# vandenheuvel/rust-lp

Measured on AMD Instinct MI355X. Metric: simplex iterations/sec, higher is better.
Workload: dtype f64; 1 GPU; dense10k: synthetic dense LP 10000x10000 f64 (+10000 slack columns), SteepestDescent, dense tableau with blocked f64-MFMA updates; m=10000, n=10000, seed=20250002, engine=tableau, update_block=64, parallelism=single GPU, solves=1

## Files before the change

include/relp_engine.h:

```cpp
#ifndef RELP_ENGINE_H
#define RELP_ENGINE_H

#include <stdint.h>

#ifdef __cplusplus
extern "C" {
#endif

typedef struct relp_engine relp_engine_t;

typedef enum {
    RELP_OK = 0,
    RELP_E_ARG = -1,
    RELP_E_HIP = -2,
    RELP_E_ZERO_PIVOT = -3,
    RELP_E_SINGULAR = -4,
    RELP_E_STATE = -5,
    RELP_E_UNSUPPORTED = -6,
    RELP_E_ALLOC = -7
} relp_status_t;

typedef enum {
    RELP_RUNNING = 0,
    RELP_OPTIMAL = 1,
    RELP_UNBOUNDED = 2,
    RELP_INFEASIBLE = 3,
    RELP_PHASE_ONE_DONE = 4,
    RELP_NO_ROW_PHASE_ONE = 5
} relp_outcome_t;

typedef enum {
    RELP_RULE_FIRST_PROFITABLE = 0,
    RELP_RULE_FIRST_PROFITABLE_WITH_MEMORY = 1,
    RELP_RULE_STEEPEST_DESCENT = 2
} relp_pivot_rule_t;

typedef enum { RELP_FORMAT_CSC = 0, RELP_FORMAT_DENSE = 1 } relp_format_t;
typedef enum { RELP_MEM_HOST = 0, RELP_MEM_DEVICE = 1 } relp_memory_t;

typedef struct {
    int32_t nr_normal;
    int32_t nr_eq, nr_range, nr_le, nr_ge;
    int32_t format;
    int32_t matrix_memory;
    const int64_t *col_ptr;
    const int32_t *row_idx;
    const double  *values;
    const double  *dense;
    int64_t        dense_ld;
    const double  *b;
    const double  *ranges;
    const double  *cost;
    const double  *upper_bound;
} relp_matrix_data_t;

typedef struct {
    int32_t device;
    int32_t phase_one_rule;
    int32_t phase_two_rule;
    double  tol_cost;
    double  tol_pivot;
    double  tol_zero;
    double  tol_tie;
    double  tol_feas;
    int32_t poll_interval;
    int32_t trace_capacity;
    int32_t shard_rank, shard_count;
    int32_t update_block;
    int32_t engine;
    int32_t ratio_rule;
    int32_t artificial_removal;
    int32_t pivot_rescue;
    int32_t auto_reinversion;
} relp_config_t;

typedef enum { RELP_RATIO_REFERENCE = 0, RELP_RATIO_LARGEST_PIVOT = 1 } relp_ratio_rule_t;
typedef enum { RELP_ARTIFICIAL_REFERENCE = 0, RELP_ARTIFICIAL_TEXTBOOK = 1 } relp_artificial_removal_t;

typedef enum {
    RELP_ENGINE_REVISED = 0,
    RELP_ENGINE_TABLEAU = 1,
    RELP_ENGINE_LU = 2,
    RELP_ENGINE_AUTO = 3
} relp_engine_kind_t;

void relp_default_config(relp_config_t *cfg);
void relp_robust_config(relp_config_t *cfg);
int32_t relp_engine_kind(const relp_engine_t *h);
relp_status_t relp_robust_stats(const relp_engine_t *h, int64_t *out4);
const char *relp_last_error(const relp_engine_t *h);
const char *relp_version(void);

relp_status_t relp_engine_create(const relp_matrix_data_t *md, const relp_config_t *cfg, relp_engine_t **out);
void          relp_engine_destroy(relp_engine_t *h);
relp_status_t relp_set_stream(relp_engine_t *h, void *hip_stream);

relp_status_t relp_select_primal_pivot_column(relp_engine_t *h, int32_t rule, int32_t *found,
                                              int32_t *column, double *relative_cost);
relp_status_t relp_relative_costs(relp_engine_t *h, double *out_n);
relp_status_t relp_generate_column(relp_engine_t *h, int32_t column, double *out_m);
relp_status_t relp_generate_element(relp_engine_t *h, int32_t row, int32_t column, double *out);
relp_status_t relp_select_primal_pivot_row(relp_engine_t *h, int32_t *found, int32_t *row);
relp_status_t relp_select_primal_pivot_row_of(relp_engine_t *h, const double *column_m, int32_t *found, int32_t *row);
relp_status_t relp_bring_into_basis(relp_engine_t *h, int32_t column, int32_t row, double relative_cost,
                                    int32_t *leaving_column);

relp_status_t relp_run(relp_engine_t *h, int64_t max_iters, int64_t *iterations_done, int32_t *outcome);
relp_status_t relp_solve_relaxation(relp_engine_t *h, int64_t max_iters, int32_t *outcome);
relp_status_t relp_from_basis(relp_engine_t *h, const int32_t *basis_columns_m);
relp_status_t relp_set_reinversion_interval(relp_engine_t *h, int64_t pivots);
int64_t       relp_reinversions(const relp_engine_t *h);
relp_status_t relp_flush(relp_engine_t *h);
relp_status_t relp_tab_flush_stats(relp_engine_t *h, int64_t *out2);
int32_t       relp_update_block(const relp_engine_t *h);
relp_status_t relp_lu_stats(const relp_engine_t *h, int64_t *out8);
relp_status_t relp_lu_lookahead_stats(const relp_engine_t *h, int64_t *out4);
relp_status_t relp_lu_kernel_layout(const relp_engine_t *h, int32_t *out4);
relp_status_t relp_lu_set_device_factorisation(relp_engine_t *h, int32_t on);
relp_status_t relp_lu_device_factorisation_stats(const relp_engine_t *h, int64_t *out6);
relp_status_t relp_lu_factor_residual(relp_engine_t *h, double *out);

relp_status_t relp_lu_phase_cycles(relp_engine_t *h, int64_t *out16);

relp_status_t relp_basis_inverse_row(relp_engine_t *h, int32_t row, double *out_m);
relp_status_t relp_should_refactor(relp_engine_t *h, int32_t *out);
relp_status_t relp_generate_column_of(relp_engine_t *h, const int32_t *row_idx, const double *values, int32_t nnz, double *out_m);
relp_status_t relp_cost_difference_of(relp_engine_t *h, const int32_t *row_idx, const double *values, int32_t nnz, double *out);
relp_status_t relp_lu_change_basis(relp_engine_t *h, int32_t pivot_row_index);
relp_status_t relp_lu_set_factors(relp_engine_t *h, const int64_t *l_col_ptr, const int32_t *l_row_idx, const double *l_values,
                                  const int64_t *u_col_ptr, const int32_t *u_row_idx, const double *u_values);
relp_status_t relp_lu_updates(relp_engine_t *h, int32_t *count);
relp_status_t relp_lu_get_update(relp_engine_t *h, int32_t k, int32_t *pivot, int32_t *idx, double *values, int32_t cap, int32_t *nnz);
relp_status_t relp_lu_get_upper(relp_engine_t *h, int64_t *col_ptr_m1, int32_t *row_idx, double *values, int64_t cap, int64_t *nnz);

int32_t relp_nr_rows(const relp_engine_t *h);
int32_t relp_nr_columns(const relp_engine_t *h);
int32_t relp_phase(const relp_engine_t *h);
int32_t relp_nr_artificial(const relp_engine_t *h);
relp_status_t relp_get_objective(relp_engine_t *h, double *out);
relp_status_t relp_get_b(relp_engine_t *h, double *out_m);
relp_status_t relp_get_minus_pi(relp_engine_t *h, double *out_m);
relp_status_t relp_get_basis_indices(relp_engine_t *h, int32_t *out_m);
relp_status_t relp_get_basis_inverse(relp_engine_t *h, double *out_mm);
relp_status_t relp_current_bfs(relp_engine_t *h, int32_t *cols, double *vals, int32_t cap, int32_t *count);
relp_status_t relp_get_iterations(relp_engine_t *h, int64_t *out);
relp_status_t relp_get_degenerate_pivots(relp_engine_t *h, int64_t *out);
relp_status_t relp_get_trace(relp_engine_t *h, int32_t *phase, int32_t *entering, int32_t *row,
                             int32_t *leaving, int64_t cap, int64_t *count);
relp_status_t relp_check_basis(relp_engine_t *h, double *max_identity_error, double *max_basic_cost,
                               double *min_b);

typedef enum {
    RELP_K_PRICE = 0, RELP_K_SELECT_COLUMN = 1, RELP_K_BUILD_COLUMN = 2, RELP_K_FTRAN = 3,
    RELP_K_RATIO = 4, RELP_K_UPDATE_VECTORS = 5, RELP_K_UPDATE_INVERSE = 6,
    RELP_K_APPLY_W = 7,
    RELP_K_UPDATE_W = 8,
    RELP_K_FLUSH = 9,
    RELP_K_FT_RUN = 10,
    RELP_K_COUNT = 11
} relp_kernel_id_t;
relp_status_t relp_profile_enable(relp_engine_t *h, int32_t enable, int64_t max_launches, int32_t sample_every);
relp_status_t relp_profile_read(relp_engine_t *h, int32_t kernel_id, int64_t *launches, double *total_ms);

relp_status_t relp_synth_fill_dense(double *device_a, int64_t ld, int32_t m, int32_t n, uint64_t seed,
                                    int64_t first_column, void *hip_stream);
relp_status_t relp_device_alloc(void **out, int64_t bytes);
relp_status_t relp_device_free(void *p);

relp_status_t relp_shard_ranges(const relp_engine_t *h, int32_t *col_lo, int32_t *col_hi,
                                int32_t *row_lo, int32_t *row_hi, int32_t *row_slice_stride);
void          relp_shard_column_range(int32_t nr_normal, int32_t rank, int32_t count, int32_t *lo, int32_t *hi);
int64_t       relp_shard_candidate_len(const relp_engine_t *h);
int64_t       relp_shard_rho_len(const relp_engine_t *h);
relp_status_t relp_shard_price(relp_engine_t *h, double *dev_candidate);
relp_status_t relp_shard_select_column(relp_engine_t *h, const double *dev_candidates, int32_t count);
relp_status_t relp_shard_ftran(relp_engine_t *h, double *dev_alpha_slice);
relp_status_t relp_shard_ratio(relp_engine_t *h, const double *dev_alpha_slices, int32_t count, double *dev_rho);
relp_status_t relp_shard_update(relp_engine_t *h, const double *dev_rho);
relp_status_t relp_shard_plan(const relp_matrix_data_t *md, const relp_config_t *cfg, int32_t *col_lo, int32_t *col_hi);
relp_status_t relp_shard_pivot(relp_engine_t *h);
relp_status_t relp_shard_flush_begin(relp_engine_t *h, double **dev_snapshot, int64_t *len_doubles);
relp_status_t relp_shard_flush_end(relp_engine_t *h);
relp_status_t relp_poll(relp_engine_t *h, int32_t *outcome, int64_t *iterations);

typedef int (*relp_allgather_fn)(void *ctx, const void *dev_send, void *dev_recv, int64_t bytes_per_rank, void *hip_stream);
typedef int (*relp_allreduce_sum_fn)(void *ctx, double *dev_buf, int64_t count, void *hip_stream);
relp_status_t relp_shard_set_collectives(relp_engine_t *h, relp_allgather_fn allgather, relp_allreduce_sum_fn allreduce_sum,
                                         void *ctx);
relp_status_t relp_shard_run(relp_engine_t *h, int64_t max_iters, int64_t *done, int32_t *outcome);
relp_status_t relp_shard_inject_failure(relp_engine_t *h, int64_t after_pivots);
#define RELP_RCCL_ID_BYTES 128
relp_status_t relp_rccl_unique_id(uint8_t id[RELP_RCCL_ID_BYTES]);
relp_status_t relp_rccl_attach(relp_engine_t *h, const uint8_t id[RELP_RCCL_ID_BYTES]);

#ifdef __cplusplus
}
#endif
#endif
```

rust-lp_amd/csrc/relp_abi.cpp:

```cpp
#include <cstring>
#include <new>

#include "relp_engine.hpp"

using relp::Engine;

struct relp_engine { Engine impl; };

#define H(h) ((h)->impl)

extern "C" {

void relp_default_config(relp_config_t* cfg) {
    std::memset(cfg, 0, sizeof(*cfg));
    cfg->device = -1;
    cfg->phase_one_rule = RELP_RULE_FIRST_PROFITABLE_WITH_MEMORY;
    cfg->phase_two_rule = RELP_RULE_STEEPEST_DESCENT;
    cfg->tol_cost = 1e-7; cfg->tol_pivot = 1e-5; cfg->tol_zero = 1e-11; cfg->tol_tie = 1e-9; cfg->tol_feas = 1e-7;
    cfg->poll_interval = 64;
    cfg->trace_capacity = 0;
    cfg->shard_rank = 0; cfg->shard_count = 1;
    cfg->update_block = -1;
    cfg->engine = RELP_ENGINE_REVISED;
}

void relp_robust_config(relp_config_t* cfg) {
    relp_default_config(cfg);
    cfg->ratio_rule = RELP_RATIO_LARGEST_PIVOT;
    cfg->artificial_removal = RELP_ARTIFICIAL_TEXTBOOK;
    cfg->pivot_rescue = 1;
    cfg->auto_reinversion = 1;
    cfg->engine = RELP_ENGINE_AUTO;
}
int32_t relp_engine_kind(const relp_engine_t* h) { return h ? H(h).engine_kind() : -1; }
relp_status_t relp_robust_stats(const relp_engine_t* h, int64_t* out4) { return (h && out4) ? H(h).robust_stats(out4) : RELP_E_ARG; }

const char* relp_last_error(const relp_engine_t* h) { return h ? H(h).last_error() : "null handle"; }
const char* relp_version(void) { return "relp-mi355x 0.2 (gfx950; engines: explicit inverse, dense tableau, sparse LU + Forrest-Tomlin)"; }

relp_status_t relp_engine_create(const relp_matrix_data_t* md, const relp_config_t* cfg, relp_engine_t** out) {
    if (!md || !cfg || !out) return RELP_E_ARG;
    relp_engine_t* h = new (std::nothrow) relp_engine_t();
    if (!h) return RELP_E_ALLOC;
    relp_status_t st = H(h).create(*md, *cfg);
    *out = h;
    return st;
}

void relp_engine_destroy(relp_engine_t* h) { delete h; }
relp_status_t relp_set_stream(relp_engine_t* h, void* s) { return h ? H(h).set_stream((hipStream_t)s) : RELP_E_ARG; }

relp_status_t relp_select_primal_pivot_column(relp_engine_t* h, int32_t rule, int32_t* found, int32_t* column, double* cost) {
    return h ? H(h).select_primal_pivot_column(rule, found, column, cost) : RELP_E_ARG;
}
relp_status_t relp_relative_costs(relp_engine_t* h, double* out) { return (h && out) ? H(h).relative_costs(out) : RELP_E_ARG; }
relp_status_t relp_generate_column(relp_engine_t* h, int32_t column, double* out) { return h ? H(h).generate_column(column, out) : RELP_E_ARG; }
relp_status_t relp_generate_element(relp_engine_t* h, int32_t row, int32_t column, double* out) {
    return h ? H(h).generate_element(row, column, out) : RELP_E_ARG;
}
relp_status_t relp_select_primal_pivot_row(relp_engine_t* h, int32_t* found, int32_t* row) {
    return h ? H(h).select_primal_pivot_row(found, row) : RELP_E_ARG;
}
relp_status_t relp_select_primal_pivot_row_of(relp_engine_t* h, const double* column, int32_t* found, int32_t* row) {
    return (h && column) ? H(h).select_primal_pivot_row_of(column, found, row) : RELP_E_ARG;
}
relp_status_t relp_bring_into_basis(relp_engine_t* h, int32_t column, int32_t row, double cost, int32_t* leaving) {
    return h ? H(h).bring_into_basis(column, row, cost, leaving) : RELP_E_ARG;
}

relp_status_t relp_run(relp_engine_t* h, int64_t max_iters, int64_t* done, int32_t* outcome) {
    return h ? H(h).run(max_iters, done, outcome) : RELP_E_ARG;
}
relp_status_t relp_solve_relaxation(relp_engine_t* h, int64_t max_iters, int32_t* outcome) {
    return h ? H(h).solve_relaxation(max_iters, outcome) : RELP_E_ARG;
}
relp_status_t relp_from_basis(relp_engine_t* h, const int32_t* basis) { return (h && basis) ? H(h).from_basis(basis) : RELP_E_ARG; }

relp_status_t relp_flush(relp_engine_t* h) { return h ? H(h).flush() : RELP_E_ARG; }
relp_status_t relp_set_reinversion_interval(relp_engine_t* h, int64_t pivots) { return h ? H(h).set_reinversion_interval(pivots) : RELP_E_ARG; }
int64_t relp_reinversions(const relp_engine_t* h) { return h ? H(h).reinversions() : -1; }
int32_t relp_update_block(const relp_engine_t* h) { return h ? H(h).update_block() : -1; }
relp_status_t relp_lu_stats(const relp_engine_t* h, int64_t* out8) { return (h && out8) ? H(h).lu_stats(out8) : RELP_E_ARG; }
relp_status_t relp_lu_lookahead_stats(const relp_engine_t* h, int64_t* out4) { return (h && out4) ? H(h).lu_lookahead_stats(out4) : RELP_E_ARG; }
relp_status_t relp_lu_kernel_layout(const relp_engine_t* h, int32_t* out4) { return (h && out4) ? H(h).lu_kernel_layout(out4) : RELP_E_ARG; }
relp_status_t relp_lu_set_device_factorisation(relp_engine_t* h, int32_t on) { return h ? H(h).lu_set_device_factorisation(on != 0) : RELP_E_ARG; }
relp_status_t relp_lu_factor_residual(relp_engine_t* h, double* out) { return (h && out) ? H(h).lu_factor_residual(out) : RELP_E_ARG; }
relp_status_t relp_lu_device_factorisation_stats(const relp_engine_t* h, int64_t* out6) { return (h && out6) ? H(h).luf_stats(out6) : RELP_E_ARG; }
relp_status_t relp_shard_inject_failure(relp_engine_t* h, int64_t after_pivots) { if (!h) return RELP_E_ARG; H(h).shard_inject_failure(after_pivots); return RELP_OK; }
relp_status_t relp_lu_phase_cycles(relp_engine_t* h, int64_t* out16) { return (h && out16) ? H(h).lu_phase_cycles(out16) : RELP_E_ARG; }
relp_status_t relp_basis_inverse_row(relp_engine_t* h, int32_t row, double* out_m) { return (h && out_m) ? H(h).basis_inverse_row(row, out_m) : RELP_E_ARG; }
relp_status_t relp_should_refactor(relp_engine_t* h, int32_t* out) { return (h && out) ? H(h).should_refactor(out) : RELP_E_ARG; }
relp_status_t relp_generate_column_of(relp_engine_t* h, const int32_t* idx, const double* val, int32_t nnz, double* out_m) {
    return h ? H(h).generate_column_of(idx, val, nnz, out_m) : RELP_E_ARG;
}
relp_status_t relp_cost_difference_of(relp_engine_t* h, const int32_t* idx, const double* val, int32_t nnz, double* out) {
    return h ? H(h).cost_difference_of(idx, val, nnz, out) : RELP_E_ARG;
}
relp_status_t relp_lu_change_basis(relp_engine_t* h, int32_t row) { return h ? H(h).lu_change_basis(row) : RELP_E_ARG; }
relp_status_t relp_lu_set_factors(relp_engine_t* h, const int64_t* l_ptr, const int32_t* l_idx, const double* l_val,
                                  const int64_t* u_ptr, const int32_t* u_idx, const double* u_val) {
    return h ? H(h).lu_set_factors(l_ptr, l_idx, l_val, u_ptr, u_idx, u_val) : RELP_E_ARG;
}
relp_status_t relp_lu_updates(relp_engine_t* h, int32_t* count) { return (h && count) ? H(h).lu_updates(count) : RELP_E_ARG; }
relp_status_t relp_lu_get_update(relp_engine_t* h, int32_t k, int32_t* pivot, int32_t* idx, double* val, int32_t cap, int32_t* nnz) {
    return h ? H(h).lu_get_update(k, pivot, idx, val, cap, nnz) : RELP_E_ARG;
}
relp_status_t relp_lu_get_upper(relp_engine_t* h, int64_t* col_ptr, int32_t* row_idx, double* values, int64_t cap, int64_t* nnz) {
    return h ? H(h).lu_get_upper(col_ptr, row_idx, values, cap, nnz) : RELP_E_ARG;
}
relp_status_t relp_shard_flush_begin(relp_engine_t* h, double** snap, int64_t* len) {
    return h ? H(h).shard_flush_begin(snap, len) : RELP_E_ARG;
}
relp_status_t relp_shard_flush_end(relp_engine_t* h) { return h ? H(h).shard_flush_end() : RELP_E_ARG; }
relp_status_t relp_shard_set_collectives(relp_engine_t* h, relp_allgather_fn ag, relp_allreduce_sum_fn ar, void* ctx) {
    return h ? H(h).shard_set_collectives(ag, ar, ctx) : RELP_E_ARG;
}
relp_status_t relp_shard_run(relp_engine_t* h, int64_t max_iters, int64_t* done, int32_t* outcome) {
    return h ? H(h).shard_run(max_iters, done, outcome) : RELP_E_ARG;
}
relp_status_t relp_rccl_attach(relp_engine_t* h, const uint8_t* id) { return (h && id) ? H(h).rccl_attach(id) : RELP_E_ARG; }

int32_t relp_nr_rows(const relp_engine_t* h) { return h ? H(h).nr_rows() : -1; }
int32_t relp_nr_columns(const relp_engine_t* h) { return h ? H(h).nr_columns() : -1; }
int32_t relp_phase(const relp_engine_t* h) { return h ? H(h).phase() : -1; }
int32_t relp_nr_artificial(const relp_engine_t* h) { return h ? H(h).nr_artificial() : -1; }
relp_status_t relp_get_objective(relp_engine_t* h, double* out) { return (h && out) ? H(h).get_objective(out) : RELP_E_ARG; }
relp_status_t relp_get_b(relp_engine_t* h, double* out) { return (h && out) ? H(h).get_vector(0, out) : RELP_E_ARG; }
relp_status_t relp_get_minus_pi(relp_engine_t* h, double* out) { return (h && out) ? H(h).get_vector(1, out) : RELP_E_ARG; }
relp_status_t relp_get_basis_indices(relp_engine_t* h, int32_t* out) { return (h && out) ? H(h).get_basis_indices(out) : RELP_E_ARG; }
relp_status_t relp_get_basis_inverse(relp_engine_t* h, double* out) { return (h && out) ? H(h).get_basis_inverse(out) : RELP_E_ARG; }
relp_status_t relp_current_bfs(relp_engine_t* h, int32_t* cols, double* vals, int32_t cap, int32_t* count) {
    return h ? H(h).current_bfs(cols, vals, cap, count) : RELP_E_ARG;
}
relp_status_t relp_get_iterations(relp_engine_t* h, int64_t* out) { return (h && out) ? H(h).get_iterations(out) : RELP_E_ARG; }
relp_status_t relp_get_degenerate_pivots(relp_engine_t* h, int64_t* out) { return (h && out) ? H(h).get_degenerate_pivots(out) : RELP_E_ARG; }
relp_status_t relp_tab_flush_stats(relp_engine_t* h, int64_t* out2) { return (h && out2) ? H(h).tab_flush_stats(out2) : RELP_E_ARG; }
relp_status_t relp_get_trace(relp_engine_t* h, int32_t* phase, int32_t* entering, int32_t* row, int32_t* leaving,
                             int64_t cap, int64_t* count) {
    return h ? H(h).get_trace(phase, entering, row, leaving, cap, count) : RELP_E_ARG;
}
relp_status_t relp_check_basis(relp_engine_t* h, double* e1, double* e2, double* mb) { return h ? H(h).check_basis(e1, e2, mb) : RELP_E_ARG; }

relp_status_t relp_profile_enable(relp_engine_t* h, int32_t enable, int64_t max_launches, int32_t sample_every) {
    return h ? H(h).profile_enable(enable != 0, max_launches, sample_every) : RELP_E_ARG;
}
relp_status_t relp_profile_read(relp_engine_t* h, int32_t kid, int64_t* launches, double* total_ms) {
    return h ? H(h).profile_read(kid, launches, total_ms) : RELP_E_ARG;
}

relp_status_t relp_synth_fill_dense(double* device_a, int64_t ld, int32_t m, int32_t n, uint64_t seed,
                                    int64_t first_column, void* hip_stream) {
    if (!device_a || ld < m || m < 0 || n < 0) return RELP_E_ARG;
    relp::launch_fill_dense(device_a, ld, m, n, seed, first_column, (hipStream_t)hip_stream);
    if (hipStreamSynchronize((hipStream_t)hip_stream) != hipSuccess) return RELP_E_HIP;
    return hipGetLastError() == hipSuccess ? RELP_OK : RELP_E_HIP;
}
relp_status_t relp_device_alloc(void** out, int64_t bytes) {
    if (!out || bytes < 0) return RELP_E_ARG;
    return hipMalloc(out, (size_t)(bytes ? bytes : 1)) == hipSuccess ? RELP_OK : RELP_E_ALLOC;
}
relp_status_t relp_device_free(void* p) { return hipFree(p) == hipSuccess ? RELP_OK : RELP_E_HIP; }

relp_status_t relp_shard_ranges(const relp_engine_t* h, int32_t* col_lo, int32_t* col_hi, int32_t* row_lo,
                                int32_t* row_hi, int32_t* stride) {
    if (!h) return RELP_E_ARG;
    H(h).shard_ranges(col_lo, col_hi, row_lo, row_hi, stride);
    return RELP_OK;
}
void relp_shard_column_range(int32_t nr_normal, int32_t rank, int32_t count, int32_t* lo, int32_t* hi) {
    relp::shard_column_range(nr_normal, rank, count, lo, hi);
}
int64_t relp_shard_candidate_len(const relp_engine_t* h) { return h ? H(h).candidate_len() : -1; }
int64_t relp_shard_rho_len(const relp_engine_t* h) { return h ? H(h).rho_len() : -1; }
relp_status_t relp_shard_price(relp_engine_t* h, double* c) { return (h && c) ? H(h).shard_price(c) : RELP_E_ARG; }
relp_status_t relp_shard_select_column(relp_engine_t* h, const double* c, int32_t count) {
    return (h && c) ? H(h).shard_select_column(c, count) : RELP_E_ARG;
}
relp_status_t relp_shard_ftran(relp_engine_t* h, double* a) { return (h && a) ? H(h).shard_ftran(a) : RELP_E_ARG; }
relp_status_t relp_shard_ratio(relp_engine_t* h, const double* a, int32_t count, double* rho) {
    return (h && a && rho) ? H(h).shard_ratio(a, count, rho) : RELP_E_ARG;
}
relp_status_t relp_shard_update(relp_engine_t* h, const double* rho) { return (h && rho) ? H(h).shard_update(rho) : RELP_E_ARG; }
relp_status_t relp_shard_pivot(relp_engine_t* h) { return h ? H(h).shard_pivot() : RELP_E_ARG; }
relp_status_t relp_shard_plan(const relp_matrix_data_t* md, const relp_config_t* cfg, int32_t* col_lo, int32_t* col_hi) {
    if (!md || !cfg) return RELP_E_ARG;
    relp::Layout layout;
    const relp_status_t st = layout.plan(*md, *cfg, nullptr);
    if (st) return st;
    if (col_lo) *col_lo = layout.col_lo;
    if (col_hi) *col_hi = layout.col_hi;
    return RELP_OK;
}
relp_status_t relp_poll(relp_engine_t* h, int32_t* outcome, int64_t* iterations) { return h ? H(h).poll(outcome, iterations) : RELP_E_ARG; }

}
```

rust-lp_amd/csrc/relp_engine.cpp:

```cpp
#include "relp_engine_internal.hpp"

#include <algorithm>
#include <chrono>
#include <cmath>
#include <cstdio>
#include <cstdlib>
#include <cstring>
#include <limits>

namespace relp {

bool Engine::hip_ok(hipError_t e, const char* what) {
    if (e == hipSuccess) return true;
    err_ = std::string(what) + ": " + hipGetErrorString(e);
    return false;
}

void Engine::free_all() {
    luf_release();
    auto fr = [](auto*& p) { if (p) { (void)hipFree(p); p = nullptr; } };
    if (owns_A_) fr(dA_);
    dA_ = nullptr;
    fr(dBinv_); fr(d_minus_pi_); fr(d_b_); fr(d_alpha_); fr(d_aq_); fr(d_rho_); fr(d_d_); fr(d_w_); fr(d_cost_);
    fr(d_basis_); fr(d_column_to_row_); fr(d_bound_row_); fr(d_vrow0_); fr(d_vrow1_); fr(d_vsign_); fr(d_trace_);
    fr(d_in_basis_); fr(d_rec_);
    fr(d_part_k1_); fr(d_part_j_);
    fr(d_fcols_); fr(d_fcount_); fr(d_fmask_); fr(d_fstats_); fr(d_R0c_);
    fr(dT0_); fr(dR0_); fr(d_b_alt_); fr(d_basis_alt_); fr(d_shadow_); fr(d_shadow_meta_);
    if (h_lu_buf_) { (void)hipHostFree(h_lu_buf_); h_lu_buf_ = nullptr; h_lu_cap_ = 0; }
    if (h_basis_) { (void)hipHostFree(h_basis_); h_basis_ = nullptr; }
    if (h_mirror_) { (void)hipHostFree(h_mirror_); h_mirror_ = nullptr; d_mirror_ = nullptr; }
    fr(d_cost_store_); fr(d_idcol_); fr(d_rmin_);
    fr(d_msg_cand_); fr(d_msg_cands_); fr(d_msg_slice_); fr(d_msg_slices_); fr(d_msg_rho_); fr(d_msg_status_); fr(d_msg_statuses_);
    fr(d_v_); fr(d_W_); fr(d_wr_); fr(d_R_); fr(d_S_); fr(d_pos_of_row_);
    fr(d_cptr_); fr(d_cidx_); fr(d_cval_); fr(d_lu_buf_); fr(d_lu_buf_alt_); fr(d_lu_scratch_); fr(d_ft_buf_); fr(d_pe_buf_);
    if (h_ft_hdr_) { (void)hipHostFree(h_ft_hdr_); h_ft_hdr_ = nullptr; }
    if (h_rec_) { (void)hipHostFree(h_rec_); h_rec_ = nullptr; }
    for (auto e : prof_ev_) (void)hipEventDestroy(e);
    prof_ev_.clear();
    if (owns_stream_ && stream_) { (void)hipStreamDestroy(stream_); }
    stream_ = nullptr;
}

Engine::~Engine() { rccl_release(); free_all(); }

ColumnTable Engine::table() const {
    ColumnTable ct;
    ct.nr_artificial = lay_.nr_artificial;
    ct.nr_normal = lay_.nr_normal;
    ct.nr_virtual = lay_.nr_virtual;
    ct.nr_constraints = lay_.mc;
    ct.column_to_row = d_column_to_row_;
    ct.bound_row = d_bound_row_;
    ct.vrow0 = d_vrow0_;
    ct.vrow1 = d_vrow1_;
    ct.vsign = d_vsign_;
    ct.cost = d_cost_;
    return ct;
}

Tolerances Engine::tolerances() const { return Tolerances{cfg_.tol_cost, cfg_.tol_pivot, cfg_.tol_zero, cfg_.tol_tie, cfg_.ratio_rule, (pivot_guard_on_ && guard_rel_ > 0.0) ? 1 : 0, guard_rel_}; }

TableauView Engine::tview() const {
    TableauView tv;
    tv.T0 = dT0_ - (int64_t)lay_.sc_lo * ld_t_; tv.ld_t = ld_t_;
    tv.R0 = dR0_ - (int64_t)lay_.sc_lo; tv.ld_r = ld_r_;
    tv.d = d_d_; tv.m = lay_.m; tv.n_store = n_store_;
    tv.col_off = phase_ == 1 ? 0 : tab_na_;
    tv.n = nr_columns();
    tv.c_lo = lay_.sc_lo; tv.c_hi = lay_.sc_hi;
    return tv;
}

FlushList Engine::flush_list() const {
    FlushList fl;
    fl.cols = d_fcols_; fl.count = d_fcount_; fl.mask = d_fmask_; fl.R0c = d_R0c_; fl.ld = ld_r_; fl.stats = d_fstats_;
    return fl;
}

SelectPartials Engine::tab_partials(int rule) const {
    SelectPartials sp;
    sp.k1 = d_part_k1_; sp.j = d_part_j_; sp.in_basis = d_in_basis_; sp.tol_cost = cfg_.tol_cost; sp.rule = rule;
    sp.n = nr_columns(); sp.offset = 0; sp.nb_struct = 0; sp.tol_tie = cfg_.tol_tie; sp.p_lo = 0; sp.cols_per_slot = 8;
    return sp;
}

DeferredUpdate Engine::deferred() const {
    DeferredUpdate du;
    du.W = d_W_; du.ld = ld_b_; du.kmax = block_; du.S = d_S_; du.pos_of_row = d_pos_of_row_; du.wr = d_wr_; du.R = d_R_;
    return du;
}

relp_status_t Engine::download_rec() {
    HIP_TRY(hipMemcpyAsync(h_rec_, d_rec_, sizeof(PivotRecord), hipMemcpyDeviceToHost, stream_));
    HIP_TRY(hipStreamSynchronize(stream_));
    return RELP_OK;
}

relp_status_t Engine::upload_rec() {
    HIP_TRY(hipMemcpyAsync(d_rec_, h_rec_, sizeof(PivotRecord), hipMemcpyHostToDevice, stream_));
    HIP_TRY(hipStreamSynchronize(stream_));
    return RELP_OK;
}

relp_status_t Engine::set_stream(hipStream_t s) {
    if (stream_) HIP_TRY(hipStreamSynchronize(stream_));
    if (owns_stream_ && stream_) HIP_TRY(hipStreamDestroy(stream_));
    stream_ = s;
    owns_stream_ = false;
    return RELP_OK;
}

relp_status_t Engine::create(const relp_matrix_data_t& md, const relp_config_t& cfg) {
    (void)hipGetLastError();
    cfg_ = cfg;
    if (cfg_.shard_count < 1) cfg_.shard_count = 1;
    if (cfg_.poll_interval < 1) cfg_.poll_interval = 64;
    if (const relp_status_t lst = lay_.build(md, cfg_, &err_)) return lst;
    if (cfg_.device >= 0) HIP_TRY(hipSetDevice(cfg_.device));
    phase_ = 1;
    n_alloc_ = lay_.nr_columns();

    HIP_TRY(hipStreamCreateWithFlags(&stream_, hipStreamNonBlocking));
    owns_stream_ = true;
    const int32_t n_local = lay_.col_hi - lay_.col_lo;
    lu_ = lay_.engine == RELP_ENGINE_LU;
    tableau_ = lay_.engine == RELP_ENGINE_TABLEAU;
    if (lu_) {
        if (cfg_.shard_count > 1) return fail(RELP_E_UNSUPPORTED, "the LU engine is not sharded");
        relp_status_t lst = lu_load_matrix(md);
        if (lst) return lst;
    } else if (md.format == RELP_FORMAT_DENSE) {
        if (lay_.nr_normal > 0 && lay_.mc > 0 && !md.dense) return fail(RELP_E_ARG, "dense matrix missing");
        const int64_t src_ld = md.dense_ld > 0 ? md.dense_ld : lay_.mc;
        if (src_ld < lay_.mc) return fail(RELP_E_ARG, "dense_ld < nr_constraints");
        if (md.matrix_memory == RELP_MEM_DEVICE && (src_ld % 2) == 0) {
            dA_ = const_cast<double*>(md.dense); ld_a_ = src_ld; owns_A_ = false;
        } else {
            ld_a_ = round_up(std::max<int64_t>(lay_.mc, 1), 2);
            HIP_TRY(dev_alloc(&dA_, ld_a_ * std::max(n_local, 1)));
            owns_A_ = true;
            if (n_local > 0 && lay_.mc > 0)
                HIP_TRY(hipMemcpy2D(dA_, ld_a_ * sizeof(double), md.dense, src_ld * sizeof(double), lay_.mc * sizeof(double),
                                    n_local, md.matrix_memory == RELP_MEM_DEVICE ? hipMemcpyDeviceToDevice : hipMemcpyHostToDevice));
        }
    } else if (md.format == RELP_FORMAT_CSC) {
        if (md.matrix_memory != RELP_MEM_HOST) return fail(RELP_E_UNSUPPORTED, "CSC input must be in host memory");
        if (!md.col_ptr) return fail(RELP_E_ARG, "col_ptr missing");
        ld_a_ = round_up(std::max<int64_t>(lay_.mc, 1), 2);
        const int64_t e0 = n_local > 0 ? md.col_ptr[lay_.col_lo] : 0, e1 = n_local > 0 ? md.col_ptr[lay_.col_hi] : 0;
        for (int64_t p = e0; p < e1; ++p)
            if (md.row_idx[p] < 0 || md.row_idx[p] >= lay_.mc) return fail(RELP_E_ARG, "row index out of range");
        const int64_t cells = ld_a_ * std::max(n_local, 1);
        HIP_TRY(dev_alloc(&dA_, cells));
        owns_A_ = true;
        HIP_TRY(hipMemset(dA_, 0, (size_t)cells * sizeof(double)));
        if (e1 > e0) {
            int64_t* t_ptr = nullptr; int32_t* t_idx = nullptr; double* t_val = nullptr;
            auto drop = [&]() { if (t_ptr) (void)hipFree(t_ptr); if (t_idx) (void)hipFree(t_idx); if (t_val) (void)hipFree(t_val); };
            if (hipMalloc(reinterpret_cast<void**>(&t_ptr), sizeof(int64_t) * (size_t)(n_local + 1)) != hipSuccess ||
                hipMalloc(reinterpret_cast<void**>(&t_idx), sizeof(int32_t) * (size_t)(e1 - e0)) != hipSuccess ||
                hipMalloc(reinterpret_cast<void**>(&t_val), sizeof(double) * (size_t)(e1 - e0)) != hipSuccess) {
                drop();
                return fail(RELP_E_ALLOC, "staging the CSC arrays");
            }
            hipError_t err = hipMemcpy(t_ptr, md.col_ptr + lay_.col_lo, sizeof(int64_t) * (size_t)(n_local + 1), hipMemcpyHostToDevice);
            if (err == hipSuccess) err = hipMemcpy(t_idx, md.row_idx + e0, sizeof(int32_t) * (size_t)(e1 - e0), hipMemcpyHostToDevice);
            if (err == hipSuccess) err = hipMemcpy(t_val, md.values + e0, sizeof(double) * (size_t)(e1 - e0), hipMemcpyHostToDevice);
            if (err == hipSuccess) {
                launch_csc_to_dense(t_ptr, t_idx, t_val, n_local, dA_, ld_a_, nullptr);
                err = hipDeviceSynchronize();
            }
            drop();
            if (err != hipSuccess) return fail(RELP_E_HIP, "dense copy of the CSC input");
        }
    } else {
        return fail(RELP_E_ARG, "unknown matrix format");
    }

    ld_b_ = round_up(lay_.m, 16);
    const int64_t rows_local = std::max(lay_.row_hi - lay_.row_lo, 1);
    HIP_TRY(dev_alloc(&dBinv_, (tableau_ || lu_) ? 16 : rows_local * ld_b_));
    HIP_TRY(dev_alloc(&d_minus_pi_, ld_b_));
    HIP_TRY(dev_alloc(&d_b_, ld_b_));
    HIP_TRY(dev_alloc(&d_alpha_, ld_b_));
    HIP_TRY(dev_alloc(&d_aq_, ld_b_));
    HIP_TRY(dev_alloc(&d_rho_, ld_b_));
    HIP_TRY(dev_alloc(&d_w_, ld_b_));
    HIP_TRY(dev_alloc(&d_d_, n_alloc_));
    HIP_TRY(dev_alloc(&d_cost_, lay_.nr_normal));
    HIP_TRY(dev_alloc(&d_basis_, lay_.m));
    HIP_TRY(dev_alloc(&d_column_to_row_, lay_.nr_artificial));
    HIP_TRY(dev_alloc(&d_bound_row_, lay_.nr_normal));
    HIP_TRY(dev_alloc(&d_vrow0_, lay_.nr_virtual));
    HIP_TRY(dev_alloc(&d_vrow1_, lay_.nr_virtual));
    HIP_TRY(dev_alloc(&d_vsign_, lay_.nr_virtual));
    HIP_TRY(dev_alloc(&d_in_basis_, n_alloc_));
    HIP_TRY(dev_alloc(&d_rec_, 1));
    {
        const int64_t slots = price_structural_blocks(lay_.col_lo, lay_.col_hi) + (lay_.nr_artificial + lay_.nr_virtual + 255) / 256 + 8 +
                              tab_scan_blocks(n_alloc_) + price_csc_blocks(0, lay_.nr_normal);
        HIP_TRY(dev_alloc(&d_part_k1_, slots));
        HIP_TRY(dev_alloc(&d_part_j_, slots));
    }
    block_ = cfg_.update_block < 0 ? (lay_.m >= 4096 ? 64 : 0) : std::min(cfg_.update_block, 128);
    if (lu_) {
        block_ = cfg_.update_block < 0 ? 128 : std::max(1, std::min(cfg_.update_block, 128));
        HIP_TRY(dev_alloc(&d_lu_scratch_, ld_b_));
        {
            const char* la = std::getenv("RELP_LU_LOOKAHEAD");
            const char* fl = std::getenv("RELP_FUSE_LANES");
            const char* df = std::getenv("RELP_LU_DEVICE_FACTOR");
            luf_enabled_ = df && std::atoi(df) != 0;
            luf_download_ = df && std::atoi(df) == 2;
            lu_lookahead_env_ = la ? std::atoi(la) : 8;
            lu_lookahead_set_ = la != nullptr;
            lu_fuse_lanes_env_ = fl ? std::atoi(fl) : 256;
        }
        relp_status_t fst = ft_plan_and_alloc();
        if (fst) return fst;
    }
    if (tableau_) {
        if (block_ == 0) block_ = 64;
        if (cfg_.update_block < 0 && lay_.m >= 4096 && n_alloc_ >= 40000) block_ = 96;
        n_store_ = n_alloc_;
        tab_na_ = lay_.nr_artificial;
        const int64_t n_owned = std::max(lay_.sc_hi - lay_.sc_lo, 1);
        ld_t_ = round_up(lay_.m, 2);
        ld_r_ = round_up(n_owned, 2);
        HIP_TRY(dev_alloc(&dT0_, ld_t_ * n_owned));
        HIP_TRY(dev_alloc(&dR0_, ld_r_ * (block_ + 1)));
        {
            const char* e = std::getenv("RELP_TAB_FLUSH_ALL");
            flush_all_ = e && std::atoi(e) != 0;
            HIP_TRY(dev_alloc(&d_fstats_, 2));
            if (!flush_all_) {
                HIP_TRY(dev_alloc(&d_fcols_, n_owned));
                HIP_TRY(dev_alloc(&d_fcount_, 1));
                HIP_TRY(dev_alloc(&d_fmask_, (n_owned + 63) / 64));
                HIP_TRY(dev_alloc(&d_R0c_, ld_r_ * block_));
            }
        }
        {
            const char* e = std::getenv("RELP_FUSED_UPDATE");
            fused_update_ = !(e && std::atoi(e) == 0);
            if (cfg_.pivot_rescue && cfg_.shard_count == 1) fused_update_ = false;
            if (fused_update_) {
                HIP_TRY(dev_alloc(&d_b_alt_, ld_b_));
                HIP_TRY(dev_alloc(&d_basis_alt_, lay_.m));
                HIP_TRY(dev_alloc(&d_shadow_, std::max(block_, 1) + 1));
                HIP_TRY(hipMalloc(reinterpret_cast<void**>(&d_shadow_meta_), 2 * sizeof(int32_t)));
                const int32_t none[2] = {-1, 0};
                HIP_TRY(hipMemcpy(d_shadow_meta_, none, sizeof none, hipMemcpyHostToDevice));
            }
        }
        HIP_TRY(dev_alloc(&d_cost_store_, n_store_));
        HIP_TRY(dev_alloc(&d_idcol_, lay_.m));
    }
    if (block_ > 0 && ft_) {
        HIP_TRY(dev_alloc(&d_v_, ld_b_));
    } else if (block_ > 0) {
        HIP_TRY(dev_alloc(&d_v_, ld_b_));
        HIP_TRY(dev_alloc(&d_W_, ld_b_ * block_));
        if (!tableau_) HIP_TRY(dev_alloc(&d_R_, ld_b_ * block_));
        HIP_TRY(dev_alloc(&d_wr_, block_));
        HIP_TRY(dev_alloc(&d_S_, block_));
        HIP_TRY(dev_alloc(&d_pos_of_row_, lay_.m));
        HIP_TRY(hipMemset(d_pos_of_row_, 0xFF, sizeof(int32_t) * lay_.m));
    }
    HIP_TRY(dev_alloc(&d_rmin_, lay_.m / 8 + 2));
    HIP_TRY(hipHostMalloc(reinterpret_cast<void**>(&h_rec_), sizeof(PivotRecord), hipHostMallocDefault));
    trace_cap_ = std::max(cfg_.trace_capacity, 0);
    if (trace_cap_ > 0) HIP_TRY(dev_alloc(&d_trace_, 4 * trace_cap_));

    auto up = [&](void* dst, const void* src, size_t bytes) -> hipError_t {
        return bytes ? hipMemcpy(dst, src, bytes, hipMemcpyHostToDevice) : hipSuccess;
    };
    HIP_TRY(up(d_cost_, lay_.cost.data(), sizeof(double) * lay_.nr_normal));
    HIP_TRY(up(d_bound_row_, lay_.bound_row.data(), sizeof(int32_t) * lay_.nr_normal));
    HIP_TRY(up(d_vrow0_, lay_.vrow0.data(), sizeof(int32_t) * lay_.nr_virtual));
    HIP_TRY(up(d_vrow1_, lay_.vrow1.data(), sizeof(int32_t) * lay_.nr_virtual));
    HIP_TRY(up(d_vsign_, lay_.vsign.data(), sizeof(int32_t) * lay_.nr_virtual));
    HIP_TRY(up(d_column_to_row_, lay_.column_to_row.data(), sizeof(int32_t) * lay_.nr_artificial));
    HIP_TRY(up(d_basis_, lay_.basis.data(), sizeof(int32_t) * lay_.m));
    HIP_TRY(up(d_b_, lay_.rhs.data(), sizeof(double) * lay_.m));
    HIP_TRY(up(d_minus_pi_, lay_.minus_pi.data(), sizeof(double) * lay_.m));
    std::vector<uint8_t> flags(n_alloc_, 0);
    for (int32_t r = 0; r < lay_.m; ++r) flags[lay_.basis[r]] = 1;
    HIP_TRY(up(d_in_basis_, flags.data(), flags.size()));
    if (lay_.row_hi > lay_.row_lo && !tableau_ && !lu_) launch_set_identity(dBinv_, ld_b_, lay_.row_lo, lay_.row_hi, stream_);
    if (tableau_) {
        idcol_h_ = lay_.basis;
        HIP_TRY(up(d_idcol_, idcol_h_.data(), sizeof(int32_t) * lay_.m));
        const double* A = dA_ - (int64_t)lay_.col_lo * ld_a_;
        launch_tab_build(tview(), A, ld_a_, table(), stream_);
        cost_store_h_.assign(n_store_, 0.0);
        for (int32_t k = 0; k < lay_.nr_artificial; ++k) cost_store_h_[k] = 1.0;
        std::vector<double> w(ld_b_, 0.0);
        for (int32_t k = 0; k < lay_.nr_artificial; ++k) w[lay_.column_to_row[k]] = 1.0;
        HIP_TRY(up(d_cost_store_, cost_store_h_.data(), sizeof(double) * n_store_));
        HIP_TRY(up(d_w_, w.data(), sizeof(double) * ld_b_));
        launch_tab_price_init(tview(), d_w_, d_cost_store_, stream_);
    }
    {
        bool sparse_input = false;
        if (md.format == RELP_FORMAT_CSC && md.col_ptr && lay_.nr_normal > 0 && lay_.mc > 0)
            sparse_input = (double)md.col_ptr[lay_.nr_normal] <= 0.10 * (double)lay_.nr_normal * (double)lay_.mc;
        reinvert_interval_ = (!lu_ && cfg_.shard_count == 1 && lay_.m <= 4096 && sparse_input) ? 1000 : 0;
        if (cfg_.auto_reinversion && !lu_ && cfg_.shard_count == 1) reinvert_interval_ = 256;
    }
    std::memset(h_rec_, 0, sizeof(PivotRecord));
    h_rec_->outcome = DEV_RUNNING;
    h_rec_->minus_objective = -lay_.phase1_objective;
    h_rec_->last_selected = -1;
    h_rec_->phase = 1;
    relp_status_t st = upload_rec();
    if (st) return st;
    HIP_TRY(hipDeviceSynchronize());
    if (hipGetLastError() != hipSuccess) return fail(RELP_E_HIP, "a kernel launch of the set-up failed");
    if (lu_ && (st = lu_refactor())) return st;
    return RELP_OK;
}

relp_status_t Engine::profile_enable(bool enable, int64_t max_launches, int32_t sample_every) {
    prof_stride_ = sample_every > 0 ? sample_every : 1;
    prof_tick_ = 0;
    HIP_TRY(hipStreamSynchronize(stream_));
    for (auto e : prof_ev_) (void)hipEventDestroy(e);
    prof_ev_.clear(); prof_kid_.clear(); prof_open_ = false;
    prof_on_ = enable;
    if (enable) {
        prof_ev_.resize((size_t)max_launches * 2);
        for (auto& e : prof_ev_) HIP_TRY(hipEventCreate(&e));
        prof_kid_.reserve((size_t)max_launches);
    }
    return RELP_OK;
}

void Engine::prof_begin(int kid, hipStream_t on) {
    prof_open_ = false;
    if (!prof_on_ || (prof_kid_.size() + 1) * 2 > prof_ev_.size()) return;
    if (kid != RELP_K_FLUSH && (prof_tick_ % prof_stride_) != 0) return;
    (void)hipEventRecord(prof_ev_[2 * prof_kid_.size()], on ? on : stream_);
    prof_kid_.push_back(kid);
    prof_open_ = true;
}

void Engine::prof_end(hipStream_t on) {
    if (!prof_open_) return;
    (void)hipEventRecord(prof_ev_[2 * (prof_kid_.size() - 1) + 1], on ? on : stream_);
    prof_open_ = false;
}

relp_status_t Engine::profile_read(int kernel_id, int64_t* launches, double* total_ms) {
    HIP_TRY(hipStreamSynchronize(stream_));
    int64_t n = 0; double ms = 0.0;
    for (size_t k = 0; k < prof_kid_.size(); ++k) {
        if (prof_kid_[k] != kernel_id) continue;
        float t = 0.f;
        if (hipEventElapsedTime(&t, prof_ev_[2 * k], prof_ev_[2 * k + 1]) == hipSuccess) { ms += t; ++n; }
    }
    if (launches) *launches = n;
    if (total_ms) *total_ms = ms;
    return RELP_OK;
}

void Engine::enqueue_price(int cost_mode, const double* vec, const PivotRecord* rec, int32_t p_lo, int32_t p_hi) {
    const ColumnTable ct = table();
    if (lu_) {
        launch_price_csc(csc(), ct, vec, d_d_, 0, lay_.nr_normal, cost_mode, SelectPartials{}, rec, stream_);
        launch_price_virtual(ct, vec, d_d_, cost_mode, rec, stream_);
        return;
    }
    const double* A = dA_ - (int64_t)lay_.col_lo * ld_a_;
    launch_price_structural(A, ld_a_, ct, vec, d_d_, p_lo, p_hi, cost_mode, rec, stream_);
    if (p_lo > 0 || p_hi < lay_.nr_normal) launch_price_mask_unowned(ct, d_d_, p_lo, p_hi, rec, stream_);
    launch_price_virtual(ct, vec, d_d_, cost_mode, rec, stream_);
}

void Engine::enqueue_iteration_tableau(int rule) {
    const TableauView tv = tview();
    const DeferredUpdate du = deferred();
    const SelectPartials sp = tab_partials(rule);
    if (fused_update_ && in_loop_) {
        prof_begin(RELP_K_FTRAN);
        launch_tab_select_column_rmin(tv, du, sp, tab_scan_blocks(lay_.sc_hi - lay_.sc_lo), d_alpha_, d_b_, tolerances(), d_rmin_,
                                      d_rec_, stream_, d_shadow_, d_shadow_meta_);
        prof_end();
        prof_begin(RELP_K_PRICE);
        launch_tab_ratio_update_all(tv, du, sp, lay_.m, d_alpha_, d_b_, d_b_alt_, d_basis_, d_basis_alt_, d_in_basis_, d_trace_,
                                    trace_cap_, tolerances(), d_rmin_, d_shadow_, d_shadow_meta_, d_rec_, stream_);
        prof_end();
        std::swap(d_b_, d_b_alt_);
        std::swap(d_basis_, d_basis_alt_);
        shadow_pending_ = true;
        if (++since_flush_ >= block_) enqueue_flush();
        return;
    }
    tab_settle();
    prof_begin(RELP_K_FTRAN);
    launch_tab_select_column_rmin(tv, du, sp, tab_scan_blocks(lay_.sc_hi - lay_.sc_lo), d_alpha_, d_b_, tolerances(), d_rmin_,
                                  d_rec_, stream_);
    prof_end();
    prof_begin(RELP_K_RATIO);
    launch_ratio_blocks(d_alpha_, d_b_, d_basis_, lay_.m, tolerances(), du, d_rmin_, d_rec_, stream_);
    prof_end();
    prof_begin(RELP_K_PRICE);
    launch_tab_update_all(tv, du, sp, lay_.m, d_alpha_, d_b_, d_basis_, d_in_basis_, d_trace_, trace_cap_, d_rec_, stream_);
    prof_end();
    if (++since_flush_ >= block_) enqueue_flush();
}

void Engine::enqueue_iteration(int rule) {
    struct Tick { int64_t& t; ~Tick() { ++t; } } tick{prof_tick_};
    if (tableau_) { enqueue_iteration_tableau(rule); return; }
    if (lu_) { enqueue_iteration_lu(rule); return; }
    const ColumnTable ct = table();
    const double* A = dA_ - (int64_t)lay_.col_lo * ld_a_;
    double* Binv = dBinv_ - (int64_t)lay_.row_lo * ld_b_;
    const int n = nr_columns();
    SelectPartials sp;
    sp.k1 = d_part_k1_; sp.j = d_part_j_; sp.in_basis = d_in_basis_; sp.tol_cost = cfg_.tol_cost; sp.rule = rule;
    const int nb_struct = price_structural_blocks(lay_.col_lo, lay_.col_hi);
    sp.n = n; sp.offset = 0; sp.nb_struct = nb_struct; sp.tol_tie = cfg_.tol_tie; sp.p_lo = lay_.col_lo; sp.cols_per_slot = 8;
    const int nb_virt = price_virtual_blocks(ct);
    prof_begin(RELP_K_PRICE);
    if (lay_.col_lo > 0 || lay_.col_hi < lay_.nr_normal) {
        launch_price_structural_sel(A, ld_a_, ct, d_minus_pi_, d_d_, lay_.col_lo, lay_.col_hi, phase_, sp, d_rec_, stream_);
        launch_price_mask_unowned(ct, d_d_, lay_.col_lo, lay_.col_hi, d_rec_, stream_);
        SelectPartials spv = sp;
        spv.offset = nb_struct;
        launch_price_virtual_sel(ct, d_minus_pi_, d_d_, phase_, spv, d_rec_, stream_);
    } else {
        launch_price_all_sel(A, ld_a_, ct, d_minus_pi_, d_d_, lay_.col_lo, lay_.col_hi, phase_, sp, d_rec_, stream_);
    }
    prof_end();
    prof_begin(RELP_K_SELECT_COLUMN);
    launch_select_partials(sp, nb_struct + nb_virt, d_d_, A, ld_a_, ct, lay_.m, d_aq_, d_rec_, stream_);
    prof_end();
    if (block_ == 0) {
        prof_begin(RELP_K_FTRAN);
        launch_ftran_rmin(Binv, ld_b_, lay_.m, d_aq_, d_alpha_, d_b_, tolerances(), d_rmin_, d_rec_, stream_);
        prof_end();
        prof_begin(RELP_K_RATIO);
        launch_ratio_rows(d_alpha_, d_b_, d_basis_, lay_.m, tolerances(), DeferredUpdate{}, d_rmin_, ftran_rows_per_block(), d_rec_,
                          stream_);
        prof_end();
        prof_begin(RELP_K_UPDATE_VECTORS);
        launch_compute_rho(Binv, ld_b_, lay_.m, lay_.row_lo, lay_.row_hi, d_rho_, d_rec_, stream_);
        prof_end();
        prof_begin(RELP_K_UPDATE_INVERSE);
        launch_update_inverse_vectors(Binv, ld_b_, lay_.m, d_alpha_, d_rho_, d_b_, d_minus_pi_, d_basis_, d_in_basis_, d_trace_,
                                      trace_cap_, d_rec_, stream_);
        prof_end();
        return;
    }
    const DeferredUpdate du = deferred();
    prof_begin(RELP_K_FTRAN);
    launch_ftran(Binv, ld_b_, lay_.m, lay_.row_lo, lay_.row_hi, d_aq_, d_v_, 0, d_rec_, stream_);
    prof_end();
    prof_begin(RELP_K_APPLY_W);
    launch_apply_w_rmin(du, lay_.m, d_v_, d_alpha_, d_b_, tolerances(), d_rmin_, d_rec_, stream_);
    prof_end();
    prof_begin(RELP_K_RATIO);
    launch_ratio_rows(d_alpha_, d_b_, d_basis_, lay_.m, tolerances(), du, d_rmin_, 256, d_rec_, stream_);
    prof_end();
    prof_begin(RELP_K_UPDATE_W);
    launch_update_w(du, lay_.m, d_alpha_, d_rec_, stream_);
    launch_rho_deferred(du, Binv, ld_b_, lay_.m, lay_.row_lo, lay_.row_hi, d_rho_, d_rec_, stream_);
    prof_end();
    prof_begin(RELP_K_UPDATE_VECTORS);
    launch_update_vectors(lay_.m, d_alpha_, d_rho_, d_b_, d_minus_pi_, d_basis_, d_in_basis_, d_trace_, trace_cap_, d_rec_,
                          stream_);
    prof_end();
    if (++since_flush_ >= block_) enqueue_flush();
}

void Engine::tab_settle() {
    if (shadow_pending_) {
        launch_tab_apply_shadow(deferred(), d_shadow_, d_shadow_meta_, stream_);
        shadow_pending_ = false;
    }
}

void Engine::enqueue_flush() {
    if (block_ == 0) return;
    if (lu_) {
        if (since_flush_ == 0 && !ft_need_refactor_) return;
        prof_begin(RELP_K_FLUSH);
        const relp_status_t st = lu_refactor();
        prof_end();
        if (st && !lu_status_) lu_status_ = st;
        return;
    }
    if (tableau_) {
        tab_settle();
        const DeferredUpdate dut = deferred();
        prof_begin(RELP_K_FLUSH);
        launch_tab_flush(tview(), dut, d_rec_, flush_list(), stream_);
        launch_flush_reset(dut, d_rec_, stream_);
        prof_end();
        since_flush_ = 0;
        if (++flushes_since_reprice_ >= kRepriceEveryFlushes) {
            flushes_since_reprice_ = 0;
            const TableauView tv = tview();
            const int rule = phase_ == 1 ? cfg_.phase_one_rule : cfg_.phase_two_rule;
            launch_tab_basis_costs(tv, d_basis_, d_cost_store_, d_w_, stream_);
            launch_tab_price_init(tv, d_w_, d_cost_store_, stream_);
            launch_tab_scan(tv, tab_partials(rule), d_rec_, stream_);
        }
        return;
    }
    const DeferredUpdate du = deferred();
    double* Binv = dBinv_ - (int64_t)lay_.row_lo * ld_b_;
    prof_begin(RELP_K_FLUSH);
    launch_flush_snapshot(du, Binv, ld_b_, lay_.row_lo, lay_.row_hi, d_rec_, stream_);
    launch_flush_apply(du, Binv, ld_b_, lay_.m, lay_.row_lo, lay_.row_hi, d_rec_, stream_);
    launch_flush_reset(du, d_rec_, stream_);
    prof_end();
    since_flush_ = 0;
}

relp_status_t Engine::flush() {
    tab_settle();
    if (cfg_.shard_count > 1 && block_ > 0 && !tableau_) {
        if (!coll_allreduce_) return fail(RELP_E_STATE, "sharded flush needs relp_shard_flush_begin/end (or the collective hooks)");
        if (since_flush_ == 0) return RELP_OK;
        double* snap = nullptr; int64_t len = 0;
        relp_status_t st = shard_flush_begin(&snap, &len);
        if (st) return st;
        if (len > 0) {
            if (coll_allreduce_(coll_ctx_, snap, len, stream_)) return fail(RELP_E_HIP, "all-reduce of the flush snapshot failed");
            if ((st = shard_flush_end())) return st;
        }
        since_flush_ = 0;
        return RELP_OK;
    }
    enqueue_flush();
    return RELP_OK;
}

relp_status_t Engine::select_primal_pivot_column(int rule, int32_t* found, int32_t* column, double* cost) {
    relp_status_t st = download_rec();
    if (st) return st;
// ... 954 lines not shown
```

rust-lp_amd/csrc/relp_engine.hpp:

```cpp
#pragma once
#include <hip/hip_runtime.h>

#include <cstdint>
#include <chrono>
#include <condition_variable>
#include <functional>
#include <mutex>
#include <string>
#include <thread>
#include <vector>

#include "../../include/relp_engine.h"
#include "relp_kernels.h"
#include "relp_layout.hpp"
#include "relp_lu.hpp"

namespace relp {

class Engine {
  public:
    Engine() = default;
    ~Engine();

    relp_status_t create(const relp_matrix_data_t& md, const relp_config_t& cfg);
    relp_status_t set_stream(hipStream_t s);

    relp_status_t select_primal_pivot_column(int rule, int32_t* found, int32_t* column, double* cost);
    relp_status_t relative_costs(double* out_n);
    relp_status_t generate_column(int32_t column, double* out_m);
    relp_status_t generate_element(int32_t row, int32_t column, double* out);
    relp_status_t select_primal_pivot_row(int32_t* found, int32_t* row);
    relp_status_t select_primal_pivot_row_of(const double* column, int32_t* found, int32_t* row);
    relp_status_t bring_into_basis(int32_t column, int32_t row, double cost, int32_t* leaving);

    relp_status_t run(int64_t max_iters, int64_t* done, int32_t* outcome);
    int32_t engine_kind() const { return lay_.engine; }
    relp_status_t robust_stats(int64_t* out4) const;
    relp_status_t solve_relaxation(int64_t max_iters, int32_t* outcome);
    relp_status_t from_basis(const int32_t* basis_columns);
    relp_status_t set_reinversion_interval(int64_t pivots);
    int64_t reinversions() const { return reinversions_; }
    relp_status_t flush();
    int32_t update_block() const { return block_; }
    relp_status_t lu_stats(int64_t* out8) const;
    relp_status_t lu_lookahead_stats(int64_t* out4) const;
    relp_status_t lu_kernel_layout(int32_t* out4) const;
    relp_status_t luf_stats(int64_t* out6) const;
    relp_status_t lu_set_device_factorisation(bool on);
    relp_status_t lu_factor_residual(double* out);
    relp_status_t lu_basis_columns(std::vector<std::vector<std::pair<int32_t, double>>>& cols);
    relp_status_t lu_basis_flat(std::vector<int64_t>& ptr, std::vector<int32_t>& idx, std::vector<double>& val);
    relp_status_t lu_phase_cycles(int64_t* out16);
    relp_status_t lu_download_basis();
    relp_status_t lu_factor_downloaded_basis();
    relp_status_t lu_refactor_lookahead(int rule, int64_t budget, bool have_basis);
    relp_status_t ft_read_report(bool* have_basis);
    void lu_refactor_clock(std::chrono::steady_clock::time_point tb, std::chrono::steady_clock::time_point t0,
                           std::chrono::steady_clock::time_point t1, std::chrono::steady_clock::time_point t2);
    relp_status_t basis_inverse_row(int32_t row, double* out_m);
    relp_status_t should_refactor(int32_t* out);
    relp_status_t generate_column_of(const int32_t* idx, const double* val, int32_t nnz, double* out_m);
    relp_status_t cost_difference_of(const int32_t* idx, const double* val, int32_t nnz, double* out);
    relp_status_t lu_change_basis(int32_t row);
    relp_status_t lu_updates(int32_t* count);
    relp_status_t lu_get_update(int32_t k, int32_t* pivot, int32_t* idx, double* val, int32_t cap, int32_t* nnz);
    relp_status_t lu_get_upper(int64_t* col_ptr, int32_t* row_idx, double* values, int64_t cap, int64_t* nnz);
    relp_status_t lu_set_factors(const int64_t* l_ptr, const int32_t* l_idx, const double* l_val, const int64_t* u_ptr,
                                 const int32_t* u_idx, const double* u_val);
    relp_status_t shard_flush_begin(double** dev_snapshot, int64_t* len);
    relp_status_t shard_flush_end();

    int32_t nr_rows() const { return lay_.m; }
    int32_t nr_columns() const { return lay_.nr_columns(); }
    int32_t phase() const { return phase_; }
    int32_t nr_artificial() const { return lay_.nr_artificial; }
    relp_status_t get_objective(double* out);
    relp_status_t get_vector(int which, double* out);
    relp_status_t get_basis_indices(int32_t* out);
    relp_status_t get_basis_inverse(double* out);
    relp_status_t current_bfs(int32_t* cols, double* vals, int32_t cap, int32_t* count);
    relp_status_t get_iterations(int64_t* out);
    relp_status_t get_degenerate_pivots(int64_t* out);
    relp_status_t tab_flush_stats(int64_t* out2);
    relp_status_t get_trace(int32_t* phase, int32_t* entering, int32_t* row, int32_t* leaving, int64_t cap,
                            int64_t* count);
    relp_status_t check_basis(double* max_identity_error, double* max_basic_cost, double* min_b);

    relp_status_t profile_enable(bool enable, int64_t max_launches, int32_t sample_every);
    relp_status_t profile_read(int kernel_id, int64_t* launches, double* total_ms);

    void shard_ranges(int32_t* col_lo, int32_t* col_hi, int32_t* row_lo, int32_t* row_hi, int32_t* stride) const;
    int64_t candidate_len() const { return lay_.candidate_len; }
    int64_t rho_len() const { return ld_b_; }
    relp_status_t shard_price(double* dev_candidate);
    relp_status_t shard_select_column(const double* dev_candidates, int32_t count);
    relp_status_t shard_ftran(double* dev_alpha_slice);
    relp_status_t shard_ratio(const double* dev_alpha_slices, int32_t count, double* dev_rho);
    relp_status_t shard_update(const double* dev_rho);
    relp_status_t shard_pivot();
    relp_status_t shard_set_collectives(relp_allgather_fn ag, relp_allreduce_sum_fn ar, void* ctx);
    relp_status_t shard_run(int64_t max_iters, int64_t* done, int32_t* outcome);
    void shard_inject_failure(int64_t after_pivots) { inject_failure_after_ = after_pivots; }
    relp_status_t rccl_attach(const uint8_t* id);
    relp_status_t poll(int32_t* outcome, int64_t* iterations);

    const char* last_error() const { return err_.c_str(); }

  private:
    Layout lay_;
    relp_config_t cfg_{};
    int32_t phase_ = 1;

    double* dA_ = nullptr; int64_t ld_a_ = 0; bool owns_A_ = false;
    double* dBinv_ = nullptr; int64_t ld_b_ = 0;
    double *d_minus_pi_ = nullptr, *d_b_ = nullptr, *d_alpha_ = nullptr, *d_aq_ = nullptr, *d_rho_ = nullptr,
           *d_d_ = nullptr, *d_w_ = nullptr, *d_cost_ = nullptr;
    int32_t *d_basis_ = nullptr, *d_column_to_row_ = nullptr, *d_bound_row_ = nullptr, *d_vrow0_ = nullptr,
            *d_vrow1_ = nullptr, *d_vsign_ = nullptr, *d_trace_ = nullptr;
    uint8_t* d_in_basis_ = nullptr;
    PivotRecord* d_rec_ = nullptr;
    PivotRecord* h_rec_ = nullptr;
    hipStream_t stream_ = nullptr; bool owns_stream_ = false;
    int64_t trace_cap_ = 0;
    int32_t block_ = 0;
    int64_t since_flush_ = 0;
    double* d_v_ = nullptr;
    double *d_W_ = nullptr, *d_wr_ = nullptr, *d_R_ = nullptr;
    int32_t *d_S_ = nullptr, *d_pos_of_row_ = nullptr;
    double* d_part_k1_ = nullptr;
    int32_t* d_part_j_ = nullptr;
    bool tableau_ = false;
    double* dT0_ = nullptr; int64_t ld_t_ = 0;
    double* dR0_ = nullptr; int64_t ld_r_ = 0;
    bool flush_all_ = false;
    int32_t *d_fcols_ = nullptr, *d_fcount_ = nullptr;
    unsigned long long *d_fmask_ = nullptr, *d_fstats_ = nullptr;
    double* d_R0c_ = nullptr;
    FlushList flush_list() const;
    double* d_cost_store_ = nullptr;
    int32_t* d_idcol_ = nullptr;
    bool fused_update_ = false, shadow_pending_ = false;
    double *d_b_alt_ = nullptr, *d_shadow_ = nullptr;
    int32_t *d_basis_alt_ = nullptr, *d_shadow_meta_ = nullptr;
    double* d_rmin_ = nullptr;
    int32_t n_store_ = 0;
    int32_t tab_na_ = 0;
    bool tab_partials_valid_ = false;
    static constexpr int kRepriceEveryFlushes = 8;
    int32_t flushes_since_reprice_ = 0;
    std::vector<int32_t> idcol_h_;
    std::vector<double> cost_store_h_;
    bool in_loop_ = false;
    void tab_settle();
    struct LoopScope {
        Engine& e;
        explicit LoopScope(Engine& en) : e(en) { e.in_loop_ = true; }
        ~LoopScope() { e.in_loop_ = false; e.tab_settle(); }
    };
    struct SettledScope {
        Engine& e; bool was;
        explicit SettledScope(Engine& en) : e(en), was(en.in_loop_) { e.in_loop_ = false; e.tab_settle(); }
        ~SettledScope() { e.in_loop_ = was; }
    };
    TableauView tview() const;
    double* d_aq_big() { return dR0_ + (int64_t)block_ * ld_r_; }
    SelectPartials tab_partials(int rule) const;
    void enqueue_iteration_tableau(int rule);
    relp_status_t tableau_reprice();
    bool lu_ = false;
    std::vector<int64_t> hc_ptr_; std::vector<int32_t> hc_idx_; std::vector<double> hc_val_;
    int64_t* d_cptr_ = nullptr; int32_t* d_cidx_ = nullptr; double* d_cval_ = nullptr;
    LUFactors hlu_;
    char* d_lu_buf_ = nullptr; int64_t lu_cap_ = 0;
    std::vector<std::vector<std::pair<int32_t, double>>> basis_cols_;
    std::vector<int64_t> basis_ptr_; std::vector<int32_t> basis_idx_; std::vector<double> basis_val_;
    struct HostPool {
        struct Slot { std::thread th; std::mutex mu; std::condition_variable cv; std::function<void()> job; bool busy = false, stop = false; };
        Slot slot[2];
        void run(int i, std::function<void()> f) {
            Slot& s = slot[i];
            if (!s.th.joinable())
                s.th = std::thread([&s] {
                    std::unique_lock<std::mutex> lk(s.mu);
                    for (;;) {
                        s.cv.wait(lk, [&s] { return s.busy || s.stop; });
                        if (s.stop) return;
                        lk.unlock(); s.job(); lk.lock();
                        s.busy = false;
                        s.cv.notify_all();
                    }
                });
            { std::lock_guard<std::mutex> lk(s.mu); s.job = std::move(f); s.busy = true; }
            s.cv.notify_all();
        }
        void wait() {
            for (Slot& s : slot) { std::unique_lock<std::mutex> lk(s.mu); s.cv.wait(lk, [&s] { return !s.busy; }); }
        }
        ~HostPool() {
            for (Slot& s : slot) {
                if (!s.th.joinable()) continue;
                { std::lock_guard<std::mutex> lk(s.mu); s.stop = true; }
                s.cv.notify_all();
                s.th.join();
            }
        }
    } host_pool_;
    char* h_lu_buf_ = nullptr; size_t h_lu_cap_ = 0;
    char* d_lu_buf_alt_ = nullptr; int64_t lu_cap_alt_ = 0;
    int32_t* h_basis_ = nullptr; int32_t m_alloc_rows_ = 0;
    FtMirror* h_mirror_ = nullptr; FtMirror* d_mirror_ = nullptr;
    double* d_lu_scratch_ = nullptr;
    DeviceLU dlu_{};
    relp_status_t lu_status_ = RELP_OK;
    int64_t lu_refactors_ = 0;
    int64_t lu_lookahead_installs_ = 0, lu_replayed_changes_ = 0;
    int32_t lu_lookahead_env_ = 8, lu_fuse_lanes_env_ = 256;
    bool lu_lookahead_set_ = false;
    int32_t lu_pipeline_cap_ = 0;
    double refactor_us_[3] = {0.0, 0.0, 0.0};
    int64_t reinvert_interval_ = 0, since_reinvert_ = 0, reinversions_ = 0;
    DeviceCSC csc() const { return DeviceCSC{d_cptr_, d_cidx_, d_cval_}; }
    auto csc_column() const {
        return [this](int32_t p, auto&& put) { for (int64_t e = hc_ptr_[p]; e < hc_ptr_[p + 1]; ++e) put(hc_idx_[e], hc_val_[e]); };
    }
    relp_status_t lu_load_matrix(const relp_matrix_data_t& md);
    relp_status_t lu_refactor();
    relp_status_t lu_upload_factors();
    relp_status_t reinvert();
    relp_status_t retabulate();
    bool retab_done_ = false;
    relp_status_t build_basis_columns(const std::vector<int32_t>& basis, std::vector<std::vector<std::pair<int32_t, double>>>* cols);
    void enqueue_iteration_lu(int rule);
    bool ft_ = false;
    FtState fts_{};
    char* d_ft_buf_ = nullptr;
    int32_t* h_ft_hdr_ = nullptr;
    int32_t ft_tcap_ = 0, ft_eta_cap_ = 0;
    struct LufState;
    LufState* luf_ = nullptr;
    bool luf_enabled_ = false;
    int64_t luf_runs_ = 0, luf_fallbacks_ = 0, luf_lds_retries_ = 0; double luf_kernel_us_ = 0.0; int32_t luf_last_bump_ = 0, luf_last_peeled_ = 0;
    relp_status_t luf_prepare();
    relp_status_t lu_factor_on_device(int32_t* device_status);
    relp_status_t luf_download_factors();
    relp_status_t lu_host_factors();
    bool luf_is_resident() const;
    bool luf_download_ = false;
    void luf_release();
    void luf_mark_dirty();
    bool hyper_forced_ = false; int32_t hyper_probe_in_[4] = {0, 0, 0, 0};
    bool ft_big_ = false; int32_t ft_rhs_cap_ = 0;
    bool ft_grid_price_ = false;
    int32_t ft_tier_ = 0;
    int64_t ft_zero_bytes_ = 0, ft_ones_bytes_ = 0;
    bool ft_need_refactor_ = false;
    relp_status_t ft_plan_and_alloc();
    relp_status_t ft_reset();
    relp_status_t ft_read_hdr();
    FtProblem ft_problem(int rule) const;
    void ft_enqueue_pivots(const FtState& go, int rule, int64_t left);
    char* d_pe_buf_ = nullptr; PriceEll pe_{};
    relp_status_t ft_build_price_ell();
    relp_status_t run_ft(int64_t max_iters, int64_t* done, int32_t* outcome);
    DeferredUpdate deferred() const;
    void enqueue_flush();
    int32_t n_alloc_ = 0;

    relp_allgather_fn coll_allgather_ = nullptr;
    relp_allreduce_sum_fn coll_allreduce_ = nullptr;
    void* coll_ctx_ = nullptr;
    void* rccl_comm_ = nullptr;
    double* d_msg_cand_ = nullptr;
    double* d_msg_cands_ = nullptr;
    double* d_msg_slice_ = nullptr;
    double* d_msg_slices_ = nullptr;
    double* d_msg_rho_ = nullptr;
    relp_status_t shard_iteration();
    relp_status_t shard_iteration_comm_only(int from_step);
    int coll_step_ = 0;
    int64_t shadow_flush_ = 0;
    relp_status_t shard_agree_on_status(relp_status_t local);
    double* d_msg_status_ = nullptr;
    double* d_msg_statuses_ = nullptr;
    int64_t inject_failure_after_ = -1;
    bool coll_broken_ = false;
    relp_status_t remove_artificial_basis_variables_sharded(std::vector<int32_t>& rows_to_remove);
    void rccl_release();

    bool prof_on_ = false;
    std::vector<hipEvent_t> prof_ev_;
    std::vector<int> prof_kid_;
    bool prof_open_ = false;
    int32_t prof_stride_ = 1;
    int64_t prof_tick_ = 0;

    std::string err_;

    ColumnTable table() const;
    Tolerances tolerances() const;
    bool hip_ok(hipError_t e, const char* what);
    relp_status_t fail(relp_status_t code, const std::string& msg) { err_ = msg; return code; }
    relp_status_t download_rec();
    relp_status_t upload_rec();
    void prof_begin(int kid, hipStream_t on = nullptr);
    void prof_end(hipStream_t on = nullptr);
    void enqueue_price(int cost_mode, const double* vec, const PivotRecord* rec, int32_t p_lo, int32_t p_hi);
    void enqueue_iteration(int rule);
    relp_status_t finish_phase_one(int32_t* outcome);
    relp_status_t remove_artificial_basis_variables(std::vector<int32_t>& rows_to_remove);
    relp_status_t switch_to_phase_two(const std::vector<int32_t>& rows_to_remove);
    std::vector<int32_t> stuck_artificials_;
    relp_status_t run_loop(int64_t max_iters, int64_t* done, int32_t* outcome);
    relp_status_t rescue_unbar_all();
    void auto_reinversion_adapt(const std::vector<double>& before, const std::vector<double>& after);
    std::vector<int32_t> barred_;
    double guard_rel_ = 0.0;
    bool pivot_guard_on_ = false;
    bool hold_phase_end_ = false;
    int64_t rescue_small_pivots_ = 0, rescue_barred_ = 0, rescue_confirmations_ = 0;
    double last_reinvert_drift_ = -1.0;
    relp_status_t remove_rows(const std::vector<int32_t>& rows);
    void free_all();
};

}
```

rust-lp_amd/csrc/relp_kernels.h:

```cpp
#pragma once
#include <hip/hip_runtime.h>
#include <stdint.h>

#include "relp_layout.hpp"

namespace relp {

enum DeviceOutcome : int32_t { DEV_RUNNING = 0, DEV_NO_CANDIDATE = 1, DEV_NO_ROW = 2 };

struct PivotRecord {
    int32_t outcome;
    int32_t q;
    double  d_q;
    int32_t r;
    int32_t leaving;
    double  alpha_r;
    double  b_r;
    double  minus_objective;
    long long iterations;
    int32_t last_selected;
    int32_t phase;
    int32_t owner_has_row;
    int32_t pad_;
    double  key1;
    int32_t n_eta;
    int32_t eta_target;
    int32_t n_eta_old;
    int32_t degenerate;
    int32_t p_now;
    int32_t pad2_;
};

struct DeferredUpdate {
    double*  W;
    int64_t  ld;
    int32_t  kmax;
    int32_t* S;
    int32_t* pos_of_row;
    double*  wr;
    double*  R;
};

struct ColumnTable {
    int32_t nr_artificial;
    int32_t nr_normal;
    int32_t nr_virtual;
    int32_t nr_constraints;
    const int32_t* column_to_row;
    const int32_t* bound_row;
    const int32_t* vrow0;
    const int32_t* vrow1;
    const int32_t* vsign;
    const double*  cost;
};

struct Tolerances { double cost, pivot, zero, tie; int32_t ratio_rule, pivot_guard; double guard_rel; };

struct SelectPartials {
    double*        k1;
    int32_t*       j;
    const uint8_t* in_basis;
    double         tol_cost;
    int32_t        rule;
    int32_t        n;
    int32_t        offset;
    int32_t        nb_struct;
    double         tol_tie;
    int32_t        p_lo;
    int32_t        cols_per_slot;
};

struct LuRow { int32_t k, e0, e1, pad_; double diag; };
struct DeviceSchedule {
    const LuRow* rows;
    const int32_t* idx; const double* val;
    const int32_t* level_ptr;
    int32_t n_levels; int32_t nnz;
    const int32_t* seg; int32_t n_seg; int32_t pad_;
};
struct DeviceLU {
    int32_t m; int32_t pad_;
    const int32_t* rowperm;
    const int32_t* colperm;
    DeviceSchedule Lf, Uf, Ub, Lb;
};
static constexpr int kEllLg = 13;
static constexpr int kEllLgWide = 24;
static constexpr int kEllPadHeaders = 4;
struct EllPass { int32_t lane0, lanes, info, level; };
struct EllSchedule {
    const EllPass*  passes;
    const int32_t*  lvl_pass;
    double*         rdiag;
    double*         sval;
    const double*   oval;
    const int32_t*  rovf;
    const uint16_t* sidx;
    const uint16_t* oidx;
    const int32_t*  via_ptr;
    const int32_t*  via_pos;
    int32_t n_passes, n_levels, m, n_lanes, n_ovf;
    int32_t bytes;
    int32_t rhs_base;
    int32_t n_triv;
    const int32_t* triv;
    const int32_t* reach;
    const int32_t* rhs_src;
    int32_t n_rhs, pad_;
    const int32_t* rhs_pos;
    const uint32_t* triv_bits;
};

struct DeviceCSC { const int64_t* col_ptr; const int32_t* row_idx; const double* values; };

static constexpr int kFtThreads = 512;
static constexpr int kFtWaves = kFtThreads / 64;
static constexpr int kFtMaxSlots = 64;
static constexpr int kFtMaxRows = 1 << 20;
static constexpr int kFtLdsBudget = 156 * 1024;
static constexpr int kFtBitmapBytes = 40 * 1024;
static inline __host__ __device__ int ft_bitmap_shift(int m, int rhs_cap) {
    int s = 0;
    while (((((long long)m + 1 + rhs_cap) >> s) + 64 + (((long long)m) >> s) + 64) / 8 > kFtBitmapBytes) ++s;
    return s;
}
struct FtPivotInfo {
    int32_t u_e0, u_e1;
    int32_t via_u0, via_u1;
    int32_t via_t0, via_t1;
    int32_t lev_ub, pad_;
};
struct FtState {
    int32_t  m, tcap, ldt, eta_cap;
    int32_t* hdr;
    int32_t* slot_pivot;
    int32_t* slot_prev;
    int32_t* slot_live;
    int32_t* tslot;
    double*  TC;
    int32_t* eta_off;
    int32_t* eta_idx; double* eta_val;
    int32_t* spk_off;
    int32_t* spk_idx; double* spk_val;
    const int32_t* inv_rowperm;
    const int32_t* inv_colperm;
    const int32_t* task_uf;
    const int32_t* task_ub;
    EllSchedule ell[4];
    const int32_t* lev_ub;
    const struct FtPivotInfo* pinfo;
    int32_t* journal;
    double*  spike;
    double*  sp_work;
    int32_t  hyper;
    int32_t  pad2_;
    double*  x_work;
    unsigned long long* chunk_mask;
    int32_t* nz_idx; double* nz_val;
    int32_t* rho_idx;
    int32_t* nzc;
    uint32_t* bits_save;
    int32_t  big;
    int32_t  rhs_cap;
    int32_t  stage[4];
    int32_t  stage_bytes;
    int32_t  lds_bytes;
    int32_t  max_updates;
    int32_t  pad_;
    long long* prof;
};
static constexpr int kPriceSlots = 8;
static constexpr int kPriceLongSlots = 24;
static constexpr int kPriceLongFlag = 0x8000;
static constexpr uint32_t kPriceLongFlag32 = 0x80000000u;
struct PriceEll {
    const uint16_t* idx; const double* val;
    const uint16_t* lidx; const double* lval;
    const uint32_t* idx32; const uint32_t* lidx32;
    const int32_t* long_cols;
    const int32_t* very_long;
    const uint16_t* long_of;
    int32_t n_long, n_very_long;
};
struct FtMirror {
    PivotRecord rec;
    int32_t hdr[4];
    int32_t walked[4], whole[4];
    int32_t sweeps[4];
    int32_t basis[1];
};
struct FtProblem {
    DeviceCSC csc; ColumnTable ct; PriceEll pe;
    double *minus_pi, *b, *alpha, *rho, *d;
    int32_t* basis; uint8_t* in_basis; int32_t* trace; int64_t trace_cap;
    PivotRecord* rec;
    FtMirror* mirror;
    Tolerances tol;
    int32_t rule, n, phase;
    int32_t external_price;
};

void launch_price_structural(const double* A, int64_t ld_a, const ColumnTable& ct, const double* minus_pi,
                             double* d, int32_t p_lo, int32_t p_hi, int32_t cost_mode, const PivotRecord* rec,
                             hipStream_t s);
void launch_price_mask_unowned(const ColumnTable& ct, double* d, int32_t p_lo, int32_t p_hi,
                               const PivotRecord* rec, hipStream_t s);
void launch_price_structural_sel(const double* A, int64_t ld_a, const ColumnTable& ct, const double* minus_pi,
                                 double* d, int32_t p_lo, int32_t p_hi, int32_t cost_mode, SelectPartials sp,
                                 const PivotRecord* rec, hipStream_t s);
void launch_price_virtual_sel(const ColumnTable& ct, const double* minus_pi, double* d, int32_t cost_mode,
                              SelectPartials sp, const PivotRecord* rec, hipStream_t s);
void launch_price_all_sel(const double* A, int64_t ld_a, const ColumnTable& ct, const double* minus_pi, double* d,
                          int32_t p_lo, int32_t p_hi, int32_t cost_mode, SelectPartials sp, const PivotRecord* rec,
                          hipStream_t s);
int32_t price_structural_blocks(int32_t p_lo, int32_t p_hi);
int32_t price_virtual_blocks(const ColumnTable& ct);
void launch_select_partials(SelectPartials sp, int32_t count, const double* d, const double* A, int64_t ld_a,
                            const ColumnTable& ct, int32_t m, double* aq, PivotRecord* rec, hipStream_t s);
void launch_ratio_eta(const double* alpha, const double* b, const int32_t* basis_indices, int32_t m, Tolerances tol,
                      const DeferredUpdate& du, PivotRecord* rec, hipStream_t s);
void launch_price_virtual(const ColumnTable& ct, const double* minus_pi, double* d, int32_t cost_mode,
                          const PivotRecord* rec, hipStream_t s);
void launch_select_column(const double* d, const uint8_t* in_basis, int32_t n, int32_t rule, double tol_cost,
                          double tol_tie, PivotRecord* rec, hipStream_t s);
void launch_build_column(const double* A, int64_t ld_a, const ColumnTable& ct, int32_t m, double* aq,
                         const PivotRecord* rec, hipStream_t s);
void launch_ftran(const double* Binv, int64_t ld_b, int32_t m, int32_t row_lo, int32_t row_hi,
                  const double* aq, double* out, int32_t out_offset, const PivotRecord* rec, hipStream_t s);
void launch_ratio(const double* alpha, const double* b, const int32_t* basis_indices, int32_t m,
                  Tolerances tol, PivotRecord* rec, hipStream_t s);
void launch_compute_rho(const double* Binv, int64_t ld_b, int32_t m, int32_t row_lo, int32_t row_hi,
                        double* rho, PivotRecord* rec, hipStream_t s);
void launch_update_vectors(int32_t m, const double* alpha, const double* rho, double* b, double* minus_pi,
                           int32_t* basis_indices, uint8_t* in_basis, int32_t* trace, int64_t trace_cap,
                           PivotRecord* rec, hipStream_t s);
void launch_update_inverse(double* Binv, int64_t ld_b, int32_t m, int32_t row_lo, int32_t row_hi,
                           const double* alpha, const double* rho, const PivotRecord* rec, hipStream_t s);
void launch_update_inverse_vectors(double* Binv, int64_t ld_b, int32_t m, const double* alpha, const double* rho, double* b,
                                   double* minus_pi, int32_t* basis_indices, uint8_t* in_basis, int32_t* trace,
                                   int64_t trace_cap, PivotRecord* rec, hipStream_t s);

void launch_weighted_column_sums(const double* Binv, int64_t ld_b, int32_t m, const double* w,
                                 double* minus_pi, hipStream_t s);
void launch_set_identity(double* Binv_local, int64_t ld_b, int32_t row_lo, int32_t row_hi, hipStream_t s);
void launch_fill_dense(double* A, int64_t ld, int32_t m, int32_t n, uint64_t seed, int64_t first_column,
                       hipStream_t s);
void launch_csc_to_dense(const int64_t* col_ptr, const int32_t* row_idx, const double* values, int32_t n_cols, double* A,
                         int64_t ld, hipStream_t s);

void launch_apply_w(const DeferredUpdate& du, int32_t m, const double* v, double* alpha, const PivotRecord* rec,
                    hipStream_t s);
int32_t ftran_rows_per_block();
void launch_ftran_rmin(const double* Binv, int64_t ld_b, int32_t m, const double* aq, double* out, const double* b,
                       Tolerances tol, double* rmin, const PivotRecord* rec, hipStream_t s);
void launch_apply_w_rmin(const DeferredUpdate& du, int32_t m, const double* v, double* alpha, const double* b, Tolerances tol,
                         double* rmin, const PivotRecord* rec, hipStream_t s);
void launch_ratio_rows(const double* alpha, const double* b, const int32_t* basis_indices, int32_t m, Tolerances tol,
                       const DeferredUpdate& du, const double* rmin, int32_t rows_per_block, PivotRecord* rec, hipStream_t s);
void launch_eta_prepare(const DeferredUpdate& du, PivotRecord* rec, hipStream_t s);
void launch_update_w(const DeferredUpdate& du, int32_t m, const double* alpha, const PivotRecord* rec, hipStream_t s);
void launch_rho_deferred(const DeferredUpdate& du, const double* Binv, int64_t ld_b, int32_t m, int32_t row_lo,
                         int32_t row_hi, double* rho, PivotRecord* rec, hipStream_t s);
void launch_flush_snapshot(const DeferredUpdate& du, const double* Binv, int64_t ld_b, int32_t row_lo, int32_t row_hi,
                           const PivotRecord* rec, hipStream_t s);
void launch_flush_apply(const DeferredUpdate& du, double* Binv, int64_t ld_b, int32_t m, int32_t row_lo,
                        int32_t row_hi, const PivotRecord* rec, hipStream_t s);
void launch_flush_reset(const DeferredUpdate& du, PivotRecord* rec, hipStream_t s);

struct TableauView {
    double*  T0;      int64_t ld_t;
    double*  R0;      int64_t ld_r;
    double*  d;
    int32_t  m;
    int32_t  n_store;
    int32_t  col_off;
    int32_t  n;
    int32_t  c_lo, c_hi;
};
void launch_tab_build(const TableauView& tv, const double* A, int64_t ld_a, const ColumnTable& ct, hipStream_t s);
void launch_tab_price_init(const TableauView& tv, const double* w, const double* cost_store, hipStream_t s);
void launch_tab_basis_costs(const TableauView& tv, const int32_t* basis_indices, const double* cost_store, double* w,
                            hipStream_t s);
void launch_tab_scan(const TableauView& tv, SelectPartials sp, const PivotRecord* rec, hipStream_t s);
int32_t tab_scan_blocks(int32_t n_owned_columns);
bool launch_lu_ftran_cols(const DeviceLU& lu, const TableauView& tv, const double* A, int64_t ld_a, const ColumnTable& ct,
                          int32_t c_first, int32_t c_count, hipStream_t s);
void launch_tab_select(const TableauView& tv, SelectPartials sp, int32_t count, PivotRecord* rec, hipStream_t s);
void launch_tab_column(const TableauView& tv, const DeferredUpdate& du, double* alpha, const PivotRecord* rec,
                       hipStream_t s);
void launch_tab_row_update(const TableauView& tv, const DeferredUpdate& du, SelectPartials sp, PivotRecord* rec,
                           hipStream_t s);
void launch_tab_update_vectors(int32_t m, const double* alpha, double* b, int32_t* basis_indices, uint8_t* in_basis,
                               int32_t* trace, int64_t trace_cap, PivotRecord* rec, hipStream_t s);
void launch_tab_update_w_vectors(const DeferredUpdate& du, int32_t m, const double* alpha, double* b,
                                 int32_t* basis_indices, uint8_t* in_basis, int32_t* trace, int64_t trace_cap,
                                 PivotRecord* rec, hipStream_t s);
void launch_tab_select_column(const TableauView& tv, const DeferredUpdate& du, SelectPartials sp, int32_t count,
                              double* alpha, PivotRecord* rec, hipStream_t s);
void launch_tab_select_column_rmin(const TableauView& tv, const DeferredUpdate& du, SelectPartials sp, int32_t count,
                                   double* alpha, const double* b, Tolerances tol, double* rmin, PivotRecord* rec,
                                   hipStream_t s, const double* shadow = nullptr, int32_t* shadow_meta = nullptr);
void launch_ratio_blocks(const double* alpha, const double* b, const int32_t* basis_indices, int32_t m, Tolerances tol,
                         const DeferredUpdate& du, const double* rmin, PivotRecord* rec, hipStream_t s);
void launch_tab_select_column_msg(const TableauView& tv, const DeferredUpdate& du, SelectPartials sp, int32_t count,
                                  double* msg, const double* b, Tolerances tol, PivotRecord* rec, hipStream_t s,
                                  const double* shadow = nullptr, int32_t* shadow_meta = nullptr);
void launch_tab_select_candidate_ratio(const double* msgs, int32_t count, int64_t msg_len, int32_t m, double* alpha,
                                       const double* b, const int32_t* basis_indices, int32_t rule, Tolerances tol,
                                       const DeferredUpdate& du, int32_t forced_row, PivotRecord* rec, hipStream_t s);
void launch_tab_zero_level_scan(const TableauView& tv, const DeferredUpdate& du, SelectPartials sp, int32_t row,
                                int32_t nr_artificial, Tolerances tol, const PivotRecord* rec, hipStream_t s);
void launch_select_candidate_ratio(const double* msgs, int32_t count, int64_t msg_len, int32_t m, double* alpha,
                                   const double* b, const int32_t* basis_indices, int32_t rule, Tolerances tol,
                                   const DeferredUpdate& du, PivotRecord* rec, hipStream_t s);
void launch_tab_update_all(const TableauView& tv, const DeferredUpdate& du, SelectPartials sp, int32_t m,
                           const double* alpha, double* b, int32_t* basis_indices, uint8_t* in_basis, int32_t* trace,
                           int64_t trace_cap, PivotRecord* rec, hipStream_t s);
struct FlushList {
    int32_t*            cols;
    int32_t*            count;
    unsigned long long* mask;
    double*             R0c;
    int64_t             ld;
    unsigned long long* stats;
};
void launch_tab_flush(const TableauView& tv, const DeferredUpdate& du, const PivotRecord* rec, const FlushList& fl,
                      hipStream_t s);
void launch_tab_ratio_update_all(const TableauView& tv, const DeferredUpdate& du, SelectPartials sp, int32_t m,
                                 const double* alpha, const double* b_in, double* b_out, const int32_t* basis_in,
                                 int32_t* basis_out, uint8_t* in_basis, int32_t* trace, int64_t trace_cap, Tolerances tol,
                                 const double* rmin, double* shadow, int32_t* shadow_meta, PivotRecord* rec, hipStream_t s,
                                 const double* msgs = nullptr, int32_t count = 0, int64_t msg_len = 0, int32_t rule = 0);
void launch_tab_apply_shadow(const DeferredUpdate& du, double* shadow, int32_t* shadow_meta, hipStream_t s);
void launch_tab_gather_columns(const TableauView& tv, const int32_t* cols, double* out, hipStream_t s);
void launch_tab_row(const TableauView& tv, const DeferredUpdate& du, int32_t row, double* out, const PivotRecord* rec,
                    hipStream_t s);

void launch_price_csc(const DeviceCSC& csc, const ColumnTable& ct, const double* vec, double* d, int32_t p_lo,
                      int32_t p_hi, int32_t cost_mode, SelectPartials sp, const PivotRecord* rec, hipStream_t s);
void launch_price_csc_all(const DeviceCSC& csc, const ColumnTable& ct, const double* vec, double* d, int32_t nr_normal,
                          int32_t cost_mode, SelectPartials sp, int32_t nb_virtual, const PivotRecord* rec, hipStream_t s);
int32_t price_csc_blocks(int32_t p_lo, int32_t p_hi);
void launch_select_partials_csc(SelectPartials sp, int32_t count, const double* d, const DeviceCSC& csc,
                                const ColumnTable& ct, int32_t m, double* aq, PivotRecord* rec, hipStream_t s);
void launch_build_column_csc(const DeviceCSC& csc, const ColumnTable& ct, int32_t m, double* aq, const PivotRecord* rec,
                             hipStream_t s);
void launch_lu_ftran(const DeviceLU& lu, const double* aq, double* v, double* scratch, const PivotRecord* rec,
                     hipStream_t s);
void launch_lu_btran(const DeviceLU& lu, const DeferredUpdate& du, const double* rhs, int32_t row, double* rho,
                     double* scratch, const PivotRecord* rec, hipStream_t s);
void launch_lu_btran_rows(const DeviceLU& lu, const DeferredUpdate& none, double* out, int64_t ld, double* scratch,
                          hipStream_t s);

size_t ft_lds_base_bytes(int32_t m, int32_t tcap, int32_t eta_cap, int32_t tier, int32_t rhs_cap);
int64_t ft_schedule_stage_bytes(int32_t m, int64_t nnz, int32_t n_levels, int32_t n_seg);
void launch_ft_run(const DeviceLU& lu, const FtState& st, const FtProblem& pb, int64_t max_pivots, hipStream_t s);
void launch_ft_ftran(const DeviceLU& lu, const FtState& st, const FtProblem& pb, int32_t column, const double* rhs, double* alpha,
                     hipStream_t s);
void launch_ft_btran(const DeviceLU& lu, const FtState& st, const FtProblem& pb, int32_t row, const double* rhs, double* rho,
                     hipStream_t s);
void launch_ft_update(const DeviceLU& lu, const FtState& st, const FtProblem& pb, hipStream_t s);
void launch_ft_replay(const DeviceLU& lu, const FtState& st, const FtProblem& pb, int32_t count, hipStream_t s);

void launch_pack_candidate(const double* aq, int32_t m, double* msg, PivotRecord* rec, hipStream_t s);
void launch_select_candidate(const double* msgs, int32_t count, int64_t msg_len, int32_t m, double* aq,
                             int32_t rule, double tol_tie, PivotRecord* rec, hipStream_t s);
void launch_gather_alpha(const double* slices, int32_t count, int32_t stride, int32_t m, double* alpha,
                         const PivotRecord* rec, hipStream_t s);
void launch_pad_slice(double* slice, int32_t valid, int32_t stride, hipStream_t s);

}
```

rust-lp_amd/csrc/relp_kernels_tableau.hip:

```cpp
#include "relp_device_common.h"

namespace relp {

typedef double double4_t __attribute__((ext_vector_type(4)));

__global__ void k_tab_build(TableauView tv, const double* __restrict__ A, int64_t ld_a, ColumnTable ct) {
    const int64_t total = (int64_t)tv.m * (tv.c_hi - tv.c_lo);
    for (int64_t idx = (int64_t)blockIdx.x * blockDim.x + threadIdx.x; idx < total; idx += (int64_t)gridDim.x * blockDim.x) {
        const int c = tv.c_lo + (int)(idx / tv.m), i = (int)(idx % tv.m);
        double v = 0.0;
        if (c < ct.nr_artificial) {
            v = (i == ct.column_to_row[c]) ? 1.0 : 0.0;
        } else {
            const int p = c - ct.nr_artificial;
            if (p < ct.nr_normal) {
                if (i < ct.nr_constraints) v = A[(int64_t)p * ld_a + i];
                else v = (i == ct.bound_row[p]) ? 1.0 : 0.0;
            } else {
                const int vv = p - ct.nr_normal;
                if (i == ct.vrow0[vv]) v = (double)ct.vsign[vv];
                else if (i == ct.vrow1[vv]) v = 1.0;
            }
        }
        tv.T0[(int64_t)c * tv.ld_t + i] = v;
    }
}

__global__ __launch_bounds__(kThreads) void k_tab_price_init(TableauView tv, const double* __restrict__ w,
                                                             const double* __restrict__ cost_store) {
    __shared__ double s_partial[4 * kVecPerBlock];
    const int v0 = tv.c_lo + blockIdx.x * kVecPerBlock;
    double dot = 0.0;
    block_multi_dot(tv.T0, tv.ld_t, tv.m, v0, tv.c_hi, w, s_partial, dot);
    const int c = v0 + threadIdx.x;
    if (threadIdx.x < kVecPerBlock && c < tv.c_hi) tv.d[c] = cost_store[c] - dot;
}

__global__ void k_tab_basis_costs(const int32_t* __restrict__ basis_indices, const double* __restrict__ cost_store,
                                  int col_off, int n_store, int m, double* __restrict__ w) {
    const int i = blockIdx.x * blockDim.x + threadIdx.x;
    if (i >= m) return;
    const int j = basis_indices[i];
    const int c = j + col_off;
    w[i] = (j < kWrappedArtificialBase && c >= 0 && c < n_store) ? cost_store[c] : 0.0;
}

__global__ __launch_bounds__(kThreads) void k_tab_scan(TableauView tv, SelectPartials sp, const PivotRecord* rec) {
    if (rec->outcome != DEV_RUNNING) return;
    const int c = tv.c_lo + blockIdx.x * kThreads + threadIdx.x;
    const int j = c - tv.col_off;
    double key = INFINITY;
    int kj = 0x7fffffff;
    if (c < tv.c_hi && j >= 0 && j < tv.n) {
        const double v = tv.d[c];
        if (!sp.in_basis[j] && v < -sp.tol_cost) { key = select_key(sp.rule, sp.n, rec, j, v); kj = j; }
    }
    block_partial_min(key, kj, sp, blockIdx.x);
}

__global__ __launch_bounds__(kSingleBlock) void k_tab_select(TableauView tv, SelectPartials sp, int count,
                                                             PivotRecord* rec) {
    if (rec->outcome != DEV_RUNNING) return;
    __shared__ double s_k1[kSingleBlock / 64];
    __shared__ int s_j[kSingleBlock / 64];
    double k1 = INFINITY;
    int bj = 0x7fffffff;
    for (int t = threadIdx.x; t < count; t += kSingleBlock) {
        const double key = sp.k1[t];
        const int j = sp.j[t];
        if (key < k1 || (key == k1 && j < bj)) { k1 = key; bj = j; }
    }
#pragma unroll
    for (int off = 32; off > 0; off >>= 1) {
        const double ok = __shfl_down(k1, off, 64);
        const int oj = __shfl_down(bj, off, 64);
        if (ok < k1 || (ok == k1 && oj < bj)) { k1 = ok; bj = oj; }
    }
    const int lane = threadIdx.x & 63, wave = threadIdx.x >> 6;
    if (lane == 0) { s_k1[wave] = k1; s_j[wave] = bj; }
    __syncthreads();
    if (threadIdx.x == 0) {
        for (int w = 1; w < kSingleBlock / 64; ++w)
            if (s_k1[w] < k1 || (s_k1[w] == k1 && s_j[w] < bj)) { k1 = s_k1[w]; bj = s_j[w]; }
        s_k1[0] = k1;
        s_j[0] = bj;
    }
    __syncthreads();
    k1 = s_k1[0];
    bj = s_j[0];
    __syncthreads();
    if (bj != 0x7fffffff && sp.rule == 2 && sp.tol_tie > 0.0) {
        const double bound = k1 + sp.tol_tie * fmax(1.0, fabs(k1));
        int lowest = 0x7fffffff;
        const int grp = threadIdx.x >> 8, u = threadIdx.x & 255;
        for (int t = grp; t < count; t += kSingleBlock / kThreads) {
            if (!(sp.k1[t] <= bound)) continue;
            const int c = tv.c_lo + t * kThreads + u;
            const int j = c - tv.col_off;
            if (c < tv.c_hi && j >= 0 && j < tv.n) {
                const double v = tv.d[c];
                if (!sp.in_basis[j] && v < -sp.tol_cost && v <= bound && j < lowest) lowest = j;
            }
        }
#pragma unroll
        for (int off = 32; off > 0; off >>= 1) lowest = min(lowest, __shfl_down(lowest, off, 64));
        if (lane == 0) s_j[wave] = lowest;
        __syncthreads();
        if (threadIdx.x == 0) {
            int low = 0x7fffffff;
            for (int w = 0; w < kSingleBlock / 64; ++w) low = min(low, s_j[w]);
            bj = low;
        }
    }
    if (threadIdx.x == 0) {
        if (bj == 0x7fffffff) {
            rec->outcome = DEV_NO_CANDIDATE;
            if (sp.rule == 1) rec->last_selected = -1;
        } else {
            rec->q = bj;
            rec->d_q = tv.d[bj + tv.col_off];
            rec->key1 = k1;
            if (sp.rule == 1) rec->last_selected = bj;
        }
    }
}

__global__ __launch_bounds__(kThreads) void k_tab_column(TableauView tv, DeferredUpdate du, double* __restrict__ alpha,
                                                         const PivotRecord* rec) {
    if (rec->outcome != DEV_RUNNING) return;
    __shared__ double s_vs[kMaxEta];
    const int p = rec->n_eta;
    const int cq = rec->q + tv.col_off;
    if ((int)threadIdx.x < p) s_vs[threadIdx.x] = tv.R0[(int64_t)threadIdx.x * tv.ld_r + cq];
    __syncthreads();
    const int i = blockIdx.x * kThreads + threadIdx.x;
    if (i >= tv.m) return;
    double a = tv.T0[(int64_t)cq * tv.ld_t + i];
    for (int j = 0; j < p; ++j) a = fma(du.W[(int64_t)j * du.ld + i], s_vs[j], a);
    alpha[i] = a;
}

__device__ __forceinline__ void tab_row_update_core(const TableauView& tv, const DeferredUpdate& du, const SelectPartials& sp,
                                                    const PivotRecord& R, int block, const double* s_wr, int p_old, int jt, int r,
                                                    int q, int leaving, double d_q, double alpha_r) {
    const PivotRecord* rec = &R;
    const int c = tv.c_lo + block * kThreads + threadIdx.x;
    const double d_old = c < tv.c_hi ? tv.d[c] : 0.0;
    __syncthreads();
    double key = INFINITY;
    int kj = 0x7fffffff;
    if (c < tv.c_hi) {
        double base;
        if (jt < p_old) base = tv.R0[(int64_t)jt * tv.ld_r + c];
        else {
            base = tv.T0[(int64_t)c * tv.ld_t + r];
            tv.R0[(int64_t)jt * tv.ld_r + c] = base;
        }
        double row = base;
        for (int j = 0; j < p_old; ++j) row = fma(s_wr[j], tv.R0[(int64_t)j * tv.ld_r + c], row);
        const double theta = d_q / alpha_r;
        const int j = c - tv.col_off;
        double dn = fma(-theta, row, d_old);
        if (j == q) dn = 0.0;
        tv.d[c] = dn;
        if (j >= 0 && j < tv.n) {
            const bool basic = (j == q) || (sp.in_basis[j] && j != leaving);
            if (!basic && dn < -sp.tol_cost) { key = select_key(sp.rule, sp.n, rec, j, dn); kj = j; }
        }
    }
    block_partial_min(key, kj, sp, block);
}

__device__ __forceinline__ void tab_row_update_body(const TableauView& tv, const DeferredUpdate& du,
                                                    const SelectPartials& sp, const PivotRecord& R, int block) {
    __shared__ double s_wr[kMaxEta];
    if ((int)threadIdx.x < du.kmax) s_wr[threadIdx.x] = du.wr[threadIdx.x];
    tab_row_update_core(tv, du, sp, R, block, s_wr, R.n_eta_old, R.eta_target, R.r, R.q, R.leaving, R.d_q, R.alpha_r);
}

__global__ __launch_bounds__(kThreads) void k_tab_row_update(TableauView tv, DeferredUpdate du, SelectPartials sp,
                                                             PivotRecord* rec) {
    const PivotRecord R = *rec;
    if (R.outcome != DEV_RUNNING) return;
    tab_row_update_body(tv, du, sp, R, blockIdx.x);
}

__device__ __forceinline__ void tab_update_w_vectors_body(const DeferredUpdate& du, int m, const double* __restrict__ alpha,
                                                          double* __restrict__ b, int32_t* __restrict__ basis_indices,
                                                          uint8_t* __restrict__ in_basis, int32_t* __restrict__ trace,
                                                          int64_t trace_cap, const PivotRecord& R, PivotRecord* rec,
                                                          int block) {
    __shared__ double s_wr2[kMaxEta];
    const int p_old = R.n_eta_old, jt = R.eta_target, r = R.r;
    if ((int)threadIdx.x < du.kmax) s_wr2[threadIdx.x] = du.wr[threadIdx.x];
    const int i = block * kThreads + threadIdx.x;
    const double a_i = i < m ? alpha[i] : 0.0;
    const double b_i = i < m ? b[i] : 0.0;
    __syncthreads();
    const double ar = R.alpha_r;
    const double br = R.b_r / ar;
    if (i < m) {
        const double a = a_i;
        const double u = (i == r) ? (1.0 / ar - 1.0) : (-a / ar);
        if (u != 0.0) {
            for (int j = 0; j < p_old; ++j) {
                const double w = s_wr2[j];
                if (w != 0.0) du.W[(int64_t)j * du.ld + i] = fma(u, w, du.W[(int64_t)j * du.ld + i]);
            }
        }
        double* tgt = du.W + (int64_t)jt * du.ld + i;
        if (jt < p_old) *tgt += u; else *tgt = u;
        if (i == r) b[i] = br;
        else if (a != 0.0) b[i] = fma(-a, br, b_i);
    }
    if (i == 0) {
        const int q = R.q, leaving = R.leaving;
        rec->minus_objective = fma(-R.d_q, br, R.minus_objective);
        basis_indices[r] = q;
        if (leaving < kWrappedArtificialBase) in_basis[leaving] = 0;
        in_basis[q] = 1;
        const long long it = R.iterations;
        if (trace && it < trace_cap) {
            trace[0 * trace_cap + it] = R.phase;
            trace[1 * trace_cap + it] = q;
            trace[2 * trace_cap + it] = r;
            trace[3 * trace_cap + it] = leaving;
        }
        if (br == 0.0) rec->degenerate += 1;
        rec->iterations = it + 1;
    }
}

__global__ __launch_bounds__(kThreads) void k_tab_update_w_vectors(DeferredUpdate du, int m,
                                                                   const double* __restrict__ alpha,
                                                                   double* __restrict__ b,
                                                                   int32_t* __restrict__ basis_indices,
                                                                   uint8_t* __restrict__ in_basis,
                                                                   int32_t* __restrict__ trace, int64_t trace_cap,
                                                                   PivotRecord* rec) {
    const PivotRecord R = *rec;
    if (R.outcome != DEV_RUNNING) return;
    tab_update_w_vectors_body(du, m, alpha, b, basis_indices, in_basis, trace, trace_cap, R, rec, blockIdx.x);
}

__global__ __launch_bounds__(kThreads) void k_tab_update_all(TableauView tv, DeferredUpdate du, SelectPartials sp,
                                                             int nb_row, int m, const double* __restrict__ alpha,
                                                             double* __restrict__ b, int32_t* __restrict__ basis_indices,
                                                             uint8_t* __restrict__ in_basis, int32_t* __restrict__ trace,
                                                             int64_t trace_cap, PivotRecord* rec) {
    const PivotRecord R = *rec;
    if (R.outcome != DEV_RUNNING) return;
    if ((int)blockIdx.x < nb_row) tab_row_update_body(tv, du, sp, R, blockIdx.x);
    else tab_update_w_vectors_body(du, m, alpha, b, basis_indices, in_basis, trace, trace_cap, R, rec, blockIdx.x - nb_row);
}

__global__ __launch_bounds__(kThreads) void k_tab_ratio_update_all(TableauView tv, DeferredUpdate du, SelectPartials sp, int nb_row,
                                                                   int m, const double* alpha,
                                                                   const double* __restrict__ b_in, double* __restrict__ b_out,
                                                                   const int32_t* __restrict__ basis_in,
                                                                   int32_t* __restrict__ basis_out, uint8_t* in_basis,
                                                                   int32_t* __restrict__ trace, int64_t trace_cap, Tolerances tol,
                                                                   const double* rmin, int nblk,
                                                                   double* __restrict__ shadow, int32_t* __restrict__ shadow_meta,
                                                                   PivotRecord* rec, const double* __restrict__ msgs, int count,
                                                                   int64_t msg_len, int rule) {
    const double first = (!msgs && (int)threadIdx.x < nblk) ? rmin[threadIdx.x] : INFINITY;
    PivotRecord R = *rec;
    const bool w_half = (int)blockIdx.x >= nb_row;
    const int wblock = (int)blockIdx.x - nb_row;
    const int i = wblock * kThreads + threadIdx.x;
    const bool mine = w_half && i < m;
    if (R.outcome != DEV_RUNNING) {
        if (mine) { b_out[i] = b_in[i]; basis_out[i] = basis_in[i]; }
        return;
    }
    if (msgs) {
        constexpr int kMaxRanks = 64;
        __shared__ double s_key[kMaxRanks], s_idx[kMaxRanks], s_dq[kMaxRanks];
        __shared__ int s_win;
        for (int g = threadIdx.x; g < count && g < kMaxRanks; g += kThreads) {
            s_key[g] = msgs[g * msg_len + 0]; s_idx[g] = msgs[g * msg_len + 1]; s_dq[g] = msgs[g * msg_len + 2];
        }
        __syncthreads();
        if (threadIdx.x == 0) {
            int win = -1; double k1 = INFINITY; double kj = 0.0;
            for (int g = 0; g < count; ++g) {
                const double a = s_key[g], j = s_idx[g];
                if (a < k1 || (a == k1 && win >= 0 && j < kj)) { k1 = a; kj = j; win = g; }
            }
            if (win >= 0 && rule == 2 && tol.tie > 0.0) {
                const double bound = k1 + tol.tie * fmax(1.0, fabs(k1));
                for (int g = 0; g < count; ++g)
                    if (s_key[g] <= bound && s_idx[g] < kj) { kj = s_idx[g]; win = g; }
            }
            s_win = win;
        }
        __syncthreads();
        const int win = s_win;
        if (win < 0) {
            if (mine) { b_out[i] = b_in[i]; basis_out[i] = basis_in[i]; }
            if (wblock == 0 && threadIdx.x == 0) {
                rec->outcome = DEV_NO_CANDIDATE;
                if (rule == 1) rec->last_selected = -1;
            }
            return;
        }
        R.q = (int)s_idx[win];
        R.d_q = s_dq[win];
        if (rule == 1) R.last_selected = R.q;
        alpha = msgs + win * msg_len + 3;
        rmin = alpha + m;
    }
    int r, leaving;
    ratio_blocks_pick<kThreads>(alpha, b_in, basis_in, m, tol, rmin, nblk, &r, &leaving, first, !msgs);
    if (r < 0) {
        if (mine) { b_out[i] = b_in[i]; basis_out[i] = basis_in[i]; }
        if (wblock == 0 && threadIdx.x == 0) rec->outcome = DEV_NO_ROW;
        return;
    }
    __shared__ double s_wr[kMaxEta];
    __shared__ double s_ab[2];
    __shared__ int s_jt;
    const int p_old = R.p_now;
    if ((int)threadIdx.x < p_old) s_wr[threadIdx.x] = du.W[(int64_t)threadIdx.x * du.ld + r];
    if (threadIdx.x == 0) {
        s_ab[0] = alpha[r]; s_ab[1] = b_in[r];
        const int slot = du.pos_of_row[r];
        s_jt = slot < 0 ? p_old : slot;
    }
    __syncthreads();
    const double alpha_r = s_ab[0], b_r = s_ab[1];
    const int jt = s_jt, q = R.q;
    if (!w_half) {
        tab_row_update_core(tv, du, sp, R, blockIdx.x, s_wr, p_old, jt, r, q, leaving, R.d_q, alpha_r);
        return;
    }
    const double br = b_r / alpha_r;
    if (i < m) {
        const double a = alpha[i], b_i = b_in[i];
        const double u = (i == r) ? (1.0 / alpha_r - 1.0) : (-a / alpha_r);
        if (i != r) {
            if (u != 0.0) {
                for (int j = 0; j < p_old; ++j) {
                    const double w = s_wr[j];
                    if (w != 0.0) du.W[(int64_t)j * du.ld + i] = fma(u, w, du.W[(int64_t)j * du.ld + i]);
                }
            }
            double* tgt = du.W + (int64_t)jt * du.ld + i;
            if (jt < p_old) *tgt += u; else *tgt = u;
        } else {
            for (int j = 0; j < p_old; ++j) {
                const double w = s_wr[j];
                shadow[j] = (u != 0.0 && w != 0.0) ? fma(u, w, w) : w;
            }
            if (jt < p_old) shadow[jt] += u; else shadow[jt] = u;
            shadow_meta[0] = r;
            shadow_meta[1] = jt < p_old ? p_old : p_old + 1;
        }
        b_out[i] = (i == r) ? br : (a != 0.0 ? fma(-a, br, b_i) : b_i);
        basis_out[i] = (i == r) ? q : basis_in[i];
    }
    if (i == 0) {
        if (msgs) { rec->q = q; rec->d_q = R.d_q; if (rule == 1) rec->last_selected = q; }
        rec->r = r; rec->leaving = leaving; rec->alpha_r = alpha_r; rec->b_r = b_r;
        rec->n_eta_old = p_old; rec->eta_target = jt;
        if (jt >= p_old) { du.S[p_old] = r; du.pos_of_row[r] = p_old; rec->n_eta = p_old + 1; }
        rec->minus_objective = fma(-R.d_q, br, R.minus_objective);
        if (leaving < kWrappedArtificialBase) in_basis[leaving] = 0;
        in_basis[q] = 1;
        const long long it = R.iterations;
        if (trace && it < trace_cap) {
            trace[0 * trace_cap + it] = R.phase;
            trace[1 * trace_cap + it] = q;
            trace[2 * trace_cap + it] = r;
            trace[3 * trace_cap + it] = leaving;
        }
        if (br == 0.0) rec->degenerate += 1;
        rec->iterations = it + 1;
    }
}

__global__ void k_tab_apply_shadow(DeferredUpdate du, double* __restrict__ shadow, int32_t* __restrict__ shadow_meta) {
    const int row = shadow_meta[0], len = shadow_meta[1];
    if (row < 0) return;
    for (int j = threadIdx.x; j < len; j += blockDim.x) du.W[(int64_t)j * du.ld + row] = shadow[j];
    __syncthreads();
    if (threadIdx.x == 0) shadow_meta[0] = -1;
}

__global__ __launch_bounds__(kThreads) void k_tab_select_column(TableauView tv, DeferredUpdate du, SelectPartials sp,
                                                                int count, double* alpha, double* msg,
                                                                const double* b, Tolerances tol,
                                                                double* rmin, PivotRecord* rec,
                                                                const double* shadow = nullptr, int32_t* shadow_meta = nullptr) {
    const int outcome = rec->outcome, p = rec->n_eta;
    if (shadow_meta) {
        const int srow = shadow_meta[0], slen = shadow_meta[1];
        if (srow >= 0 && srow / kThreads == (int)blockIdx.x) {
            if ((int)threadIdx.x < slen) du.W[(int64_t)threadIdx.x * du.ld + srow] = shadow[threadIdx.x];
            __syncthreads();
            if (threadIdx.x == 0) shadow_meta[0] = -1;
        }
        if (blockIdx.x == 0 && threadIdx.x == 0) rec->p_now = p;
    }
    double k1 = INFINITY;
    int bj = 0x7fffffff;
    if ((int)threadIdx.x < count) { k1 = sp.k1[threadIdx.x]; bj = sp.j[threadIdx.x]; }
    const int i = blockIdx.x * kThreads + threadIdx.x;
    const double b_i = (rmin && i < tv.m) ? b[i] : 0.0;
    if (outcome != DEV_RUNNING) return;
    __shared__ double s_k1[kThreads / 64];
    __shared__ int s_j[kThreads / 64];
    __shared__ double s_vs[kMaxEta];
    const int lane = threadIdx.x & 63, wave = threadIdx.x >> 6;
    for (int t = threadIdx.x + kThreads; t < count; t += kThreads) {
        const double key = sp.k1[t];
        const int j = sp.j[t];
        if (key < k1 || (key == k1 && j < bj)) { k1 = key; bj = j; }
    }
#pragma unroll
    for (int off = 32; off > 0; off >>= 1) {
        const double ok = __shfl_down(k1, off, 64);
        const int oj = __shfl_down(bj, off, 64);
        if (ok < k1 || (ok == k1 && oj < bj)) { k1 = ok; bj = oj; }
    }
    if (lane == 0) { s_k1[wave] = k1; s_j[wave] = bj; }
    __syncthreads();
    k1 = s_k1[0]; bj = s_j[0];
    for (int w = 1; w < kThreads / 64; ++w)
        if (s_k1[w] < k1 || (s_k1[w] == k1 && s_j[w] < bj)) { k1 = s_k1[w]; bj = s_j[w]; }
    __syncthreads();
    if (bj != 0x7fffffff && sp.rule == 2 && sp.tol_tie > 0.0) {
        const double bound = k1 + sp.tol_tie * fmax(1.0, fabs(k1));
        int lowest = 0x7fffffff;
        constexpr int kListMax = 32;
        __shared__ int s_list[kListMax];
        __shared__ int s_cnt;
        if (threadIdx.x == 0) s_cnt = 0;
        __syncthreads();
        for (int t = threadIdx.x; t < count; t += kThreads) {
            if (!(sp.k1[t] <= bound)) continue;
            const int pos = atomicAdd(&s_cnt, 1);
            if (pos < kListMax) s_list[pos] = t;
        }
        __syncthreads();
        const int listed = s_cnt;
        auto scan_slot = [&](int t) {
            const int c = tv.c_lo + t * kThreads + threadIdx.x;
            const int j = c - tv.col_off;
            if (c < tv.c_hi && j >= 0 && j < tv.n) {
                const double v = tv.d[c];
                if (!sp.in_basis[j] && v < -sp.tol_cost && v <= bound && j < lowest) lowest = j;
            }
        };
        if (listed <= kListMax) {
            for (int i = 0; i < listed; ++i) scan_slot(s_list[i]);
        } else {
            for (int t = 0; t < count; ++t)
                if (sp.k1[t] <= bound) scan_slot(t);
        }
#pragma unroll
        for (int off = 32; off > 0; off >>= 1) lowest = min(lowest, __shfl_down(lowest, off, 64));
        if (lane == 0) s_j[wave] = lowest;
        __syncthreads();
        bj = s_j[0];
        for (int w = 1; w < kThreads / 64; ++w) bj = min(bj, s_j[w]);
    }
    if (bj == 0x7fffffff) {
        if (msg) {
            if (i < tv.m) alpha[i] = 0.0;
            if (i == 0) { msg[0] = INFINITY; msg[1] = 0.0; msg[2] = 0.0; }
        } else if (blockIdx.x == 0 && threadIdx.x == 0) {
            rec->outcome = DEV_NO_CANDIDATE;
            if (sp.rule == 1) rec->last_selected = -1;
        }
        return;
    }
    const int cq = bj + tv.col_off;
    if (blockIdx.x == 0 && threadIdx.x == 0) {
        if (msg) { msg[0] = k1; msg[1] = (double)bj; msg[2] = tv.d[cq]; }
        else {
            rec->q = bj;
            rec->d_q = tv.d[cq];
            rec->key1 = k1;
            if (sp.rule == 1) rec->last_selected = bj;
        }
    }
    if ((int)threadIdx.x < p) s_vs[threadIdx.x] = tv.R0[(int64_t)threadIdx.x * tv.ld_r + cq];
    const double t0 = i < tv.m ? tv.T0[(int64_t)cq * tv.ld_t + i] : 0.0;
    __syncthreads();
    double ratio = INFINITY;
    if (i < tv.m) {
        double a = t0;
        for (int j = 0; j < p; ++j) a = fma(du.W[(int64_t)j * du.ld + i], s_vs[j], a);
        alpha[i] = a;
        const double bz = b_i <= tol.zero ? 0.0 : b_i;
        if (a > tol.pivot) ratio = bz / a;
    }
    if (!rmin) return;
#pragma unroll
    for (int off = 32; off > 0; off >>= 1) ratio = fmin(ratio, __shfl_down(ratio, off, 64));
    if (lane == 0) s_k1[wave] = ratio;
    __syncthreads();
    if (threadIdx.x == 0) rmin[blockIdx.x] = fmin(fmin(s_k1[0], s_k1[1]), fmin(s_k1[2], s_k1[3]));
}

__global__ __launch_bounds__(kSingleBlock) void k_ratio_blocks(const double* __restrict__ alpha, const double* __restrict__ b,
                                                               const int32_t* __restrict__ basis_indices, int m,
                                                               Tolerances tol, DeferredUpdate du,
                                                               const double* __restrict__ rmin, int nblk, PivotRecord* rec) {
    const int outcome = rec->outcome, p = rec->n_eta;
    const double first = (int)threadIdx.x < nblk ? rmin[threadIdx.x] : INFINITY;
    if (outcome != DEV_RUNNING) return;
    ratio_blocks_body<kSingleBlock>(alpha, b, basis_indices, m, tol, du, rmin, nblk, p, rec, first, true);
}

__global__ __launch_bounds__(kSingleBlock) void k_tab_select_candidate_ratio(const double* __restrict__ msgs, int count,
                                                                             int64_t msg_len, int m, double* __restrict__ alpha,
                                                                             const double* __restrict__ b,
                                                                             const int32_t* __restrict__ basis_indices,
                                                                             int rule, Tolerances tol, DeferredUpdate du,
                                                                             int forced_row, PivotRecord* rec) {
    const int outcome = rec->outcome, p = rec->n_eta;
    if (outcome != DEV_RUNNING) return;
    constexpr int kMaxRanks = 64;
    __shared__ double s_key[kMaxRanks], s_idx[kMaxRanks], s_dq[kMaxRanks];
    __shared__ int s_win;
    for (int g = threadIdx.x; g < count && g < kMaxRanks; g += kSingleBlock) {
        s_key[g] = msgs[g * msg_len + 0];
        s_idx[g] = msgs[g * msg_len + 1];
        s_dq[g] = msgs[g * msg_len + 2];
    }
    __syncthreads();
    if (threadIdx.x == 0) {
        int win = -1; double k1 = INFINITY; double kj = 0.0;
        for (int g = 0; g < count; ++g) {
            const double a = s_key[g], j = s_idx[g];
            if (a < k1 || (a == k1 && win >= 0 && j < kj)) { k1 = a; kj = j; win = g; }
        }
        if (win >= 0 && rule == 2 && tol.tie > 0.0) {
            const double bound = k1 + tol.tie * fmax(1.0, fabs(k1));
            for (int g = 0; g < count; ++g)
                if (s_key[g] <= bound && s_idx[g] < kj) { kj = s_idx[g]; win = g; }
        }
        s_win = win;
        if (win < 0) {
            rec->outcome = DEV_NO_CANDIDATE;
            if (rule == 1) rec->last_selected = -1;
        } else {
            rec->q = (int)s_idx[win];
            rec->d_q = s_dq[win];
            if (rule == 1) rec->last_selected = (int)s_idx[win];
        }
    }
    __syncthreads();
    const int win = s_win;
    if (win < 0) return;
    const double* __restrict__ col = msgs + win * msg_len + 3;
    const int nblk = (m + kThreads - 1) / kThreads;
    if (forced_row >= 0) {
        for (int i = threadIdx.x; i < m; i += kSingleBlock) alpha[i] = col[i];
        ratio_commit<kSingleBlock>(basis_indices[forced_row], forced_row, col, b, du, p, rec);
        return;
    }
    const double first = (int)threadIdx.x < nblk ? col[m + threadIdx.x] : INFINITY;
    constexpr int kCopy = 16;
    double cp[kCopy];
#pragma unroll
    for (int u = 0; u < kCopy; ++u) {
        const int i = threadIdx.x + u * kSingleBlock;
        cp[u] = i < m ? col[i] : 0.0;
    }
    ratio_blocks_body<kSingleBlock>(col, b, basis_indices, m, tol, du, col + m, nblk, p, rec, first, true);
#pragma unroll
    for (int u = 0; u < kCopy; ++u) {
        const int i = threadIdx.x + u * kSingleBlock;
        if (i < m) alpha[i] = cp[u];
    }
    for (int i = threadIdx.x + kCopy * kSingleBlock; i < m; i += kSingleBlock) alpha[i] = col[i];
}

__global__ void k_tab_update_vectors(int m, const double* __restrict__ alpha, double* __restrict__ b,
                                     int32_t* __restrict__ basis_indices, uint8_t* __restrict__ in_basis,
                                     int32_t* __restrict__ trace, int64_t trace_cap, PivotRecord* rec) {
    if (rec->outcome != DEV_RUNNING) return;
    const int i = blockIdx.x * blockDim.x + threadIdx.x;
    const int r = rec->r;
    const double br = rec->b_r / rec->alpha_r;
    if (i < m) {
        if (i == r) b[i] = br;
        else {
            const double a = alpha[i];
            if (a != 0.0) b[i] = fma(-a, br, b[i]);
        }
    }
    if (i == 0) {
        const int q = rec->q, leaving = rec->leaving;
        rec->minus_objective = fma(-rec->d_q, br, rec->minus_objective);
        basis_indices[r] = q;
        if (leaving < kWrappedArtificialBase) in_basis[leaving] = 0;
        in_basis[q] = 1;
        const long long it = rec->iterations;
        if (trace && it < trace_cap) {
            trace[0 * trace_cap + it] = rec->phase;
            trace[1 * trace_cap + it] = q;
            trace[2 * trace_cap + it] = r;
            trace[3 * trace_cap + it] = leaving;
        }
        if (br == 0.0) rec->degenerate += 1;
        rec->iterations = it + 1;
    }
}

template <int MT, int NT>
__global__ __launch_bounds__(kThreads) void k_tab_flush(TableauView tv, DeferredUpdate du, const int32_t* p_dev,
                                                        unsigned long long* stats) {
    constexpr int kFlushMT = MT, kFlushNT = NT;
    const int p = *p_dev;
    if (p == 0) return;
    if (stats && blockIdx.x == 0 && blockIdx.y == 0 && threadIdx.x == 0) { stats[0] += 1; stats[1] += tv.c_hi - tv.c_lo; }
    const int lane = threadIdx.x & 63, wave = threadIdx.x >> 6;
    const int c_wave = tv.c_lo + blockIdx.x * (2 * 16 * MT) + (wave & 1) * (16 * MT);
    const int i_wave = blockIdx.y * (2 * 16 * NT) + (wave >> 1) * (16 * NT);
    if (c_wave >= tv.c_hi || i_wave >= tv.m) return;
    const int lm = lane & 15, lk = lane >> 4;
    double4_t acc[kFlushMT][kFlushNT];
#pragma unroll
    for (int a = 0; a < kFlushMT; ++a)
#pragma unroll
        for (int b = 0; b < kFlushNT; ++b)
#pragma unroll
            for (int g = 0; g < 4; ++g) {
                const int c = c_wave + a * 16 + lk + 4 * g;
                const int i = i_wave + b * 16 + lm;
                acc[a][b][g] = (c < tv.c_hi && i < tv.m) ? tv.T0[(int64_t)c * tv.ld_t + i] : 0.0;
            }
    double af[kFlushMT], bf[kFlushNT], afn[kFlushMT], bfn[kFlushNT];
    auto load_frags = [&](int k0, double* fa, double* fb) {
        const int k = k0 + lk;
        const bool kv = k < p;
#pragma unroll
        for (int a = 0; a < kFlushMT; ++a) {
            const int c = c_wave + a * 16 + lm;
            fa[a] = (kv && c < tv.c_hi) ? tv.R0[(int64_t)k * tv.ld_r + c] : 0.0;
        }
#pragma unroll
        for (int b = 0; b < kFlushNT; ++b) {
            const int i = i_wave + b * 16 + lm;
            fb[b] = (kv && i < tv.m) ? du.W[(int64_t)k * du.ld + i] : 0.0;
        }
    };
    load_frags(0, af, bf);
    for (int k0 = 0; k0 < p; k0 += 4) {
        load_frags(k0 + 4, afn, bfn);
#pragma unroll
        for (int a = 0; a < kFlushMT; ++a)
#pragma unroll
            for (int b = 0; b < kFlushNT; ++b)
                acc[a][b] = __builtin_amdgcn_mfma_f64_16x16x4f64(af[a], bf[b], acc[a][b], 0, 0, 0);
#pragma unroll
        for (int a = 0; a < kFlushMT; ++a) af[a] = afn[a];
#pragma unroll
        for (int b = 0; b < kFlushNT; ++b) bf[b] = bfn[b];
    }
#pragma unroll
    for (int a = 0; a < kFlushMT; ++a)
#pragma unroll
        for (int b = 0; b < kFlushNT; ++b)
#pragma unroll
            for (int g = 0; g < 4; ++g) {
                const int c = c_wave + a * 16 + lk + 4 * g;
                const int i = i_wave + b * 16 + lm;
                if (c < tv.c_hi && i < tv.m) tv.T0[(int64_t)c * tv.ld_t + i] = acc[a][b][g];
            }
}

template <int WC, int WR, int KC, bool kList>
__global__ __launch_bounds__(WC * WR * 64) void k_tab_flush_lds(TableauView tv, DeferredUpdate du, const int32_t* p_dev,
                                                                FlushList fl) {
    constexpr int MT = 4, NT = 2;
    constexpr int TC = WC * 16 * MT, TR = WR * 16 * NT, NTHR = WC * WR * 64;
    constexpr int RA = KC * TC / 2 / NTHR, RB = KC * TR / 2 / NTHR;
    static_assert(RA * NTHR * 2 == KC * TC && RB * NTHR * 2 == KC * TR, "staging must divide evenly");
    const int p = *p_dev;
    const int n_cols = kList ? *fl.count : tv.c_hi - tv.c_lo;
    if (p == 0) return;
    if (kList && (int)blockIdx.y * TC >= n_cols) return;
    if (!kList && fl.stats && blockIdx.x == 0 && blockIdx.y == 0 && threadIdx.x == 0) { fl.stats[0] += 1; fl.stats[1] += n_cols; }
    __shared__ __align__(16) double As[2][KC][TC];
    __shared__ __align__(16) double Bs[2][KC][TR];
    const int tid = threadIdx.x, lane = tid & 63, wave = tid >> 6;
    const int wc = wave % WC, wr = wave / WC;
    const int x_blk = blockIdx.y * TC, i_blk = blockIdx.x * TR;
    const int x_wave = x_blk + wc * 16 * MT, i_wave = i_blk + wr * 16 * NT;
    const bool active = x_wave < n_cols && i_wave < tv.m;
    const int lm = lane & 15, lk = lane >> 4;
    const double* a_src = kList ? fl.R0c : tv.R0 + tv.c_lo;
    const int64_t a_ld = kList ? fl.ld : tv.ld_r;
    const int col_lane = kList && active && x_wave + lane < n_cols ? fl.cols[x_wave + lane] : -1;
    auto column = [&](int a, int g) -> int {
        const int x = a * 16 + lk + 4 * g;
        if (kList) return __shfl(col_lane, x, 64);
        return x_wave + x < n_cols ? tv.c_lo + x_wave + x : -1;
    };
    double2 ra[RA], rb[RB];
    auto gload = [&](int kc) {
#pragma unroll
        for (int u = 0; u < RA; ++u) {
            const int idx = tid + NTHR * u, k = idx / (TC / 2), x = x_blk + 2 * (idx % (TC / 2));
            ra[u] = (kc + k < p && x < a_ld) ? *reinterpret_cast<const double2*>(a_src + (int64_t)(kc + k) * a_ld + x)
                                             : make_double2(0.0, 0.0);
        }
#pragma unroll
        for (int u = 0; u < RB; ++u) {
            const int idx = tid + NTHR * u, k = idx / (TR / 2), i = i_blk + 2 * (idx % (TR / 2));
            rb[u] = (kc + k < p && i < (int)du.ld) ? *reinterpret_cast<const double2*>(du.W + (int64_t)(kc + k) * du.ld + i)
                                                   : make_double2(0.0, 0.0);
        }
    };
    auto lstore = [&](int buf) {
#pragma unroll
        for (int u = 0; u < RA; ++u) {
            const int idx = tid + NTHR * u;
            *reinterpret_cast<double2*>(&As[buf][idx / (TC / 2)][2 * (idx % (TC / 2))]) = ra[u];
        }
#pragma unroll
        for (int u = 0; u < RB; ++u) {
            const int idx = tid + NTHR * u;
            *reinterpret_cast<double2*>(&Bs[buf][idx / (TR / 2)][2 * (idx % (TR / 2))]) = rb[u];
        }
    };
    gload(0);
    double4_t acc[MT][NT];
#pragma unroll
    for (int a = 0; a < MT; ++a)
#pragma unroll
        for (int b = 0; b < NT; ++b)
#pragma unroll
            for (int g = 0; g < 4; ++g) {
                const int c = column(a, g);
                const int i = i_wave + b * 16 + lm;
                acc[a][b][g] = (active && c >= 0 && i < tv.m) ? tv.T0[(int64_t)c * tv.ld_t + i] : 0.0;
            }
    lstore(0);
    __syncthreads();
    const int nchunks = (p + KC - 1) / KC;
    for (int ch = 0; ch < nchunks; ++ch) {
        const int buf = ch & 1;
        if (ch + 1 < nchunks) gload((ch + 1) * KC);
        if (active) {
            const int kmax = min(KC, p - ch * KC);
            for (int k0 = 0; k0 < kmax; k0 += 4) {
                double af[MT], bf[NT];
#pragma unroll
                for (int a = 0; a < MT; ++a) af[a] = As[buf][k0 + lk][wc * 16 * MT + a * 16 + lm];
#pragma unroll
                for (int b = 0; b < NT; ++b) bf[b] = Bs[buf][k0 + lk][wr * 16 * NT + b * 16 + lm];
#pragma unroll
                for (int a = 0; a < MT; ++a)
#pragma unroll
                    for (int b = 0; b < NT; ++b)
                        acc[a][b] = __builtin_amdgcn_mfma_f64_16x16x4f64(af[a], bf[b], acc[a][b], 0, 0, 0);
            }
        }
        if (ch + 1 < nchunks) lstore(buf ^ 1);
        __syncthreads();
    }
    if (!active) return;
#pragma unroll
    for (int a = 0; a < MT; ++a)
#pragma unroll
        for (int b = 0; b < NT; ++b)
#pragma unroll
            for (int g = 0; g < 4; ++g) {
                const int c = column(a, g);
                const int i = i_wave + b * 16 + lm;
                if (c >= 0 && i < tv.m) tv.T0[(int64_t)c * tv.ld_t + i] = acc[a][b][g];
            }
}

__global__ __launch_bounds__(kThreads) void k_tab_flush_mark(TableauView tv, FlushList fl, const int32_t* p_dev) {
    const int p = *p_dev;
    if (p == 0) return;
    __shared__ unsigned long long s_mask[kThreads / 64];
    const int lane = threadIdx.x & 63, wave = threadIdx.x >> 6;
    const int c = tv.c_lo + blockIdx.x * 64 + lane;
    bool nz = false;
    if (c < tv.c_hi) {
        for (int j0 = wave; j0 < p; j0 += 4 * 8) {
            double v[8];
#pragma unroll
            for (int u = 0; u < 8; ++u) v[u] = j0 + 4 * u < p ? tv.R0[(int64_t)(j0 + 4 * u) * tv.ld_r + c] : 0.0;
#pragma unroll
            for (int u = 0; u < 8; ++u) nz |= !(v[u] == 0.0);
        }
    }
    const unsigned long long m = __ballot(nz);
    if (lane == 0) s_mask[wave] = m;
    __syncthreads();
    if (threadIdx.x == 0) fl.mask[blockIdx.x] = s_mask[0] | s_mask[1] | s_mask[2] | s_mask[3];
}

__global__ __launch_bounds__(kThreads) void k_tab_flush_compact(TableauView tv, FlushList fl, const int32_t* p_dev, int nb) {
    const int p = *p_dev;
    if (p == 0) return;
    __shared__ int s_before[kThreads / 64];
    const int lane = threadIdx.x & 63, wave = threadIdx.x >> 6;
    int before = 0;
    for (int b = threadIdx.x; b < (int)blockIdx.x; b += kThreads) before += __popcll(fl.mask[b]);
#pragma unroll
    for (int off = 32; off > 0; off >>= 1) before += __shfl_down(before, off, 64);
    if (lane == 0) s_before[wave] = before;
    __syncthreads();
    before = s_before[0] + s_before[1] + s_before[2] + s_before[3];
    const unsigned long long mask = fl.mask[blockIdx.x];
    if ((mask >> lane) & 1ull) {
        const int c = tv.c_lo + blockIdx.x * 64 + lane;
        const int x = before + __popcll(mask & ((1ull << lane) - 1ull));
        if (wave == 0) fl.cols[x] = c;
        for (int j0 = wave; j0 < p; j0 += 4 * 8) {
            double v[8];
#pragma unroll
            for (int u = 0; u < 8; ++u) v[u] = j0 + 4 * u < p ? tv.R0[(int64_t)(j0 + 4 * u) * tv.ld_r + c] : 0.0;
#pragma unroll
            for (int u = 0; u < 8; ++u)
                if (j0 + 4 * u < p) fl.R0c[(int64_t)(j0 + 4 * u) * fl.ld + x] = v[u];
        }
    }
    if ((int)blockIdx.x == nb - 1 && threadIdx.x == 0) {
        const int count = before + __popcll(mask);
        *fl.count = count;
        fl.stats[0] += 1;
        fl.stats[1] += count;
    }
}

__global__ void k_tab_gather_columns(TableauView tv, const int32_t* __restrict__ cols, double* __restrict__ out) {
    const int64_t total = (int64_t)tv.m * tv.m;
    for (int64_t idx = (int64_t)blockIdx.x * blockDim.x + threadIdx.x; idx < total; idx += (int64_t)gridDim.x * blockDim.x) {
        const int k = (int)(idx / tv.m), i = (int)(idx % tv.m);
        out[(int64_t)i * tv.m + k] = tv.T0[(int64_t)cols[k] * tv.ld_t + i];
    }
}

__global__ __launch_bounds__(kThreads) void k_tab_row(TableauView tv, DeferredUpdate du, int row, double* __restrict__ out,
                                                      const PivotRecord* rec) {
    __shared__ double s_w[kMaxEta];
    const int p = rec->n_eta;
    if ((int)threadIdx.x < p) s_w[threadIdx.x] = du.W[(int64_t)threadIdx.x * du.ld + row];
    __syncthreads();
    const int c = tv.c_lo + blockIdx.x * kThreads + threadIdx.x;
    if (c >= tv.c_hi) return;
    double v = tv.T0[(int64_t)c * tv.ld_t + row];
    for (int j = 0; j < p; ++j) v = fma(s_w[j], tv.R0[(int64_t)j * tv.ld_r + c], v);
    out[c - tv.c_lo] = v;
}

__global__ __launch_bounds__(kThreads) void k_tab_zero_level_scan(TableauView tv, DeferredUpdate du, SelectPartials sp, int row,
                                                                  int nr_artificial, Tolerances tol, const PivotRecord* rec) {
    const int outcome = rec->outcome, p = rec->n_eta;
    if (outcome != DEV_RUNNING) return;
    __shared__ double s_w[kMaxEta];
    if ((int)threadIdx.x < p) s_w[threadIdx.x] = du.W[(int64_t)threadIdx.x * du.ld + row];
    __syncthreads();
    const int c = tv.c_lo + blockIdx.x * kThreads + threadIdx.x;
    const int j = c - tv.col_off;
    double key = INFINITY;
    int kj = 0x7fffffff;
    if (c < tv.c_hi && j >= nr_artificial && j < tv.n && !sp.in_basis[j] && fabs(tv.d[c]) <= tol.cost) {
        double v = tv.T0[(int64_t)c * tv.ld_t + row];
        for (int k = 0; k < p; ++k) v = fma(s_w[k], tv.R0[(int64_t)k * tv.ld_r + c], v);
        if (fabs(v) > tol.pivot) { key = (double)j; kj = j; }
    }
    block_partial_min(key, kj, sp, blockIdx.x);
}

int32_t tab_scan_blocks(int32_t n_owned_columns) { return cdiv(n_owned_columns, kThreads); }

void launch_tab_build(const TableauView& tv, const double* A, int64_t ld_a, const ColumnTable& ct, hipStream_t s) {
    const int64_t total = (int64_t)tv.m * (tv.c_hi - tv.c_lo);
    if (total <= 0) return;
    hipLaunchKernelGGL(k_tab_build, dim3(element_blocks(total)), dim3(256), 0, s, tv, A, ld_a, ct);
}

void launch_tab_price_init(const TableauView& tv, const double* w, const double* cost_store, hipStream_t s) {
    if (tv.c_hi <= tv.c_lo) return;
    hipLaunchKernelGGL(k_tab_price_init, dim3(cdiv(tv.c_hi - tv.c_lo, kVecPerBlock)), dim3(kThreads), 0, s, tv, w,
                       cost_store);
}

void launch_tab_basis_costs(const TableauView& tv, const int32_t* basis_indices, const double* cost_store, double* w,
                            hipStream_t s) {
    hipLaunchKernelGGL(k_tab_basis_costs, dim3(cdiv(tv.m, 256)), dim3(256), 0, s, basis_indices, cost_store, tv.col_off,
                       tv.n_store, tv.m, w);
}

void launch_tab_scan(const TableauView& tv, SelectPartials sp, const PivotRecord* rec, hipStream_t s) {
    if (tv.c_hi <= tv.c_lo) return;
    hipLaunchKernelGGL(k_tab_scan, dim3(tab_scan_blocks(tv.c_hi - tv.c_lo)), dim3(kThreads), 0, s, tv, sp, rec);
}

void launch_tab_select(const TableauView& tv, SelectPartials sp, int32_t count, PivotRecord* rec, hipStream_t s) {
    hipLaunchKernelGGL(k_tab_select, dim3(1), dim3(kSingleBlock), 0, s, tv, sp, count, rec);
}

void launch_tab_column(const TableauView& tv, const DeferredUpdate& du, double* alpha, const PivotRecord* rec,
                       hipStream_t s) {
    hipLaunchKernelGGL(k_tab_column, dim3(cdiv(tv.m, kThreads)), dim3(kThreads), 0, s, tv, du, alpha, rec);
}

void launch_tab_row_update(const TableauView& tv, const DeferredUpdate& du, SelectPartials sp, PivotRecord* rec,
                           hipStream_t s) {
    if (tv.c_hi <= tv.c_lo) return;
    hipLaunchKernelGGL(k_tab_row_update, dim3(tab_scan_blocks(tv.c_hi - tv.c_lo)), dim3(kThreads), 0, s, tv, du, sp,
                       rec);
}

void launch_tab_update_vectors(int32_t m, const double* alpha, double* b, int32_t* basis_indices, uint8_t* in_basis,
                               int32_t* trace, int64_t trace_cap, PivotRecord* rec, hipStream_t s) {
    hipLaunchKernelGGL(k_tab_update_vectors, dim3(cdiv(m, 256)), dim3(256), 0, s, m, alpha, b, basis_indices, in_basis,
                       trace, trace_cap, rec);
}

void launch_tab_update_w_vectors(const DeferredUpdate& du, int32_t m, const double* alpha, double* b,
                                 int32_t* basis_indices, uint8_t* in_basis, int32_t* trace, int64_t trace_cap,
                                 PivotRecord* rec, hipStream_t s) {
    hipLaunchKernelGGL(k_tab_update_w_vectors, dim3(cdiv(m, kThreads)), dim3(kThreads), 0, s, du, m, alpha, b,
                       basis_indices, in_basis, trace, trace_cap, rec);
}

void launch_tab_select_column(const TableauView& tv, const DeferredUpdate& du, SelectPartials sp, int32_t count,
                              double* alpha, PivotRecord* rec, hipStream_t s) {
    hipLaunchKernelGGL(k_tab_select_column, dim3(cdiv(tv.m, kThreads)), dim3(kThreads), 0, s, tv, du, sp, count, alpha,
                       (double*)nullptr, (const double*)nullptr, Tolerances{}, (double*)nullptr, rec, (const double*)nullptr,
                       (int32_t*)nullptr);
}

void launch_tab_select_column_rmin(const TableauView& tv, const DeferredUpdate& du, SelectPartials sp, int32_t count,
                                   double* alpha, const double* b, Tolerances tol, double* rmin, PivotRecord* rec,
                                   hipStream_t s, const double* shadow, int32_t* shadow_meta) {
    hipLaunchKernelGGL(k_tab_select_column, dim3(cdiv(tv.m, kThreads)), dim3(kThreads), 0, s, tv, du, sp, count, alpha,
                       (double*)nullptr, b, tol, rmin, rec, shadow, shadow_meta);
}

void launch_tab_ratio_update_all(const TableauView& tv, const DeferredUpdate& du, SelectPartials sp, int32_t m,
                                 const double* alpha, const double* b_in, double* b_out, const int32_t* basis_in,
                                 int32_t* basis_out, uint8_t* in_basis, int32_t* trace, int64_t trace_cap, Tolerances tol,
                                 const double* rmin, double* shadow, int32_t* shadow_meta, PivotRecord* rec, hipStream_t s,
                                 const double* msgs, int32_t count, int64_t msg_len, int32_t rule) {
    const int nb_row = tv.c_hi > tv.c_lo ? tab_scan_blocks(tv.c_hi - tv.c_lo) : 0;
    const int nb_w = cdiv(m, kThreads);
    hipLaunchKernelGGL(k_tab_ratio_update_all, dim3(nb_row + nb_w), dim3(kThreads), 0, s, tv, du, sp, nb_row, m, alpha, b_in,
                       b_out, basis_in, basis_out, in_basis, trace, trace_cap, tol, rmin, nb_w, shadow, shadow_meta, rec, msgs,
                       (int)count, msg_len, (int)rule);
}

void launch_tab_apply_shadow(const DeferredUpdate& du, double* shadow, int32_t* shadow_meta, hipStream_t s) {
    hipLaunchKernelGGL(k_tab_apply_shadow, dim3(1), dim3(128), 0, s, du, shadow, shadow_meta);
}

void launch_ratio_blocks(const double* alpha, const double* b, const int32_t* basis_indices, int32_t m, Tolerances tol,
                         const DeferredUpdate& du, const double* rmin, PivotRecord* rec, hipStream_t s) {
    hipLaunchKernelGGL(k_ratio_blocks, dim3(1), dim3(kSingleBlock), 0, s, alpha, b, basis_indices, m, tol, du, rmin,
                       cdiv(m, kThreads), rec);
}

void launch_tab_select_column_msg(const TableauView& tv, const DeferredUpdate& du, SelectPartials sp, int32_t count,
                                  double* msg, const double* b, Tolerances tol, PivotRecord* rec, hipStream_t s,
                                  const double* shadow, int32_t* shadow_meta) {
    hipLaunchKernelGGL(k_tab_select_column, dim3(cdiv(tv.m, kThreads)), dim3(kThreads), 0, s, tv, du, sp, count, msg + 3,
                       msg, b, tol, msg + 3 + tv.m, rec, shadow, shadow_meta);
}

void launch_tab_select_candidate_ratio(const double* msgs, int32_t count, int64_t msg_len, int32_t m, double* alpha,
                                       const double* b, const int32_t* basis_indices, int32_t rule, Tolerances tol,
                                       const DeferredUpdate& du, int32_t forced_row, PivotRecord* rec, hipStream_t s) {
    hipLaunchKernelGGL(k_tab_select_candidate_ratio, dim3(1), dim3(kSingleBlock), 0, s, msgs, count, msg_len, m, alpha, b,
                       basis_indices, rule, tol, du, forced_row, rec);
}

void launch_tab_zero_level_scan(const TableauView& tv, const DeferredUpdate& du, SelectPartials sp, int32_t row,
                                int32_t nr_artificial, Tolerances tol, const PivotRecord* rec, hipStream_t s) {
    if (tv.c_hi <= tv.c_lo) return;
    hipLaunchKernelGGL(k_tab_zero_level_scan, dim3(tab_scan_blocks(tv.c_hi - tv.c_lo)), dim3(kThreads), 0, s, tv, du, sp, row,
                       nr_artificial, tol, rec);
}

void launch_tab_update_all(const TableauView& tv, const DeferredUpdate& du, SelectPartials sp, int32_t m,
                           const double* alpha, double* b, int32_t* basis_indices, uint8_t* in_basis, int32_t* trace,
                           int64_t trace_cap, PivotRecord* rec, hipStream_t s) {
    const int nb_row = tv.c_hi > tv.c_lo ? tab_scan_blocks(tv.c_hi - tv.c_lo) : 0;
    const int nb_w = cdiv(m, kThreads);
    hipLaunchKernelGGL(k_tab_update_all, dim3(nb_row + nb_w), dim3(kThreads), 0, s, tv, du, sp, nb_row, m, alpha, b,
                       basis_indices, in_basis, trace, trace_cap, rec);
}

void launch_tab_flush(const TableauView& tv, const DeferredUpdate& du, const PivotRecord* rec, const FlushList& fl,
                      hipStream_t s) {
    if (tv.c_hi <= tv.c_lo) return;
    const int ncols = tv.c_hi - tv.c_lo;
    const int32_t* p_dev = &rec->n_eta;
    if ((int64_t)ncols * tv.m >= (1 << 16)) {
        constexpr int WC = 2, WR = 4, KC = 16;
        dim3 grid(cdiv(tv.m, WR * 32), cdiv(ncols, WC * 64));
        if (fl.cols) {
            const int nb = cdiv(ncols, 64);
            hipLaunchKernelGGL(k_tab_flush_mark, dim3(nb), dim3(kThreads), 0, s, tv, fl, p_dev);
            hipLaunchKernelGGL(k_tab_flush_compact, dim3(nb), dim3(kThreads), 0, s, tv, fl, p_dev, nb);
            hipLaunchKernelGGL((k_tab_flush_lds<WC, WR, KC, true>), grid, dim3(WC * WR * 64), 0, s, tv, du, p_dev, fl);
        } else {
            hipLaunchKernelGGL((k_tab_flush_lds<WC, WR, KC, false>), grid, dim3(WC * WR * 64), 0, s, tv, du, p_dev, fl);
        }
        return;
    }
    constexpr int MT = 4, NT = 2;
    dim3 grid(cdiv(ncols, 2 * 16 * MT), cdiv(tv.m, 2 * 16 * NT));
    hipLaunchKernelGGL((k_tab_flush<MT, NT>), grid, dim3(kThreads), 0, s, tv, du, p_dev, fl.stats);
}

void launch_tab_gather_columns(const TableauView& tv, const int32_t* cols, double* out, hipStream_t s) {
    const int64_t total = (int64_t)tv.m * tv.m;
    hipLaunchKernelGGL(k_tab_gather_columns, dim3(element_blocks(total)), dim3(256), 0, s, tv, cols, out);
}

void launch_tab_row(const TableauView& tv, const DeferredUpdate& du, int32_t row, double* out, const PivotRecord* rec,
                    hipStream_t s) {
    if (tv.c_hi <= tv.c_lo) return;
    hipLaunchKernelGGL(k_tab_row, dim3(tab_scan_blocks(tv.c_hi - tv.c_lo)), dim3(kThreads), 0, s, tv, du, row, out, rec);
}


}
```

rust-lp_amd/engine.py:

```python
from __future__ import annotations

import ctypes as C
import os
from typing import List, Optional, Tuple

import numpy as np

from .matrix_data import MatrixData

_HERE = os.path.dirname(os.path.abspath(__file__))
LIB_PATH = os.path.join(_HERE, "librelp_engine.so")

FIRST_PROFITABLE, FIRST_PROFITABLE_WITH_MEMORY, STEEPEST_DESCENT = 0, 1, 2
RUNNING, OPTIMAL, UNBOUNDED, INFEASIBLE, PHASE_ONE_DONE, NO_ROW_PHASE_ONE = range(6)
OUTCOME_NAMES = {RUNNING: "running", OPTIMAL: "optimal", UNBOUNDED: "unbounded", INFEASIBLE: "infeasible",
                 PHASE_ONE_DONE: "phase_one_done", NO_ROW_PHASE_ONE: "no_row_phase_one"}
(K_PRICE, K_SELECT_COLUMN, K_BUILD_COLUMN, K_FTRAN, K_RATIO, K_UPDATE_VECTORS, K_UPDATE_INVERSE, K_APPLY_W,
 K_UPDATE_W, K_FLUSH, K_FT_RUN) = range(11)
KERNEL_NAMES = ["price", "select_column", "build_column", "ftran", "ratio", "update_vectors", "update_inverse",
                "apply_w", "update_w", "flush", "ft_run"]
ENGINE_REVISED, ENGINE_TABLEAU, ENGINE_LU, ENGINE_AUTO = 0, 1, 2, 3
RATIO_REFERENCE, RATIO_LARGEST_PIVOT = 0, 1
ARTIFICIAL_REFERENCE, ARTIFICIAL_TEXTBOOK = 0, 1
E_ARG, E_HIP, E_ZERO_PIVOT, E_SINGULAR, E_STATE, E_UNSUPPORTED, E_ALLOC = -1, -2, -3, -4, -5, -6, -7
FORMAT_CSC, FORMAT_DENSE = 0, 1
MEM_HOST, MEM_DEVICE = 0, 1


class RelpError(RuntimeError):
    pass


class _MatrixData(C.Structure):
    _fields_ = [("nr_normal", C.c_int32), ("nr_eq", C.c_int32), ("nr_range", C.c_int32), ("nr_le", C.c_int32),
                ("nr_ge", C.c_int32), ("format", C.c_int32), ("matrix_memory", C.c_int32),
                ("col_ptr", C.c_void_p), ("row_idx", C.c_void_p), ("values", C.c_void_p),
                ("dense", C.c_void_p), ("dense_ld", C.c_int64),
                ("b", C.c_void_p), ("ranges", C.c_void_p), ("cost", C.c_void_p), ("upper_bound", C.c_void_p)]


class Config(C.Structure):
    _fields_ = [("device", C.c_int32), ("phase_one_rule", C.c_int32), ("phase_two_rule", C.c_int32),
                ("tol_cost", C.c_double), ("tol_pivot", C.c_double), ("tol_zero", C.c_double),
                ("tol_tie", C.c_double), ("tol_feas", C.c_double),
                ("poll_interval", C.c_int32), ("trace_capacity", C.c_int32),
                ("shard_rank", C.c_int32), ("shard_count", C.c_int32),
                ("update_block", C.c_int32), ("engine", C.c_int32),
                ("ratio_rule", C.c_int32), ("artificial_removal", C.c_int32),
                ("pivot_rescue", C.c_int32), ("auto_reinversion", C.c_int32)]


_SIGNATURES = {
    "relp_default_config": (None, [C.POINTER(Config)]),
    "relp_robust_config": (None, [C.POINTER(Config)]),
    "relp_engine_kind": (C.c_int32, [C.c_void_p]),
    "relp_robust_stats": (C.c_int, [C.c_void_p, C.POINTER(C.c_int64)]),
    "relp_last_error": (C.c_char_p, [C.c_void_p]),
    "relp_version": (C.c_char_p, []),
    "relp_engine_create": (C.c_int, [C.POINTER(_MatrixData), C.POINTER(Config), C.POINTER(C.c_void_p)]),
    "relp_engine_destroy": (None, [C.c_void_p]),
    "relp_set_stream": (C.c_int, [C.c_void_p, C.c_void_p]),
    "relp_select_primal_pivot_column": (C.c_int, [C.c_void_p, C.c_int32, C.POINTER(C.c_int32), C.POINTER(C.c_int32),
                                                  C.POINTER(C.c_double)]),
    "relp_relative_costs": (C.c_int, [C.c_void_p, C.c_void_p]),
    "relp_generate_column": (C.c_int, [C.c_void_p, C.c_int32, C.c_void_p]),
    "relp_generate_element": (C.c_int, [C.c_void_p, C.c_int32, C.c_int32, C.POINTER(C.c_double)]),
    "relp_select_primal_pivot_row": (C.c_int, [C.c_void_p, C.POINTER(C.c_int32), C.POINTER(C.c_int32)]),
    "relp_select_primal_pivot_row_of": (C.c_int, [C.c_void_p, C.POINTER(C.c_double), C.POINTER(C.c_int32), C.POINTER(C.c_int32)]),
    "relp_bring_into_basis": (C.c_int, [C.c_void_p, C.c_int32, C.c_int32, C.c_double, C.POINTER(C.c_int32)]),
    "relp_run": (C.c_int, [C.c_void_p, C.c_int64, C.POINTER(C.c_int64), C.POINTER(C.c_int32)]),
    "relp_solve_relaxation": (C.c_int, [C.c_void_p, C.c_int64, C.POINTER(C.c_int32)]),
    "relp_from_basis": (C.c_int, [C.c_void_p, C.c_void_p]),
    "relp_flush": (C.c_int, [C.c_void_p]),
    "relp_update_block": (C.c_int32, [C.c_void_p]),
    "relp_tab_flush_stats": (C.c_int, [C.c_void_p, C.POINTER(C.c_int64)]),
    "relp_lu_stats": (C.c_int, [C.c_void_p, C.POINTER(C.c_int64)]),
    "relp_lu_lookahead_stats": (C.c_int, [C.c_void_p, C.POINTER(C.c_int64)]),
    "relp_lu_kernel_layout": (C.c_int, [C.c_void_p, C.POINTER(C.c_int32)]),
    "relp_lu_set_device_factorisation": (C.c_int, [C.c_void_p, C.c_int32]),
    "relp_lu_device_factorisation_stats": (C.c_int, [C.c_void_p, C.POINTER(C.c_int64)]),
    "relp_lu_factor_residual": (C.c_int, [C.c_void_p, C.POINTER(C.c_double)]),
    "relp_lu_phase_cycles": (C.c_int, [C.c_void_p, C.POINTER(C.c_int64)]),
    "relp_basis_inverse_row": (C.c_int, [C.c_void_p, C.c_int32, C.c_void_p]),
    "relp_should_refactor": (C.c_int, [C.c_void_p, C.POINTER(C.c_int32)]),
    "relp_generate_column_of": (C.c_int, [C.c_void_p, C.c_void_p, C.c_void_p, C.c_int32, C.c_void_p]),
    "relp_cost_difference_of": (C.c_int, [C.c_void_p, C.c_void_p, C.c_void_p, C.c_int32, C.POINTER(C.c_double)]),
    "relp_lu_change_basis": (C.c_int, [C.c_void_p, C.c_int32]),
    "relp_lu_set_factors": (C.c_int, [C.c_void_p] + [C.c_void_p] * 6),
    "relp_lu_updates": (C.c_int, [C.c_void_p, C.POINTER(C.c_int32)]),
    "relp_lu_get_update": (C.c_int, [C.c_void_p, C.c_int32, C.POINTER(C.c_int32), C.c_void_p, C.c_void_p, C.c_int32, C.POINTER(C.c_int32)]),
    "relp_lu_get_upper": (C.c_int, [C.c_void_p, C.c_void_p, C.c_void_p, C.c_void_p, C.c_int64, C.POINTER(C.c_int64)]),
    "relp_shard_flush_begin": (C.c_int, [C.c_void_p, C.POINTER(C.c_void_p), C.POINTER(C.c_int64)]),
    "relp_shard_flush_end": (C.c_int, [C.c_void_p]),
    "relp_nr_rows": (C.c_int32, [C.c_void_p]),
    "relp_nr_columns": (C.c_int32, [C.c_void_p]),
    "relp_phase": (C.c_int32, [C.c_void_p]),
    "relp_nr_artificial": (C.c_int32, [C.c_void_p]),
    "relp_get_objective": (C.c_int, [C.c_void_p, C.POINTER(C.c_double)]),
    "relp_get_b": (C.c_int, [C.c_void_p, C.c_void_p]),
    "relp_get_minus_pi": (C.c_int, [C.c_void_p, C.c_void_p]),
    "relp_get_basis_indices": (C.c_int, [C.c_void_p, C.c_void_p]),
    "relp_get_basis_inverse": (C.c_int, [C.c_void_p, C.c_void_p]),
    "relp_current_bfs": (C.c_int, [C.c_void_p, C.c_void_p, C.c_void_p, C.c_int32, C.POINTER(C.c_int32)]),
    "relp_get_iterations": (C.c_int, [C.c_void_p, C.POINTER(C.c_int64)]),
    "relp_get_degenerate_pivots": (C.c_int, [C.c_void_p, C.POINTER(C.c_int64)]),
    "relp_get_trace": (C.c_int, [C.c_void_p, C.c_void_p, C.c_void_p, C.c_void_p, C.c_void_p, C.c_int64,
                                 C.POINTER(C.c_int64)]),
    "relp_check_basis": (C.c_int, [C.c_void_p, C.POINTER(C.c_double), C.POINTER(C.c_double), C.POINTER(C.c_double)]),
    "relp_profile_enable": (C.c_int, [C.c_void_p, C.c_int32, C.c_int64, C.c_int32]),
    "relp_profile_read": (C.c_int, [C.c_void_p, C.c_int32, C.POINTER(C.c_int64), C.POINTER(C.c_double)]),
    "relp_synth_fill_dense": (C.c_int, [C.c_void_p, C.c_int64, C.c_int32, C.c_int32, C.c_uint64, C.c_int64, C.c_void_p]),
    "relp_device_alloc": (C.c_int, [C.POINTER(C.c_void_p), C.c_int64]),
    "relp_device_free": (C.c_int, [C.c_void_p]),
    "relp_shard_ranges": (C.c_int, [C.c_void_p] + [C.POINTER(C.c_int32)] * 5),
    "relp_shard_column_range": (None, [C.c_int32, C.c_int32, C.c_int32, C.POINTER(C.c_int32), C.POINTER(C.c_int32)]),
    "relp_shard_candidate_len": (C.c_int64, [C.c_void_p]),
    "relp_shard_rho_len": (C.c_int64, [C.c_void_p]),
    "relp_shard_price": (C.c_int, [C.c_void_p, C.c_void_p]),
    "relp_shard_select_column": (C.c_int, [C.c_void_p, C.c_void_p, C.c_int32]),
    "relp_shard_ftran": (C.c_int, [C.c_void_p, C.c_void_p]),
    "relp_shard_ratio": (C.c_int, [C.c_void_p, C.c_void_p, C.c_int32, C.c_void_p]),
    "relp_shard_update": (C.c_int, [C.c_void_p, C.c_void_p]),
    "relp_poll": (C.c_int, [C.c_void_p, C.POINTER(C.c_int32), C.POINTER(C.c_int64)]),
    "relp_shard_pivot": (C.c_int, [C.c_void_p]),
    "relp_set_reinversion_interval": (C.c_int, [C.c_void_p, C.c_int64]),
    "relp_reinversions": (C.c_int64, [C.c_void_p]),
    "relp_shard_set_collectives": (C.c_int, [C.c_void_p, C.c_void_p, C.c_void_p, C.c_void_p]),
    "relp_shard_run": (C.c_int, [C.c_void_p, C.c_int64, C.POINTER(C.c_int64), C.POINTER(C.c_int32)]),
    "relp_shard_inject_failure": (C.c_int, [C.c_void_p, C.c_int64]),
    "relp_rccl_unique_id": (C.c_int, [C.POINTER(C.c_uint8)]),
    "relp_rccl_attach": (C.c_int, [C.c_void_p, C.POINTER(C.c_uint8)]),
    "relp_shard_plan": (C.c_int, [C.POINTER(_MatrixData), C.POINTER(Config), C.POINTER(C.c_int32), C.POINTER(C.c_int32)]),
}

_lib = None


def load_library():
    global _lib
    if _lib is None:
        if not os.path.exists(LIB_PATH):
            raise RelpError(f"{LIB_PATH} is missing: run `python -c 'import __graft_entry__ as g; g.build()'` "
                            "(hipcc --offload-arch=gfx950).  There is no CPU fallback.")
        lib = C.CDLL(LIB_PATH)
        for name, (res, args) in _SIGNATURES.items():
            fn = getattr(lib, name)
            fn.restype = res
            fn.argtypes = args
        _lib = lib
    return _lib


def default_config(**overrides) -> Config:
    cfg = Config()
    load_library().relp_default_config(C.byref(cfg))
    for k, v in overrides.items():
        if not hasattr(cfg, k):
            raise TypeError(f"unknown config field {k}")
        setattr(cfg, k, v)
    return cfg


def robust_config(**overrides) -> Config:
    cfg = Config()
    load_library().relp_robust_config(C.byref(cfg))
    for k, v in overrides.items():
        if not hasattr(cfg, k):
            raise TypeError(f"unknown config field {k}")
        setattr(cfg, k, v)
    return cfg


def shard_column_range(nr_normal: int, rank: int, count: int) -> Tuple[int, int]:
    lo, hi = C.c_int32(), C.c_int32()
    load_library().relp_shard_column_range(nr_normal, rank, count, C.byref(lo), C.byref(hi))
    return lo.value, hi.value


def shard_plan(provider: MatrixData, config: Config) -> Tuple[int, int]:
    md = _MatrixData()
    md.nr_normal, md.nr_eq, md.nr_range = provider.nr_normal, provider.nr_eq, provider.nr_range
    md.nr_le, md.nr_ge = provider.nr_le, provider.nr_ge
    ub = np.ascontiguousarray(provider.upper_bound, dtype=np.float64)
    md.upper_bound = ub.ctypes.data
    lo, hi = C.c_int32(), C.c_int32()
    st = load_library().relp_shard_plan(C.byref(md), C.byref(config), C.byref(lo), C.byref(hi))
    if st != 0:
        raise RelpError(f"relp_shard_plan failed ({st})")
    return lo.value, hi.value


class Tableau:

    def __init__(self, provider: MatrixData, config: Optional[Config] = None, *, device_dense_ptr: Optional[int] = None,
                 device_dense_ld: Optional[int] = None, **config_overrides):
        self._lib = load_library()
        cfg = config if config is not None else default_config()
        for k, v in config_overrides.items():
            setattr(cfg, k, v)
        self.config = cfg
        keep = []

        def ptr(a, dtype):
            arr = np.ascontiguousarray(a, dtype=dtype)
            keep.append(arr)
            return arr.ctypes.data

        md = _MatrixData()
        md.nr_normal, md.nr_eq, md.nr_range = provider.nr_normal, provider.nr_eq, provider.nr_range
        md.nr_le, md.nr_ge = provider.nr_le, provider.nr_ge
        if device_dense_ptr is not None:
            md.format, md.matrix_memory = FORMAT_DENSE, MEM_DEVICE
            md.dense = device_dense_ptr
            md.dense_ld = device_dense_ld or provider.nr_constraints
        elif provider.dense is not None:
            md.format, md.matrix_memory = FORMAT_DENSE, MEM_HOST
            dense = np.asfortranarray(provider.dense, dtype=np.float64)
            keep.append(dense)
            md.dense = dense.ctypes.data
            md.dense_ld = dense.shape[0]
        else:
            md.format, md.matrix_memory = FORMAT_CSC, MEM_HOST
            md.col_ptr = ptr(provider.col_ptr, np.int64)
            md.row_idx = ptr(provider.row_idx, np.int32)
            md.values = ptr(provider.values, np.float64)
        md.b = ptr(provider.b, np.float64)
        md.ranges = ptr(provider.ranges, np.float64)
        md.cost = ptr(provider.cost, np.float64)
        md.upper_bound = ptr(provider.upper_bound, np.float64)
        h = C.c_void_p()
        st = self._lib.relp_engine_create(C.byref(md), C.byref(cfg), C.byref(h))
        self._h = h
        if st != 0:
            msg = self._lib.relp_last_error(h).decode() if h else "allocation failed"
            if h:
                self._lib.relp_engine_destroy(h)
            self._h = None
            raise RelpError(f"relp_engine_create failed ({st}): {msg}")
        self.provider = provider
        del keep

    def close(self):
        if getattr(self, "_h", None):
            self._lib.relp_engine_destroy(self._h)
            self._h = None

    def __del__(self):
        try:
            self.close()
        except Exception:
            pass

    def _ck(self, st):
        if st != 0:
            raise RelpError(f"relp call failed ({st}): {self._lib.relp_last_error(self._h).decode()}")

    @property
    def handle(self):
        return self._h

    def set_stream(self, hip_stream: int):
        self._ck(self._lib.relp_set_stream(self._h, hip_stream))

    def nr_rows(self) -> int:
        return self._lib.relp_nr_rows(self._h)

    def nr_columns(self) -> int:
        return self._lib.relp_nr_columns(self._h)

    def nr_artificial_variables(self) -> int:
        return self._lib.relp_nr_artificial(self._h)

    @property
    def phase(self) -> int:
        return self._lib.relp_phase(self._h)

    def select_primal_pivot_column(self, rule: int) -> Optional[Tuple[int, float]]:
        found, col, cost = C.c_int32(), C.c_int32(), C.c_double()
        self._ck(self._lib.relp_select_primal_pivot_column(self._h, rule, C.byref(found), C.byref(col), C.byref(cost)))
        return (col.value, cost.value) if found.value else None

    def relative_costs(self) -> np.ndarray:
        out = np.zeros(self.nr_columns())
        self._ck(self._lib.relp_relative_costs(self._h, out.ctypes.data))
        return out

    def relative_cost(self, j: int) -> float:
        return float(self.relative_costs()[j])

    def generate_column(self, j: int) -> np.ndarray:
        out = np.zeros(self.nr_rows())
        self._ck(self._lib.relp_generate_column(self._h, j, out.ctypes.data))
        return out

    def generate_element(self, i: int, j: int) -> float:
        v = C.c_double()
        self._ck(self._lib.relp_generate_element(self._h, i, j, C.byref(v)))
        return v.value

    def set_reinversion_interval(self, pivots: int) -> None:
        self._ck(self._lib.relp_set_reinversion_interval(self._h, int(pivots)))

    def reinversions(self) -> int:
        return int(self._lib.relp_reinversions(self._h))

    def select_primal_pivot_row(self, column=None) -> Optional[int]:
        found, row = C.c_int32(), C.c_int32()
        if column is None:
            self._ck(self._lib.relp_select_primal_pivot_row(self._h, C.byref(found), C.byref(row)))
        else:
            col = np.ascontiguousarray(column, dtype=np.float64)
            if col.shape != (self.nr_rows(),):
                raise ValueError("column must have nr_rows() entries")
            self._ck(self._lib.relp_select_primal_pivot_row_of(self._h, col.ctypes.data_as(C.POINTER(C.c_double)),
                                                              C.byref(found), C.byref(row)))
        return row.value if found.value else None

    def bring_into_basis(self, column: int, row: int, cost: float) -> int:
        leaving = C.c_int32()
        self._ck(self._lib.relp_bring_into_basis(self._h, column, row, cost, C.byref(leaving)))
        return leaving.value

    def run(self, max_iters: int) -> Tuple[int, int]:
        done, oc = C.c_int64(), C.c_int32()
        self._ck(self._lib.relp_run(self._h, max_iters, C.byref(done), C.byref(oc)))
        return done.value, oc.value

    def solve_relaxation(self, max_iters: int = 1 << 40) -> int:
        oc = C.c_int32()
        self._ck(self._lib.relp_solve_relaxation(self._h, max_iters, C.byref(oc)))
        return oc.value

    def flush(self) -> None:
        self._ck(self._lib.relp_flush(self._h))

    def update_block(self) -> int:
        return self._lib.relp_update_block(self._h)

    def flush_stats(self) -> Tuple[int, int]:
        out = (C.c_int64 * 2)()
        self._ck(self._lib.relp_tab_flush_stats(self._h, out))
        return int(out[0]), int(out[1])

    def engine_kind(self) -> int:
        return int(self._lib.relp_engine_kind(self._h))

    def robust_stats(self) -> dict:
        out = (C.c_int64 * 4)()
        self._ck(self._lib.relp_robust_stats(self._h, out))
        return dict(zip(("small_pivots", "columns_barred", "confirmations", "reinversion_interval"), (int(v) for v in out)))

    def lu_stats(self) -> dict:
        out = (C.c_int64 * 8)()
        self._ck(self._lib.relp_lu_stats(self._h, out))
        keys = ("refactorisations", "m", "nnz_l", "nnz_u", "levels_l", "levels_u", "levels_ut", "levels_lt")
        stats = dict(zip(keys, (int(v) for v in out)))
        la = (C.c_int64 * 4)()
        self._ck(self._lib.relp_lu_lookahead_stats(self._h, la))
        stats.update(lookahead_installs=int(la[0]), replayed_changes=int(la[1]), lookahead=int(la[2]), fuse_lanes=int(la[3]))
        return stats

    def lu_kernel_layout(self) -> dict:
        out = (C.c_int32 * 4)()
        self._ck(self._lib.relp_lu_kernel_layout(self._h, out))
        return {"persistent_kernel": bool(out[0]), "layout": int(out[1]), "tail_slots": int(out[2]), "grid_price": bool(out[3])}

    def lu_set_device_factorisation(self, on: bool) -> None:
        self._ck(self._lib.relp_lu_set_device_factorisation(self._h, 1 if on else 0))

    def lu_factor_residual(self) -> float:
        out = C.c_double()
        self._ck(self._lib.relp_lu_factor_residual(self._h, C.byref(out)))
        return out.value

    def lu_device_factorisation_stats(self) -> dict:
        out = (C.c_int64 * 6)()
        self._ck(self._lib.relp_lu_device_factorisation_stats(self._h, out))
        keys = ("enabled", "device_factorisations", "host_fallbacks", "kernel_us", "last_bump", "last_peeled")
        return dict(zip(keys, (int(v) for v in out)))

    def basis_inverse_row(self, row: int) -> np.ndarray:
        out = np.zeros(self.nr_rows())
        self._ck(self._lib.relp_basis_inverse_row(self._h, row, out.ctypes.data))
        return out

    def should_refactor(self) -> bool:
        v = C.c_int32()
        self._ck(self._lib.relp_should_refactor(self._h, C.byref(v)))
        return bool(v.value)

    @staticmethod
    def _sparse(column):
        idx = np.ascontiguousarray([i for i, _ in column], dtype=np.int32)
        val = np.ascontiguousarray([v for _, v in column], dtype=np.float64)
        return idx, val

    def generate_column_of(self, column) -> np.ndarray:
        idx, val = self._sparse(column)
        out = np.zeros(self.nr_rows())
        self._ck(self._lib.relp_generate_column_of(self._h, idx.ctypes.data, val.ctypes.data, len(idx), out.ctypes.data))
        return out

    def cost_difference_of(self, column) -> float:
        idx, val = self._sparse(column)
        v = C.c_double()
        self._ck(self._lib.relp_cost_difference_of(self._h, idx.ctypes.data, val.ctypes.data, len(idx), C.byref(v)))
        return v.value

    def lu_change_basis(self, pivot_row_index: int) -> None:
        self._ck(self._lib.relp_lu_change_basis(self._h, pivot_row_index))

    def lu_set_factors(self, lower_columns, upper_columns) -> None:
        m = self.nr_rows()

        def csc(cols):
            cols = list(cols) + [[] for _ in range(m - len(cols))]
            ptr = np.zeros(m + 1, dtype=np.int64)
            for j, c in enumerate(cols):
                ptr[j + 1] = ptr[j] + len(c)
            idx = np.ascontiguousarray([i for c in cols for i, _ in c] or [0], dtype=np.int32)
            val = np.ascontiguousarray([v for c in cols for _, v in c] or [0.0], dtype=np.float64)
            return ptr, idx, val
        lp, li, lv = csc(lower_columns)
        up, ui, uv = csc(upper_columns)
        self._ck(self._lib.relp_lu_set_factors(self._h, lp.ctypes.data, li.ctypes.data, lv.ctypes.data, up.ctypes.data,
                                               ui.ctypes.data, uv.ctypes.data))

    def lu_updates(self):
        n = C.c_int32()
        self._ck(self._lib.relp_lu_updates(self._h, C.byref(n)))
        m = self.nr_rows()
        out = []
        for k in range(n.value):
            pivot, nnz = C.c_int32(), C.c_int32()
            idx, val = np.zeros(m, dtype=np.int32), np.zeros(m)
            self._ck(self._lib.relp_lu_get_update(self._h, k, C.byref(pivot), idx.ctypes.data, val.ctypes.data, m, C.byref(nnz)))
            out.append((pivot.value, list(zip(idx[:nnz.value].tolist(), val[:nnz.value].tolist()))))
        return out

    def lu_upper(self):
        m = self.nr_rows()
        cap = m * (m + 1) // 2 + m
        ptr, idx, val, nnz = np.zeros(m + 1, dtype=np.int64), np.zeros(cap, dtype=np.int32), np.zeros(cap), C.c_int64()
        self._ck(self._lib.relp_lu_get_upper(self._h, ptr.ctypes.data, idx.ctypes.data, val.ctypes.data, cap, C.byref(nnz)))
        return [list(zip(idx[ptr[j]:ptr[j + 1]].tolist(), val[ptr[j]:ptr[j + 1]].tolist())) for j in range(m)]

    PHASE_NAMES = ("price", "scatter", "l_solve", "eta_forward", "spike_push", "u_solve", "ratio", "b_update", "u_bar",
                   "ut_solve", "compact", "eta_backward", "lt_solve", "vectors", "load_store", "stage_and_level0")

    def lu_phase_cycles(self) -> dict:
        out = (C.c_int64 * 16)()
        self._ck(self._lib.relp_lu_phase_cycles(self._h, out))
        return dict(zip(self.PHASE_NAMES, (int(v) for v in out)))

    def from_basis(self, basis_columns) -> None:
        arr = np.ascontiguousarray(basis_columns, dtype=np.int32)
        self._ck(self._lib.relp_from_basis(self._h, arr.ctypes.data))

    def objective_function_value(self) -> float:
        v = C.c_double()
        self._ck(self._lib.relp_get_objective(self._h, C.byref(v)))
        return v.value

    def b(self) -> np.ndarray:
        out = np.zeros(self.nr_rows())
        self._ck(self._lib.relp_get_b(self._h, out.ctypes.data))
        return out

    def minus_pi(self) -> np.ndarray:
        out = np.zeros(self.nr_rows())
        self._ck(self._lib.relp_get_minus_pi(self._h, out.ctypes.data))
        return out

    def basis_indices(self) -> np.ndarray:
        out = np.zeros(self.nr_rows(), dtype=np.int32)
        self._ck(self._lib.relp_get_basis_indices(self._h, out.ctypes.data))
        return out

    def basis_inverse(self) -> np.ndarray:
        m = self.nr_rows()
        out = np.zeros((m, m))
        self._ck(self._lib.relp_get_basis_inverse(self._h, out.ctypes.data))
        return out

    def current_bfs(self) -> List[Tuple[int, float]]:
        m = self.nr_rows()
        cols, vals, cnt = np.zeros(m, dtype=np.int32), np.zeros(m), C.c_int32()
        self._ck(self._lib.relp_current_bfs(self._h, cols.ctypes.data, vals.ctypes.data, m, C.byref(cnt)))
        return list(zip(cols[:cnt.value].tolist(), vals[:cnt.value].tolist()))

    def degenerate_pivots(self) -> int:
        out = C.c_int64()
        self._ck(self._lib.relp_get_degenerate_pivots(self._h, C.byref(out)))
        return out.value

    def iterations(self) -> int:
        v = C.c_int64()
        self._ck(self._lib.relp_get_iterations(self._h, C.byref(v)))
        return v.value

    def trace(self) -> List[Tuple[int, int, int, int]]:
        cap = int(self.config.trace_capacity)
        arrs = [np.zeros(max(cap, 1), dtype=np.int32) for _ in range(4)]
        cnt = C.c_int64()
        self._ck(self._lib.relp_get_trace(self._h, *[a.ctypes.data for a in arrs], cap, C.byref(cnt)))
        k = min(cnt.value, cap)
        return list(zip(*(a[:k].tolist() for a in arrs)))

    def check_basis(self) -> Tuple[float, float, float]:
        a, b, c = C.c_double(), C.c_double(), C.c_double()
        self._ck(self._lib.relp_check_basis(self._h, C.byref(a), C.byref(b), C.byref(c)))
        return a.value, b.value, c.value

    def profile_enable(self, enable: bool, max_launches: int = 0, sample_every: int = 1):
        self._ck(self._lib.relp_profile_enable(self._h, int(enable), max_launches, sample_every))

    def profile_read(self):
        out = {}
        for kid, name in enumerate(KERNEL_NAMES):
            n, ms = C.c_int64(), C.c_double()
            self._ck(self._lib.relp_profile_read(self._h, kid, C.byref(n), C.byref(ms)))
            out[name] = (n.value, ms.value)
        return out


def phase_one_primal(tableau: Tableau, max_iters: int = 1 << 40) -> int:
    if tableau.phase != 1:
        raise RelpError("tableau is not artificial")
    return tableau.run(max_iters)[1]


def phase_two_primal(tableau: Tableau, max_iters: int = 1 << 40) -> int:
    if tableau.phase != 2:
        raise RelpError("tableau still has artificial variables")
    return tableau.run(max_iters)[1]


def solve_relaxation(provider: MatrixData, **config_overrides):
    t = Tableau(provider, **config_overrides)
    return t.solve_relaxation(), t


VERIFY_IDENTITY, VERIFY_BASIC, VERIFY_MIN_B = 1e-5, 1e-3, -1e-6
VERIFIED_LEGS = (("read", "robust", ENGINE_LU), ("scaled", "robust", ENGINE_LU), ("scaled", "robust-dantzig", ENGINE_LU),
                 ("scaled", "robust-dantzig", ENGINE_TABLEAU), ("read", "robust-dantzig", ENGINE_LU), ("scaled", "robust", ENGINE_REVISED),
                 ("read", "robust", ENGINE_REVISED), ("read", "robust", ENGINE_TABLEAU), ("scaled", "robust", ENGINE_TABLEAU),
                 ("read", "default", ENGINE_LU), ("read", "default", ENGINE_REVISED), ("read", "default", ENGINE_TABLEAU),
                 ("read", "robust-dantzig", ENGINE_TABLEAU, 12))
_ENGINE_NAMES = {ENGINE_REVISED: "revised", ENGINE_TABLEAU: "tableau", ENGINE_LU: "lu"}


def solve_verified(provider: MatrixData, pivots_per_leg: Optional[int] = None, seconds_per_leg: float = 60.0, legs=VERIFIED_LEGS):
    import time
    budget = pivots_per_leg if pivots_per_leg is not None else 30 * (int(provider.nr_rows) + int(provider.nr_columns))
    report = {"legs": [], "verified": False, "scaled": False}
    scaled = None
    said = {}
    last = RUNNING
    for entry in legs:
        data, cfg_name, kind = entry[:3]
        times = entry[3] if len(entry) > 3 else 1
        leg = {"data": data, "config": cfg_name, "engine": _ENGINE_NAMES[kind]}
        report["legs"].append(leg)
        t0 = time.perf_counter()
        if data == "scaled" and scaled is None:
            scaled = provider.scaled()
        if cfg_name == "robust":
            cfg = robust_config(engine=kind)
        elif cfg_name == "robust-dantzig":
            cfg = robust_config(engine=kind, phase_one_rule=STEEPEST_DESCENT, phase_two_rule=STEEPEST_DESCENT)
        else:
            cfg = default_config(engine=kind)
        try:
            t = Tableau(scaled[0] if data == "scaled" else provider, config=cfg)
        except RelpError as e:
            leg["outcome"] = "create_failed: " + str(e)[:120]
            continue
        try:
            oc, total = RUNNING, 0
            while total < times * budget and time.perf_counter() - t0 < times * seconds_per_leg:
                done, oc = t.run(min(20000, times * budget - total))
                total += done
                if oc not in (RUNNING, PHASE_ONE_DONE):
                    break
            leg["pivots"] = total
            leg["outcome"] = OUTCOME_NAMES.get(oc, str(oc)) if oc not in (RUNNING, PHASE_ONE_DONE) else "limit"
            last = oc
            if oc == OPTIMAL:
                ident, basic, min_b = t.check_basis()
                leg["check_basis"] = [ident, basic, min_b]
                if ident <= VERIFY_IDENTITY and basic <= VERIFY_BASIC and min_b >= VERIFY_MIN_B:
                    report["verified"] = True
                    report["scaled"] = data == "scaled"
                    if data == "scaled":
                        report["row_scale"], report["column_scale"] = scaled[1], scaled[2]
                    return OPTIMAL, t, report
            elif oc in (INFEASIBLE, UNBOUNDED) and data == "read":
                ident, basic, min_b = t.check_basis()
                leg["check_basis"] = [ident, basic, min_b]
                if ident <= VERIFY_IDENTITY and basic <= VERIFY_BASIC and np.isfinite(t.objective_function_value()):
                    said.setdefault(oc, set()).add(kind)
        except RelpError as e:
            leg["outcome"] = "error: " + str(e)[:120]
        t.close()
    for oc, engines in said.items():
        if len(engines) >= 2:
            report["verified"] = True
            return oc, None, report
    return last, None, report
```

Measured before the change: 39310 iterations/s.

## Batch pending eta loads and split W-vector updates across extra blocks

Templates the tableau kernels on a load batch size, so each thread issues B independent loads of W/R0 entries before consuming them. This replaces serial load-fma chains and exposes memory-level parallelism. It also splits the per-row W update in the fused ratio/update kernel across several block groups (w_split, default 2, capped by a CU budget), so the update over the pending eta columns runs on more blocks. The costs are extra template instantiations, higher register pressure and more blocks launched, and the rank-1 W update is now split across blocks, which changes correctness-sensitive indexing.

```diff
diff --git a/include/relp_engine.h b/include/relp_engine.h
--- a/include/relp_engine.h
+++ b/include/relp_engine.h
@@ -112,6 +112,7 @@
 int64_t       relp_reinversions(const relp_engine_t *h);
 relp_status_t relp_flush(relp_engine_t *h);
 relp_status_t relp_tab_flush_stats(relp_engine_t *h, int64_t *out2);
+int32_t       relp_tab_load_batch(const relp_engine_t *h);
 int32_t       relp_update_block(const relp_engine_t *h);
 relp_status_t relp_lu_stats(const relp_engine_t *h, int64_t *out8);
 relp_status_t relp_lu_lookahead_stats(const relp_engine_t *h, int64_t *out4);
diff --git a/rust-lp_amd/csrc/relp_abi.cpp b/rust-lp_amd/csrc/relp_abi.cpp
--- a/rust-lp_amd/csrc/relp_abi.cpp
+++ b/rust-lp_amd/csrc/relp_abi.cpp
@@ -80,6 +80,7 @@
 relp_status_t relp_set_reinversion_interval(relp_engine_t* h, int64_t pivots) { return h ? H(h).set_reinversion_interval(pivots) : RELP_E_ARG; }
 int64_t relp_reinversions(const relp_engine_t* h) { return h ? H(h).reinversions() : -1; }
 int32_t relp_update_block(const relp_engine_t* h) { return h ? H(h).update_block() : -1; }
+int32_t relp_tab_load_batch(const relp_engine_t* h) { return h ? H(h).tab_load_batch_size() : -1; }
 relp_status_t relp_lu_stats(const relp_engine_t* h, int64_t* out8) { return (h && out8) ? H(h).lu_stats(out8) : RELP_E_ARG; }
 relp_status_t relp_lu_lookahead_stats(const relp_engine_t* h, int64_t* out4) { return (h && out4) ? H(h).lu_lookahead_stats(out4) : RELP_E_ARG; }
 relp_status_t relp_lu_kernel_layout(const relp_engine_t* h, int32_t* out4) { return (h && out4) ? H(h).lu_kernel_layout(out4) : RELP_E_ARG; }
diff --git a/rust-lp_amd/csrc/relp_engine.cpp b/rust-lp_amd/csrc/relp_engine.cpp
--- a/rust-lp_amd/csrc/relp_engine.cpp
+++ b/rust-lp_amd/csrc/relp_engine.cpp
@@ -88,6 +88,7 @@
 DeferredUpdate Engine::deferred() const {
     DeferredUpdate du;
     du.W = d_W_; du.ld = ld_b_; du.kmax = block_; du.S = d_S_; du.pos_of_row = d_pos_of_row_; du.wr = d_wr_; du.R = d_R_;
+    du.batch = load_batch_; du.w_split = w_split_;
     return du;
 }
 
@@ -240,6 +241,12 @@
                 HIP_TRY(dev_alloc(&d_fmask_, (n_owned + 63) / 64));
                 HIP_TRY(dev_alloc(&d_R0c_, ld_r_ * block_));
             }
+        }
+        {
+            const char* e = std::getenv("RELP_TAB_LOAD_BATCH");
+            load_batch_ = tab_load_batch(e ? std::atoi(e) : 0);
+            const char* w = std::getenv("RELP_TAB_W_SPLIT");
+            w_split_ = w && std::atoi(w) >= 1 ? std::min(std::atoi(w), 16) : kTabSplitDefault;
         }
         {
             const char* e = std::getenv("RELP_FUSED_UPDATE");
diff --git a/rust-lp_amd/csrc/relp_engine.hpp b/rust-lp_amd/csrc/relp_engine.hpp
--- a/rust-lp_amd/csrc/relp_engine.hpp
+++ b/rust-lp_amd/csrc/relp_engine.hpp
@@ -82,6 +82,7 @@
     relp_status_t get_iterations(int64_t* out);
     relp_status_t get_degenerate_pivots(int64_t* out);
     relp_status_t tab_flush_stats(int64_t* out2);
+    int32_t tab_load_batch_size() const { return tableau_ ? load_batch_ : 0; }
     relp_status_t get_trace(int32_t* phase, int32_t* entering, int32_t* row, int32_t* leaving, int64_t cap,
                             int64_t* count);
     relp_status_t check_basis(double* max_identity_error, double* max_basic_cost, double* min_b);
@@ -137,6 +138,7 @@
     unsigned long long *d_fmask_ = nullptr, *d_fstats_ = nullptr;
     double* d_R0c_ = nullptr;
     FlushList flush_list() const;
+    int32_t load_batch_ = 0, w_split_ = 0;
     double* d_cost_store_ = nullptr;
     int32_t* d_idcol_ = nullptr;
     bool fused_update_ = false, shadow_pending_ = false;
diff --git a/rust-lp_amd/csrc/relp_kernels.h b/rust-lp_amd/csrc/relp_kernels.h
--- a/rust-lp_amd/csrc/relp_kernels.h
+++ b/rust-lp_amd/csrc/relp_kernels.h
@@ -39,6 +39,8 @@
     int32_t* pos_of_row;
     double*  wr;
     double*  R;
+    int32_t  batch;
+    int32_t  w_split;
 };
 
 struct ColumnTable {
@@ -324,6 +326,10 @@
     int64_t             ld;
     unsigned long long* stats;
 };
+static constexpr int32_t kTabLoadBatchDefault = 8;
+static constexpr int32_t kTabSplitDefault = 2;
+static constexpr int32_t kTabSplitCUs = 256;
+int32_t tab_load_batch(int32_t wanted);
 void launch_tab_flush(const TableauView& tv, const DeferredUpdate& du, const PivotRecord* rec, const FlushList& fl,
                       hipStream_t s);
 void launch_tab_ratio_update_all(const TableauView& tv, const DeferredUpdate& du, SelectPartials sp, int32_t m,
diff --git a/rust-lp_amd/csrc/relp_kernels_tableau.hip b/rust-lp_amd/csrc/relp_kernels_tableau.hip
--- a/rust-lp_amd/csrc/relp_kernels_tableau.hip
+++ b/rust-lp_amd/csrc/relp_kernels_tableau.hip
@@ -1,8 +1,39 @@
 #include "relp_device_common.h"
+#include <type_traits>
 
 namespace relp {
 
 typedef double double4_t __attribute__((ext_vector_type(4)));
+
+template <int B, class Use>
+__device__ __forceinline__ void for_pending(const double* base, int64_t stride, int64_t x, int n, Use&& use) {
+    int j0 = 0;
+    for (; j0 + B <= n; j0 += B) {
+        double v[B];
+#pragma unroll
+        for (int t = 0; t < B; ++t) v[t] = base[(int64_t)(j0 + t) * stride + x];
+#pragma unroll
+        for (int t = 0; t < B; ++t) use(j0 + t, v[t]);
+    }
+    if (B > 1 && j0 < n) {
+        double v[B];
+#pragma unroll
+        for (int t = 0; t < B; ++t) v[t] = j0 + t < n ? base[(int64_t)(j0 + t) * stride + x] : 0.0;
+#pragma unroll
+        for (int t = 0; t < B; ++t)
+            if (j0 + t < n) use(j0 + t, v[t]);
+    }
+}
+
+template <int B>
+__device__ __forceinline__ void tab_update_w_row(const DeferredUpdate& du, int i, double u, const double* s_wr, int j0, int j1) {
+    if (u == 0.0 || j1 <= j0) return;
+    double* col = du.W + (int64_t)j0 * du.ld;
+    for_pending<B>(col, du.ld, i, j1 - j0, [&](int j, double old) {
+        const double w = s_wr[j0 + j];
+        if (w != 0.0) col[(int64_t)j * du.ld + i] = fma(u, w, old);
+    });
+}
 
 __global__ void k_tab_build(TableauView tv, const double* __restrict__ A, int64_t ld_a, ColumnTable ct) {
     const int64_t total = (int64_t)tv.m * (tv.c_hi - tv.c_lo);
@@ -125,6 +156,7 @@
     }
 }
 
+template <int B>
 __global__ __launch_bounds__(kThreads) void k_tab_column(TableauView tv, DeferredUpdate du, double* __restrict__ alpha,
                                                          const PivotRecord* rec) {
     if (rec->outcome != DEV_RUNNING) return;
@@ -136,10 +168,11 @@
     const int i = blockIdx.x * kThreads + threadIdx.x;
     if (i >= tv.m) return;
     double a = tv.T0[(int64_t)cq * tv.ld_t + i];
-    for (int j = 0; j < p; ++j) a = fma(du.W[(int64_t)j * du.ld + i], s_vs[j], a);
+    for_pending<B>(du.W, du.ld, i, p, [&](int j, double w) { a = fma(w, s_vs[j], a); });
     alpha[i] = a;
 }
 
+template <int B>
 __device__ __forceinline__ void tab_row_update_core(const TableauView& tv, const DeferredUpdate& du, const SelectPartials& sp,
                                                     const PivotRecord& R, int block, const double* s_wr, int p_old, int jt, int r,
                                                     int q, int leaving, double d_q, double alpha_r) {
@@ -157,7 +190,7 @@
             tv.R0[(int64_t)jt * tv.ld_r + c] = base;
         }
         double row = base;
-        for (int j = 0; j < p_old; ++j) row = fma(s_wr[j], tv.R0[(int64_t)j * tv.ld_r + c], row);
+        for_pending<B>(tv.R0, tv.ld_r, c, p_old, [&](int j, double r0) { row = fma(s_wr[j], r0, row); });
         const double theta = d_q / alpha_r;
         const int j = c - tv.col_off;
         double dn = fma(-theta, row, d_old);
@@ -171,20 +204,23 @@
     block_partial_min(key, kj, sp, block);
 }
 
+template <int B>
 __device__ __forceinline__ void tab_row_update_body(const TableauView& tv, const DeferredUpdate& du,
                                                     const SelectPartials& sp, const PivotRecord& R, int block) {
     __shared__ double s_wr[kMaxEta];
     if ((int)threadIdx.x < du.kmax) s_wr[threadIdx.x] = du.wr[threadIdx.x];
-    tab_row_update_core(tv, du, sp, R, block, s_wr, R.n_eta_old, R.eta_target, R.r, R.q, R.leaving, R.d_q, R.alpha_r);
-}
-
+    tab_row_update_core<B>(tv, du, sp, R, block, s_wr, R.n_eta_old, R.eta_target, R.r, R.q, R.leaving, R.d_q, R.alpha_r);
+}
+
+template <int B>
 __global__ __launch_bounds__(kThreads) void k_tab_row_update(TableauView tv, DeferredUpdate du, SelectPartials sp,
                                                              PivotRecord* rec) {
     const PivotRecord R = *rec;
     if (R.outcome != DEV_RUNNING) return;
-    tab_row_update_body(tv, du, sp, R, blockIdx.x);
-}
-
+    tab_row_update_body<B>(tv, du, sp, R, blockIdx.x);
+}
+
+template <int B>
 __device__ __forceinline__ void tab_update_w_vectors_body(const DeferredUpdate& du, int m, const double* __restrict__ alpha,
                                                           double* __restrict__ b, int32_t* __restrict__ basis_indices,
                                                           uint8_t* __restrict__ in_basis, int32_t* __restrict__ trace,
@@ -202,12 +238,7 @@
     if (i < m) {
         const double a = a_i;
         const double u = (i == r) ? (1.0 / ar - 1.0) : (-a / ar);
-        if (u != 0.0) {
-            for (int j = 0; j < p_old; ++j) {
-                const double w = s_wr2[j];
-                if (w != 0.0) du.W[(int64_t)j * du.ld + i] = fma(u, w, du.W[(int64_t)j * du.ld + i]);
-            }
-        }
+        tab_update_w_row<B>(du, i, u, s_wr2, 0, p_old);
         double* tgt = du.W + (int64_t)jt * du.ld + i;
         if (jt < p_old) *tgt += u; else *tgt = u;
         if (i == r) b[i] = br;
@@ -231,6 +262,7 @@
     }
 }
 
+template <int B>
 __global__ __launch_bounds__(kThreads) void k_tab_update_w_vectors(DeferredUpdate du, int m,
                                                                    const double* __restrict__ alpha,
                                                                    double* __restrict__ b,
@@ -240,9 +272,10 @@
                                                                    PivotRecord* rec) {
     const PivotRecord R = *rec;
     if (R.outcome != DEV_RUNNING) return;
-    tab_update_w_vectors_body(du, m, alpha, b, basis_indices, in_basis, trace, trace_cap, R, rec, blockIdx.x);
-}
-
+    tab_update_w_vectors_body<B>(du, m, alpha, b, basis_indices, in_basis, trace, trace_cap, R, rec, blockIdx.x);
+}
+
+template <int B>
 __global__ __launch_bounds__(kThreads) void k_tab_update_all(TableauView tv, DeferredUpdate du, SelectPartials sp,
                                                              int nb_row, int m, const double* __restrict__ alpha,
                                                              double* __restrict__ b, int32_t* __restrict__ basis_indices,
@@ -250,10 +283,11 @@
                                                              int64_t trace_cap, PivotRecord* rec) {
     const PivotRecord R = *rec;
     if (R.outcome != DEV_RUNNING) return;
-    if ((int)blockIdx.x < nb_row) tab_row_update_body(tv, du, sp, R, blockIdx.x);
-    else tab_update_w_vectors_body(du, m, alpha, b, basis_indices, in_basis, trace, trace_cap, R, rec, blockIdx.x - nb_row);
-}
-
+    if ((int)blockIdx.x < nb_row) tab_row_update_body<B>(tv, du, sp, R, blockIdx.x);
+    else tab_update_w_vectors_body<B>(du, m, alpha, b, basis_indices, in_basis, trace, trace_cap, R, rec, blockIdx.x - nb_row);
+}
+
+template <int B>
 __global__ __launch_bounds__(kThreads) void k_tab_ratio_update_all(TableauView tv, DeferredUpdate du, SelectPartials sp, int nb_row,
                                                                    int m, const double* alpha,
                                                                    const double* __restrict__ b_in, double* __restrict__ b_out,
@@ -263,13 +297,15 @@
                                                                    const double* rmin, int nblk,
                                                                    double* __restrict__ shadow, int32_t* __restrict__ shadow_meta,
                                                                    PivotRecord* rec, const double* __restrict__ msgs, int count,
-                                                                   int64_t msg_len, int rule) {
+                                                                   int64_t msg_len, int rule, int split) {
     const double first = (!msgs && (int)threadIdx.x < nblk) ? rmin[threadIdx.x] : INFINITY;
     PivotRecord R = *rec;
     const bool w_half = (int)blockIdx.x >= nb_row;
-    const int wblock = (int)blockIdx.x - nb_row;
+    const int part = w_half ? ((int)blockIdx.x - nb_row) / nblk : 0;
+    const int wblock = (int)blockIdx.x - nb_row - part * nblk;
     const int i = wblock * kThreads + threadIdx.x;
-    const bool mine = w_half && i < m;
+    const bool lead = w_half && part == 0;
+    const bool mine = lead && i < m;
     if (R.outcome != DEV_RUNNING) {
         if (mine) { b_out[i] = b_in[i]; basis_out[i] = basis_in[i]; }
         return;
@@ -299,7 +335,7 @@
         const int win = s_win;
         if (win < 0) {
             if (mine) { b_out[i] = b_in[i]; basis_out[i] = basis_in[i]; }
-            if (wblock == 0 && threadIdx.x == 0) {
+            if (lead && wblock == 0 && threadIdx.x == 0) {
                 rec->outcome = DEV_NO_CANDIDATE;
                 if (rule == 1) rec->last_selected = -1;
             }
@@ -315,7 +351,7 @@
     ratio_blocks_pick<kThreads>(alpha, b_in, basis_in, m, tol, rmin, nblk, &r, &leaving, first, !msgs);
     if (r < 0) {
         if (mine) { b_out[i] = b_in[i]; basis_out[i] = basis_in[i]; }
-        if (wblock == 0 && threadIdx.x == 0) rec->outcome = DEV_NO_ROW;
+        if (lead && wblock == 0 && threadIdx.x == 0) rec->outcome = DEV_NO_ROW;
         return;
     }
     __shared__ double s_wr[kMaxEta];
@@ -332,22 +368,28 @@
     const double alpha_r = s_ab[0], b_r = s_ab[1];
     const int jt = s_jt, q = R.q;
     if (!w_half) {
-        tab_row_update_core(tv, du, sp, R, blockIdx.x, s_wr, p_old, jt, r, q, leaving, R.d_q, alpha_r);
+        tab_row_update_core<B>(tv, du, sp, R, blockIdx.x, s_wr, p_old, jt, r, q, leaving, R.d_q, alpha_r);
         return;
     }
     const double br = b_r / alpha_r;
+    const int share = (p_old + split - 1) / split;
+    const int j_lo = min(part * share, p_old), j_hi = min(j_lo + share, p_old);
+    if (!lead) {
+        if (i < m && i != r) {
+            const double u = -alpha[i] / alpha_r;
+            tab_update_w_row<B>(du, i, u, s_wr, j_lo, j_hi);
+            if (jt >= j_lo && jt < j_hi) du.W[(int64_t)jt * du.ld + i] += u;
+        }
+        return;
+    }
     if (i < m) {
         const double a = alpha[i], b_i = b_in[i];
         const double u = (i == r) ? (1.0 / alpha_r - 1.0) : (-a / alpha_r);
         if (i != r) {
-            if (u != 0.0) {
-                for (int j = 0; j < p_old; ++j) {
-                    const double w = s_wr[j];
-                    if (w != 0.0) du.W[(int64_t)j * du.ld + i] = fma(u, w, du.W[(int64_t)j * du.ld + i]);
-                }
-            }
+            tab_update_w_row<B>(du, i, u, s_wr, j_lo, j_hi);
             double* tgt = du.W + (int64_t)jt * du.ld + i;
-            if (jt < p_old) *tgt += u; else *tgt = u;
+            if (jt >= p_old) *tgt = u;
+            else if (jt < j_hi) *tgt += u;
         } else {
             for (int j = 0; j < p_old; ++j) {
                 const double w = s_wr[j];
@@ -388,11 +430,12 @@
     if (threadIdx.x == 0) shadow_meta[0] = -1;
 }
 
+template <int B>
 __global__ __launch_bounds__(kThreads) void k_tab_select_column(TableauView tv, DeferredUpdate du, SelectPartials sp,
                                                                 int count, double* alpha, double* msg,
                                                                 const double* b, Tolerances tol,
                                                                 double* rmin, PivotRecord* rec,
-                                                                const double* shadow = nullptr, int32_t* shadow_meta = nullptr) {
+                                                                const double* shadow, int32_t* shadow_meta) {
     const int outcome = rec->outcome, p = rec->n_eta;
     if (shadow_meta) {
         const int srow = shadow_meta[0], slen = shadow_meta[1];
@@ -492,7 +535,7 @@
     double ratio = INFINITY;
     if (i < tv.m) {
         double a = t0;
-        for (int j = 0; j < p; ++j) a = fma(du.W[(int64_t)j * du.ld + i], s_vs[j], a);
+        for_pending<B>(du.W, du.ld, i, p, [&](int j, double w) { a = fma(w, s_vs[j], a); });
         alpha[i] = a;
         const double bz = b_i <= tol.zero ? 0.0 : b_i;
         if (a > tol.pivot) ratio = bz / a;
@@ -843,6 +886,7 @@
     }
 }
 
+template <int B>
 __global__ __launch_bounds__(kThreads) void k_tab_row(TableauView tv, DeferredUpdate du, int row, double* __restrict__ out,
                                                       const PivotRecord* rec) {
     __shared__ double s_w[kMaxEta];
@@ -852,10 +896,11 @@
     const int c = tv.c_lo + blockIdx.x * kThreads + threadIdx.x;
     if (c >= tv.c_hi) return;
     double v = tv.T0[(int64_t)c * tv.ld_t + row];
-    for (int j = 0; j < p; ++j) v = fma(s_w[j], tv.R0[(int64_t)j * tv.ld_r + c], v);
+    for_pending<B>(tv.R0, tv.ld_r, c, p, [&](int j, double r0) { v = fma(s_w[j], r0, v); });
     out[c - tv.c_lo] = v;
 }
 
+template <int B>
 __global__ __launch_bounds__(kThreads) void k_tab_zero_level_scan(TableauView tv, DeferredUpdate du, SelectPartials sp, int row,
                                                                   int nr_artificial, Tolerances tol, const PivotRecord* rec) {
     const int outcome = rec->outcome, p = rec->n_eta;
@@ -869,13 +914,28 @@
     int kj = 0x7fffffff;
     if (c < tv.c_hi && j >= nr_artificial && j < tv.n && !sp.in_basis[j] && fabs(tv.d[c]) <= tol.cost) {
         double v = tv.T0[(int64_t)c * tv.ld_t + row];
-        for (int k = 0; k < p; ++k) v = fma(s_w[k], tv.R0[(int64_t)k * tv.ld_r + c], v);
+        for_pending<B>(tv.R0, tv.ld_r, c, p, [&](int k, double r0) { v = fma(s_w[k], r0, v); });
         if (fabs(v) > tol.pivot) { key = (double)j; kj = j; }
     }
     block_partial_min(key, kj, sp, blockIdx.x);
 }
 
 int32_t tab_scan_blocks(int32_t n_owned_columns) { return cdiv(n_owned_columns, kThreads); }
+
+int32_t tab_load_batch(int32_t wanted) {
+    return (wanted == 1 || wanted == 8 || wanted == 16 || wanted == 32) ? wanted : kTabLoadBatchDefault;
+}
+
+template <class Launch>
+static void with_load_batch(int32_t batch, Launch&& launch) {
+    switch (tab_load_batch(batch)) {
+    case 1:  launch(std::integral_constant<int, 1>{}); break;
+    case 16: launch(std::integral_constant<int, 16>{}); break;
+    case 32: launch(std::integral_constant<int, 32>{}); break;
+    default: launch(std::integral_constant<int, 8>{}); break;
+    }
+    static_assert(kTabLoadBatchDefault == 8, "the default of tab_load_batch is the switch's default case");
+}
 
 void launch_tab_build(const TableauView& tv, const double* A, int64_t ld_a, const ColumnTable& ct, hipStream_t s) {
     const int64_t total = (int64_t)tv.m * (tv.c_hi - tv.c_lo);
@@ -906,14 +966,18 @@
 
 void launch_tab_column(const TableauView& tv, const DeferredUpdate& du, double* alpha, const PivotRecord* rec,
                        hipStream_t s) {
-    hipLaunchKernelGGL(k_tab_column, dim3(cdiv(tv.m, kThreads)), dim3(kThreads), 0, s, tv, du, alpha, rec);
+    with_load_batch(du.batch, [&](auto B) {
+        hipLaunchKernelGGL((k_tab_column<decltype(B)::value>), dim3(cdiv(tv.m, kThreads)), dim3(kThreads), 0, s, tv, du, alpha, rec);
+    });
 }
 
 void launch_tab_row_update(const TableauView& tv, const DeferredUpdate& du, SelectPartials sp, PivotRecord* rec,
                            hipStream_t s) {
     if (tv.c_hi <= tv.c_lo) return;
-    hipLaunchKernelGGL(k_tab_row_update, dim3(tab_scan_blocks(tv.c_hi - tv.c_lo)), dim3(kThreads), 0, s, tv, du, sp,
-                       rec);
+    with_load_batch(du.batch, [&](auto B) {
+        hipLaunchKernelGGL((k_tab_row_update<decltype(B)::value>), dim3(tab_scan_blocks(tv.c_hi - tv.c_lo)), dim3(kThreads), 0, s, tv, du, sp,
+                           rec);
+    });
 }
 
 void launch_tab_update_vectors(int32_t m, const double* alpha, double* b, int32_t* basis_indices, uint8_t* in_basis,
@@ -925,22 +989,28 @@
 void launch_tab_update_w_vectors(const DeferredUpdate& du, int32_t m, const double* alpha, double* b,
                                  int32_t* basis_indices, uint8_t* in_basis, int32_t* trace, int64_t trace_cap,
                                  PivotRecord* rec, hipStream_t s) {
-    hipLaunchKernelGGL(k_tab_update_w_vectors, dim3(cdiv(m, kThreads)), dim3(kThreads), 0, s, du, m, alpha, b,
-                       basis_indices, in_basis, trace, trace_cap, rec);
+    with_load_batch(du.batch, [&](auto B) {
+        hipLaunchKernelGGL((k_tab_update_w_vectors<decltype(B)::value>), dim3(cdiv(m, kThreads)), dim3(kThreads), 0, s, du, m, alpha, b,
+                           basis_indices, in_basis, trace, trace_cap, rec);
+    });
 }
 
 void launch_tab_select_column(const TableauView& tv, const DeferredUpdate& du, SelectPartials sp, int32_t count,
                               double* alpha, PivotRecord* rec, hipStream_t s) {
-    hipLaunchKernelGGL(k_tab_select_column, dim3(cdiv(tv.m, kThreads)), dim3(kThreads), 0, s, tv, du, sp, count, alpha,
-                       (double*)nullptr, (const double*)nullptr, Tolerances{}, (double*)nullptr, rec, (const double*)nullptr,
-                       (int32_t*)nullptr);
+    with_load_batch(du.batch, [&](auto B) {
+        hipLaunchKernelGGL((k_tab_select_column<decltype(B)::value>), dim3(cdiv(tv.m, kThreads)), dim3(kThreads), 0, s, tv, du, sp, count, alpha,
+                           (double*)nullptr, (const double*)nullptr, Tolerances{}, (double*)nullptr, rec, (const double*)nullptr,
+                           (int32_t*)nullptr);
+    });
 }
 
 void launch_tab_select_column_rmin(const TableauView& tv, const DeferredUpdate& du, SelectPartials sp, int32_t count,
                                    double* alpha, const double* b, Tolerances tol, double* rmin, PivotRecord* rec,
                                    hipStream_t s, const double* shadow, int32_t* shadow_meta) {
-    hipLaunchKernelGGL(k_tab_select_column, dim3(cdiv(tv.m, kThreads)), dim3(kThreads), 0, s, tv, du, sp, count, alpha,
-                       (double*)nullptr, b, tol, rmin, rec, shadow, shadow_meta);
+    with_load_batch(du.batch, [&](auto B) {
+        hipLaunchKernelGGL((k_tab_select_column<decltype(B)::value>), dim3(cdiv(tv.m, kThreads)), dim3(kThreads), 0, s, tv, du, sp, count, alpha,
+                           (double*)nullptr, b, tol, rmin, rec, shadow, shadow_meta);
+    });
 }
 
 void launch_tab_ratio_update_all(const TableauView& tv, const DeferredUpdate& du, SelectPartials sp, int32_t m,
@@ -950,9 +1020,12 @@
                                  const double* msgs, int32_t count, int64_t msg_len, int32_t rule) {
     const int nb_row = tv.c_hi > tv.c_lo ? tab_scan_blocks(tv.c_hi - tv.c_lo) : 0;
     const int nb_w = cdiv(m, kThreads);
-    hipLaunchKernelGGL(k_tab_ratio_update_all, dim3(nb_row + nb_w), dim3(kThreads), 0, s, tv, du, sp, nb_row, m, alpha, b_in,
-                       b_out, basis_in, basis_out, in_basis, trace, trace_cap, tol, rmin, nb_w, shadow, shadow_meta, rec, msgs,
-                       (int)count, msg_len, (int)rule);
+    int split = tab_load_batch(du.batch) == 1 ? 1 : std::max(1, std::min({(int)du.w_split, (int)du.kmax, (kTabSplitCUs - nb_row) / nb_w}));
+    with_load_batch(du.batch, [&](auto B) {
+        hipLaunchKernelGGL((k_tab_ratio_update_all<decltype(B)::value>), dim3(nb_row + split * nb_w), dim3(kThreads), 0, s, tv, du, sp, nb_row, m,
+                           alpha, b_in, b_out, basis_in, basis_out, in_basis, trace, trace_cap, tol, rmin, nb_w, shadow,
+                           shadow_meta, rec, msgs, (int)count, msg_len, (int)rule, split);
+    });
 }
 
 void launch_tab_apply_shadow(const DeferredUpdate& du, double* shadow, int32_t* shadow_meta, hipStream_t s) {
@@ -968,8 +1041,10 @@
 void launch_tab_select_column_msg(const TableauView& tv, const DeferredUpdate& du, SelectPartials sp, int32_t count,
                                   double* msg, const double* b, Tolerances tol, PivotRecord* rec, hipStream_t s,
                                   const double* shadow, int32_t* shadow_meta) {
-    hipLaunchKernelGGL(k_tab_select_column, dim3(cdiv(tv.m, kThreads)), dim3(kThreads), 0, s, tv, du, sp, count, msg + 3,
-                       msg, b, tol, msg + 3 + tv.m, rec, shadow, shadow_meta);
+    with_load_batch(du.batch, [&](auto B) {
+        hipLaunchKernelGGL((k_tab_select_column<decltype(B)::value>), dim3(cdiv(tv.m, kThreads)), dim3(kThreads), 0, s, tv, du, sp, count, msg + 3,
+                           msg, b, tol, msg + 3 + tv.m, rec, shadow, shadow_meta);
+    });
 }
 
 void launch_tab_select_candidate_ratio(const double* msgs, int32_t count, int64_t msg_len, int32_t m, double* alpha,
@@ -982,8 +1057,10 @@
 void launch_tab_zero_level_scan(const TableauView& tv, const DeferredUpdate& du, SelectPartials sp, int32_t row,
                                 int32_t nr_artificial, Tolerances tol, const PivotRecord* rec, hipStream_t s) {
     if (tv.c_hi <= tv.c_lo) return;
-    hipLaunchKernelGGL(k_tab_zero_level_scan, dim3(tab_scan_blocks(tv.c_hi - tv.c_lo)), dim3(kThreads), 0, s, tv, du, sp, row,
-                       nr_artificial, tol, rec);
+    with_load_batch(du.batch, [&](auto B) {
+        hipLaunchKernelGGL((k_tab_zero_level_scan<decltype(B)::value>), dim3(tab_scan_blocks(tv.c_hi - tv.c_lo)), dim3(kThreads), 0, s, tv, du, sp,
+                           row, nr_artificial, tol, rec);
+    });
 }
 
 void launch_tab_update_all(const TableauView& tv, const DeferredUpdate& du, SelectPartials sp, int32_t m,
@@ -991,8 +1068,10 @@
                            int64_t trace_cap, PivotRecord* rec, hipStream_t s) {
     const int nb_row = tv.c_hi > tv.c_lo ? tab_scan_blocks(tv.c_hi - tv.c_lo) : 0;
     const int nb_w = cdiv(m, kThreads);
-    hipLaunchKernelGGL(k_tab_update_all, dim3(nb_row + nb_w), dim3(kThreads), 0, s, tv, du, sp, nb_row, m, alpha, b,
-                       basis_indices, in_basis, trace, trace_cap, rec);
+    with_load_batch(du.batch, [&](auto B) {
+        hipLaunchKernelGGL((k_tab_update_all<decltype(B)::value>), dim3(nb_row + nb_w), dim3(kThreads), 0, s, tv, du, sp, nb_row, m, alpha, b,
+                           basis_indices, in_basis, trace, trace_cap, rec);
+    });
 }
 
 void launch_tab_flush(const TableauView& tv, const DeferredUpdate& du, const PivotRecord* rec, const FlushList& fl,
@@ -1026,8 +1105,10 @@
 void launch_tab_row(const TableauView& tv, const DeferredUpdate& du, int32_t row, double* out, const PivotRecord* rec,
                     hipStream_t s) {
     if (tv.c_hi <= tv.c_lo) return;
-    hipLaunchKernelGGL(k_tab_row, dim3(tab_scan_blocks(tv.c_hi - tv.c_lo)), dim3(kThreads), 0, s, tv, du, row, out, rec);
-}
-
-
-}
+    with_load_batch(du.batch, [&](auto B) {
+        hipLaunchKernelGGL((k_tab_row<decltype(B)::value>), dim3(tab_scan_blocks(tv.c_hi - tv.c_lo)), dim3(kThreads), 0, s, tv, du, row, out, rec);
+    });
+}
+
+
+}
diff --git a/rust-lp_amd/engine.py b/rust-lp_amd/engine.py
--- a/rust-lp_amd/engine.py
+++ b/rust-lp_amd/engine.py
@@ -73,6 +73,7 @@
     "relp_from_basis": (C.c_int, [C.c_void_p, C.c_void_p]),
     "relp_flush": (C.c_int, [C.c_void_p]),
     "relp_update_block": (C.c_int32, [C.c_void_p]),
+    "relp_tab_load_batch": (C.c_int32, [C.c_void_p]),
     "relp_tab_flush_stats": (C.c_int, [C.c_void_p, C.POINTER(C.c_int64)]),
     "relp_lu_stats": (C.c_int, [C.c_void_p, C.POINTER(C.c_int64)]),
     "relp_lu_lookahead_stats": (C.c_int, [C.c_void_p, C.POINTER(C.c_int64)]),
@@ -337,6 +338,9 @@
     def update_block(self) -> int:
         return self._lib.relp_update_block(self._h)
 
+    def load_batch(self) -> int:
+        return self._lib.relp_tab_load_batch(self._h)
+
     def flush_stats(self) -> Tuple[int, int]:
         out = (C.c_int64 * 2)()
         self._ck(self._lib.relp_tab_flush_stats(self._h, out))
```

After: 45040 iterations/s, median of 6. 14.6% higher.
